# DSXiangLi/ChineseNER

Hardware: NVIDIA H100
Metric: sentences/sec bert_bilstm_crf MSRA L=128 (higher is better)
Workload: dtype bf16

## Files before the change

### chinesener_b200/_lib.py

```python
import ctypes
import os

import torch

_HERE = os.path.dirname(os.path.abspath(__file__))
LIB_PATH = os.path.join(_HERE, "libner_b200.so")

_c = ctypes
_vp, _i = _c.c_void_p, _c.c_int

SIGNATURES = {
    "ner_strerror": (_c.c_char_p, [_i]),
    "ner_abi_version": (_i, []),
    "ner_build_info": (_c.c_char_p, []),
    "ner_crf_viterbi": (_i, [_vp, _vp, _vp, _vp, _vp, _i, _i, _i, _vp]),
    "ner_crf_viterbi_plan": (_i, [_i, _i, _i, _i, _i]),
    "ner_crf_loglik_fwd": (_i, [_vp, _vp, _vp, _vp, _vp, _vp, _vp, _i, _i, _i, _i, _vp]),
    "ner_crf_loglik_bwd": (_i, [_vp, _vp, _vp, _vp, _vp, _vp, _vp, _c.c_float, _vp, _vp, _i, _i, _i, _vp]),
    "ner_crf_partial_loglik_fwd": (_i, [_vp, _vp, _vp, _vp, _vp, _vp, _vp, _i, _i, _i, _i, _vp]),
    "ner_crf_partial_loglik_bwd": (_i, [_vp, _vp, _vp, _vp, _vp, _vp, _vp, _c.c_float, _vp, _vp, _i, _i, _i, _vp]),
    "ner_crf_distill_fwd": (_i, [_vp, _vp, _vp, _vp, _vp, _c.c_float, _vp, _vp, _i, _i, _i, _i, _vp]),
    "ner_crf_distill_bwd": (_i, [_vp, _vp, _vp, _vp, _vp, _c.c_float, _vp, _vp, _vp, _c.c_float, _vp, _vp, _vp, _i, _i,
                                 _i, _i, _vp]),
    "ner_crf_viterbi_nbest_workspace_bytes": (_c.c_size_t, [_i, _i, _i, _i]),
    "ner_crf_viterbi_nbest": (_i, [_vp, _vp, _vp, _i, _vp, _vp, _vp, _vp, _c.c_size_t, _i, _i, _i, _vp]),
    "ner_gemm_bf16": (_i, [_vp, _vp, _vp, _vp, _vp, _i, _i, _i, _i, _i, _vp]),
    "ner_pack_weight_bf16": (_i, [_vp, _vp, _i, _i, _vp]),
    "ner_cast_bf16": (_i, [_vp, _vp, _c.c_size_t, _vp]),
    "ner_dense_small_n": (_i, [_vp, _i, _vp, _vp, _vp, _i, _i, _i, _vp, _vp]),
    "ner_seq_pack_plan": (_i, [_vp, _vp, _vp, _i, _i, _vp]),
    "ner_bert_embed_ln": (_i, [_vp] * 9 + [_i] * 6 + [_c.c_float, _vp, _i, _vp]),
    "ner_layernorm": (_i, [_vp, _i] + [_vp] * 5 + [_i, _i, _c.c_float, _vp]),
    "ner_layernorm_dropout": (_i, [_vp, _i] + [_vp] * 5 + [_i, _i, _c.c_float, _c.c_float, _c.c_uint64, _vp]),
    "ner_bert_attention": (_i, [_vp, _vp, _vp, _i, _i, _i, _i, _c.c_float, _c.c_float, _vp, _i, _c.c_float, _c.c_uint64, _vp]),
    "ner_bilstm_recurrence": (_i, [_vp] * 5 + [_i, _i, _i, _i, _c.c_float, _vp, _vp, _vp, _vp, _c.c_float, _c.c_uint64, _vp]),
    "ner_bilstm_recurrence_bwd": (_i, [_vp] * 7 + [_i, _i, _i, _i, _c.c_float, _c.c_uint64, _vp]),
    "ner_bigru_recurrence": (_i, [_vp] * 5 + [_i, _i, _i, _i, _i] + [_vp] * 4 + [_c.c_float, _c.c_uint64, _vp]),
    "ner_bigru_recurrence_bwd": (_i, [_vp] * 7 + [_i, _i, _i, _i, _c.c_float, _c.c_uint64, _vp]),
    "ner_transpose_cast_bf16": (_i, [_vp, _vp, _i, _i, _i, _i, _vp]),
    "ner_colsum_add": (_i, [_vp, _vp, _i, _i, _i, _c.c_float, _vp]),
    "ner_dense_small_n_bwd": (_i, [_vp] * 6 + [_i, _i, _i, _vp]),
    "ner_dropout": (_i, [_vp, _vp, _c.c_size_t, _c.c_float, _c.c_uint64, _vp]),
    "ner_relu_bwd_f32": (_i, [_vp, _vp, _vp, _c.c_size_t, _vp]),
    "ner_relu_f32": (_i, [_vp, _vp, _c.c_size_t, _vp]),
    "ner_reduce_max_time": (_i, [_vp, _vp, _i, _i, _i, _vp]),
    "ner_reduce_max_time_bwd": (_i, [_vp, _vp, _vp, _vp, _i, _i, _i, _c.c_float, _vp]),
    "ner_softmax_xent": (_i, [_vp, _vp, _vp, _vp, _i, _i, _c.c_float, _vp]),
    "ner_attention_f32_bwd": (_i, [_vp, _i, _vp, _i, _vp, _i, _vp, _vp, _vp, _vp, _c.c_float, _vp, _i, _vp, _i, _vp, _i, _vp, _i,
                                   _vp, _vp, _i, _i, _i, _i, _vp]),
    "ner_dropout_bf16": (_i, [_vp, _vp, _c.c_size_t, _c.c_float, _c.c_uint64, _vp]),
    "ner_sumsq_add": (_i, [_vp, _c.c_size_t, _vp, _vp, _vp]),
    "ner_sumsq_scratch_floats": (_c.c_size_t, []),
    "ner_token_xent": (_i, [_vp] * 6 + [_c.c_float, _vp, _i, _i, _i, _vp]),
    "ner_token_xent_scratch_floats": (_c.c_size_t, []),
    "ner_token_dice": (_i, [_vp] * 6 + [_c.c_float] * 3 + [_vp, _i, _i, _i, _vp]),
    "ner_mrc_pairs": (_i, [_vp] * 6 + [_i] * 6 + [_vp] * 7),
    "ner_mrc_merge": (_i, [_vp] * 3 + [_i] * 6 + [_vp, _vp]),
    "ner_mrc_span_targets": (_i, [_vp, _vp, _i, _i, _vp, _vp, _vp, _vp]),
    "ner_mrc_span_match_fwd_workspace_bytes": (_c.c_size_t, [_i, _i]),
    "ner_mrc_span_match_fwd": (_i, [_vp, _i] + [_vp] * 5 + [_i] * 3 + [_c.c_float, _c.c_uint64] + [_vp] * 3
                               + [_c.c_size_t, _vp]),
    "ner_mrc_span_match_bwd_workspace_bytes": (_c.c_size_t, [_i, _i]),
    "ner_mrc_span_match_bwd": (_i, [_vp, _i] + [_vp] * 5 + [_i] * 3 + [_c.c_float, _c.c_float, _c.c_uint64] + [_vp] * 5
                               + [_c.c_size_t, _vp]),
    "ner_mrc_span_decode_workspace_bytes": (_c.c_size_t, [_i, _i]),
    "ner_mrc_span_decode": (_i, [_vp] * 3 + [_i] + [_vp] * 5 + [_i] * 8 + [_vp] * 5 + [_c.c_size_t, _vp]),
    "ner_gp_targets": (_i, [_vp] * 3 + [_i] * 3 + [_vp, _vp]),
    "ner_gp_rope": (_i, [_vp, _i, _vp] + [_i] * 3 + [_vp] * 3),
    "ner_gp_rope_bwd": (_i, [_vp, _vp] + [_i] * 3 + [_vp, _i, _vp]),
    "ner_gp_loss_workspace_bytes": (_c.c_size_t, [_i] * 3),
    "ner_gp_loss_fwd": (_i, [_vp] * 5 + [_i] * 3 + [_vp] * 3 + [_c.c_size_t, _vp]),
    "ner_gp_loss_bwd": (_i, [_vp] * 5 + [_i] * 3 + [_c.c_float, _vp, _vp]),
    "ner_gp_decode_workspace_bytes": (_c.c_size_t, [_i] * 3),
    "ner_gp_decode": (_i, [_vp] * 5 + [_i] * 7 + [_vp] * 5 + [_c.c_size_t, _vp]),
    "ner_window_plan": (_i, [_vp] * 3 + [_i] * 5 + [_vp] * 6),
    "ner_layernorm_bwd": (_i, [_vp, _i] + [_vp] * 7 + [_i, _i, _c.c_float, _vp]),
    "ner_layernorm_dropout_bwd": (_i, [_vp, _i] + [_vp] * 7 + [_i, _i, _c.c_float, _c.c_float, _c.c_uint64, _vp]),
    "ner_layernorm_dropout_bwd_bias": (_i, [_vp, _i] + [_vp] * 8 + [_i, _i, _c.c_float, _c.c_float, _c.c_uint64, _vp]),
    "ner_transpose_bf16": (_i, [_vp, _vp, _i, _i, _i, _vp]),
    "ner_colsum_bf16_add": (_i, [_vp, _vp, _i, _i, _vp]),
    "ner_gelu_bf16": (_i, [_vp, _vp, _c.c_size_t, _i, _vp]),
    "ner_gelu_f32": (_i, [_vp, _vp, _c.c_size_t, _i, _vp]),
    "ner_gelu_bwd_bf16": (_i, [_vp, _vp, _vp, _c.c_size_t, _i, _vp]),
    "ner_gelu_bwd_bias_bf16": (_i, [_vp, _vp, _vp, _vp, _i, _i, _i, _vp]),
    "ner_bert_embed_bwd": (_i, [_vp] * 6 + [_i] * 5 + [_vp]),
    "ner_bert_attention_bwd": (_i, [_vp] * 5 + [_i] * 4 + [_c.c_float, _c.c_float, _c.c_float, _c.c_uint64, _vp]),
    "ner_bert_attention_bwd_packed": (_i, [_vp] * 5 + [_i] * 4 + [_c.c_float, _c.c_float, _c.c_uint64, _vp]),
    "ner_gather_rows": (_i, [_vp, _vp, _vp, _i, _i, _vp]),
    "ner_scatter_rows": (_i, [_vp, _vp, _vp, _i, _i, _vp]),
    "ner_adam_step": (_i, [_vp] * 4 + [_c.c_size_t] + [_c.c_float] * 5 + [_i, _c.c_float, _vp, _c.c_float, _vp]),
    "ner_softlexicon_pool_fwd": (_i, [_vp] * 4 + [_i] * 6 + [_vp]),
    "ner_embedding_lookup": (_i, [_vp, _vp, _vp, _i, _i, _i, _i, _vp]),
    "ner_cast_pad_bf16": (_i, [_vp, _vp, _i, _i, _i, _i, _vp]),
    "ner_split_bf16": (_i, [_vp, _vp, _vp, _i, _i, _i, _i, _vp]),
    "ner_attention_f32": (_i, [_vp, _i, _vp, _i, _vp, _i, _vp, _vp, _vp, _vp, _c.c_float, _vp, _vp, _vp, _i, _i, _i, _i, _vp]),
    "ner_softlexicon_pool_bwd": (_i, [_vp] * 4 + [_i] * 5 + [_vp]),
    "ner_multihot_embed_fwd": (_i, [_vp] * 3 + [_i] * 4 + [_vp]),
    "ner_small_table_grad_scratch_floats": (_c.c_size_t, [_i, _i]),
    "ner_small_table_grad": (_i, [_vp] * 4 + [_i] * 4 + [_vp, _vp]),
    "ner_gemm_e4m3": (_i, [_vp] * 7 + [_i] * 4 + [_vp]),
    "ner_quantize_weight_e4m3": (_i, [_vp, _vp, _vp, _i, _i, _vp]),
    "ner_bert_embed_ln_e4m3": (_i, [_vp] * 11 + [_i] * 6 + [_c.c_float, _vp, _i, _vp]),
    "ner_layernorm_e4m3": (_i, [_vp, _i] + [_vp] * 7 + [_i, _i, _c.c_float, _vp]),
}



class BertConfig(_c.Structure):
    _fields_ = [("hidden_size", _i), ("num_heads", _i), ("intermediate_size", _i), ("num_layers", _i),
                ("vocab_size", _i), ("type_vocab_size", _i), ("max_position", _i), ("ln_eps", _c.c_float),
                ("gelu_erf", _i), ("gemm_tile", _i)]


class BertLayerWeights(_c.Structure):
    _fields_ = [(n, _vp) for n in ("wqkv", "bqkv", "wo", "bo", "ln1_gamma", "ln1_beta", "wi", "bi", "wd", "bd",
                                   "ln2_gamma", "ln2_beta")]


class BertLayerWeightsFp8(_c.Structure):
    _fields_ = [(n, _vp) for n in ("wqkv", "sqkv", "bqkv", "wo", "bo", "ln1_gamma", "ln1_beta", "wi", "si", "bi", "wd", "sd",
                                   "bd", "ln2_gamma", "ln2_beta")]


class BertLayerGrads(_c.Structure):
    _fields_ = [(n, _vp) for n in ("wqkv_kn", "wo_kn", "wi_kn", "wd_kn", "d_wq", "d_wk", "d_wv", "d_bq", "d_bk", "d_bv",
                                   "d_wo", "d_bo", "d_ln1_gamma", "d_ln1_beta", "d_wi", "d_bi", "d_wd", "d_bd",
                                   "d_ln2_gamma", "d_ln2_beta")]


SIGNATURES["ner_bert_train_saved_bytes"] = (_c.c_size_t, [_c.POINTER(BertConfig), _i])
SIGNATURES["ner_bert_train_scratch_bytes"] = (_c.c_size_t, [_c.POINTER(BertConfig), _i])
SIGNATURES["ner_bert_encoder_train_fwd"] = (_i, [_c.POINTER(BertConfig)] + [_vp] * 5 + [_c.POINTER(BertLayerWeights)] + [_vp] * 3
                                            + [_i, _i, _c.c_float, _c.c_float, _c.c_uint64, _vp, _vp, _vp, _c.c_size_t, _vp])
SIGNATURES["ner_bert_encoder_train_bwd"] = (_i, [_c.POINTER(BertConfig), _vp, _c.POINTER(BertLayerWeights), _c.POINTER(BertLayerGrads)]
                                            + [_vp] * 5 + [_vp] * 3 + [_i, _i, _c.c_float, _c.c_float, _c.c_uint64, _vp, _vp,
                                                                       _c.c_size_t, _vp, _c.c_size_t, _vp])
SIGNATURES["ner_bert_train_packed_saved_bytes"] = (_c.c_size_t, [_c.POINTER(BertConfig), _i])
SIGNATURES["ner_bert_train_packed_scratch_bytes"] = (_c.c_size_t, [_c.POINTER(BertConfig), _i, _i])
SIGNATURES["ner_bert_encoder_train_fwd_packed"] = (_i, [_c.POINTER(BertConfig)] + [_vp] * 5 + [_c.POINTER(BertLayerWeights)] + [_vp] * 2
                                                   + [_i, _i, _vp, _vp, _i, _c.c_float, _c.c_float, _c.c_uint64, _vp, _vp, _vp,
                                                      _c.c_size_t, _vp])
SIGNATURES["ner_bert_encoder_train_bwd_packed"] = (_i, [_c.POINTER(BertConfig), _vp, _c.POINTER(BertLayerWeights),
                                                        _c.POINTER(BertLayerGrads)] + [_vp] * 5 + [_vp] * 2
                                                   + [_i, _i, _vp, _vp, _i, _c.c_float, _c.c_float, _c.c_uint64, _vp, _vp,
                                                      _c.c_size_t, _vp, _c.c_size_t, _vp])
SIGNATURES["ner_bert_bilstm_crf_predict_workspace_bytes"] = (_c.c_size_t, [_c.POINTER(BertConfig), _i, _i, _i, _i, _i])
SIGNATURES["ner_bert_bilstm_crf_predict"] = (_i, [_c.POINTER(BertConfig)] + [_vp] * 5 + [_c.POINTER(BertLayerWeights)] + [_vp] * 4
                                             + [_i, _i] + [_vp] * 3 + [_i] + [_vp] * 4 + [_i, _i, _i, _vp, _vp, _c.c_size_t, _vp])
SIGNATURES["ner_bert_embed_sum"] = (_i, [_vp] * 6 + [_i] * 6 + [_vp])
SIGNATURES["ner_axpy_f32"] = (_i, [_vp, _vp, _c.c_size_t, _c.c_float, _vp])
SIGNATURES["ner_bert_encoder_workspace_bytes"] = (_c.c_size_t, [_c.POINTER(BertConfig), _i])
SIGNATURES["ner_bert_encoder_fwd"] = (_i, [_c.POINTER(BertConfig)] + [_vp] * 5 + [_c.POINTER(BertLayerWeights)] + [_vp] * 3
                                      + [_i, _i, _vp, _vp, _i, _vp, _vp, _vp, _c.c_size_t, _vp])
SIGNATURES["ner_bert_encoder_fp8_workspace_bytes"] = (_c.c_size_t, [_c.POINTER(BertConfig), _i])
SIGNATURES["ner_bert_encoder_fwd_fp8"] = (_i, [_c.POINTER(BertConfig)] + [_vp] * 5 + [_c.POINTER(BertLayerWeightsFp8)] + [_vp] * 3
                                          + [_i, _i, _vp, _vp, _i, _vp, _vp, _vp, _c.c_size_t, _vp])

class PackEntry(_c.Structure):
    _fields_ = [("src", _vp), ("K", _i), ("N", _i), ("dst_nk_bf16", _vp), ("ld_nk", _i), ("dst_kn_bf16", _vp), ("ld_kn", _i)]


SIGNATURES["ner_pack_weights_group_bf16"] = (_i, [_vp, _vp, _i, _i, _vp])


class WgradProblem(_c.Structure):
    _fields_ = [("x_bf16", _vp), ("ld_x", _i), ("dy_bf16", _vp), ("ld_dy", _i), ("dy_col0", _i), ("dw", _vp), ("k_in", _i),
                ("n_out", _i)]


SIGNATURES["ner_wgrad_group_bf16"] = (_i, [_c.POINTER(WgradProblem), _i, _i, _vp])
SIGNATURES["ner_bert_train_bwd_set_layer_events"] = (_i, [_vp, _i])
SIGNATURES["ner_extract_spans"] = (_i, [_vp, _vp, _vp, _vp, _i, _i, _i, _i, _vp])
SIGNATURES["ner_lexicon_create"] = (_vp, [_vp, _vp, _vp, _i])
SIGNATURES["ner_lexicon_destroy"] = (None, [_vp])
SIGNATURES["ner_lexicon_num_nodes"] = (_c.c_int64, [_vp])
SIGNATURES["ner_lexicon_build"] = (_i, [_vp, _vp, _vp, _i, _vp, _vp, _i, _i, _vp, _vp, _i])
SIGNATURES["ner_lexicon_build_lattice"] = (_i, [_vp, _vp, _vp, _i, _i, _i, _vp, _vp, _vp, _i])
SIGNATURES["ner_lattice_recurrence"] = (_i, [_vp] * 9 + [_i] * 4 + [_vp] * 8)
SIGNATURES["ner_lattice_recurrence_bwd"] = (_i, [_vp] * 16 + [_i] * 4 + [_vp])

VIT_PLANS = ("small", "tma", "parked", "onchip_128", "onchip_32", "small_any_b", "none")

_lib = None


class NerB200Error(RuntimeError):
    pass


def lib():
    global _lib
    if _lib is None:
        if not os.path.exists(LIB_PATH):
            raise NerB200Error(
                f"{LIB_PATH} not found: build it with `python -m chinesener_b200.build` "
                "(there is no CPU fallback for the sm_90a kernels)")
        h = ctypes.CDLL(LIB_PATH)
        for name, (res, args) in SIGNATURES.items():
            fn = getattr(h, name)
            fn.restype = res
            fn.argtypes = args
        _lib = h
    return _lib


LAUNCHES = 0
_HOOK = None


def check(status):
    global LAUNCHES
    LAUNCHES += 1
    if status != 0:
        raise NerB200Error(lib().ner_strerror(status).decode())


def ptr(t):
    return 0 if t is None else t.data_ptr()


_raw_stream = getattr(torch._C, "_cuda_getCurrentRawStream", None)


def stream():
    if _raw_stream is not None:
        return _raw_stream(torch.cuda.current_device())
    return torch.cuda.current_stream().cuda_stream


def require_cuda(*tensors):
    for t in tensors:
        if t is not None and not t.is_cuda:
            raise NerB200Error("ner_b200 kernels take CUDA tensors (got a CPU tensor); there is no CPU path")
        if t is not None and not t.is_contiguous():
            raise NerB200Error("ner_b200 kernels take contiguous row-major tensors")
```

### chinesener_b200/csrc/bert_ops.cu

```cuda
#include "common.cuh"

namespace {

using namespace nerdev;

constexpr int LN_MAXV = 8;

template <bool Q = false>
__device__ __forceinline__ void ln_row(float4 (&v)[LN_MAXV], int nv4, int H, int lane, float eps,
                                       const float* __restrict__ gamma, const float* __restrict__ beta,
                                       float* __restrict__ out_f32, __nv_bfloat16* __restrict__ out_bf16,
                                       uint8_t* __restrict__ out_q = nullptr, float* __restrict__ out_s = nullptr) {
  float s = 0.f;
#pragma unroll
  for (int k = 0; k < LN_MAXV; ++k)
    if (k < nv4 && (lane + 32 * k) * 4 < H) s += v[k].x + v[k].y + v[k].z + v[k].w;
  s = warp_sum(s);
  const float mean = s / (float)H;
  float q = 0.f;
#pragma unroll
  for (int k = 0; k < LN_MAXV; ++k)
    if (k < nv4 && (lane + 32 * k) * 4 < H) {
      const float a = v[k].x - mean, b = v[k].y - mean, c = v[k].z - mean, d = v[k].w - mean;
      q += a * a + b * b + c * c + d * d;
    }
  q = warp_sum(q);
  const float rstd = rsqrtf(q / (float)H + eps);
#pragma unroll
  for (int k = 0; k < LN_MAXV; ++k) {
    const int e = (lane + 32 * k) * 4;
    if (k < nv4 && e < H) {
      const float4 g = __ldg(reinterpret_cast<const float4*>(gamma + e));
      const float4 b = __ldg(reinterpret_cast<const float4*>(beta + e));
      float4 o;
      o.x = (v[k].x - mean) * rstd * g.x + b.x;
      o.y = (v[k].y - mean) * rstd * g.y + b.y;
      o.z = (v[k].z - mean) * rstd * g.z + b.z;
      o.w = (v[k].w - mean) * rstd * g.w + b.w;
      if (out_f32 != nullptr) *reinterpret_cast<float4*>(out_f32 + e) = o;
      if (out_bf16 != nullptr) {
        __nv_bfloat162 lo = __floats2bfloat162_rn(o.x, o.y), hi = __floats2bfloat162_rn(o.z, o.w);
        uint2 pk;
        pk.x = *reinterpret_cast<uint32_t*>(&lo);
        pk.y = *reinterpret_cast<uint32_t*>(&hi);
        *reinterpret_cast<uint2*>(out_bf16 + e) = pk;
      }
      if constexpr (Q) {
        const float s = e4m3_scale(warp_max(fmaxf(fmaxf(fabsf(o.x), fabsf(o.y)), fmaxf(fabsf(o.z), fabsf(o.w)))));
        const uint32_t lo = cvt_e4m3x2(__fdiv_rn(o.x, s), __fdiv_rn(o.y, s)), hi = cvt_e4m3x2(__fdiv_rn(o.z, s), __fdiv_rn(o.w, s));
        *reinterpret_cast<uint32_t*>(out_q + e) = lo | (hi << 16);
        if (lane == 0) out_s[k] = s;
      }
    }
  }
}

template <bool Q>
__global__ void __launch_bounds__(256)
bert_embed_ln_kernel(const float* __restrict__ word_emb, const float* __restrict__ type_emb,
                     const float* __restrict__ pos_emb, const float* __restrict__ gamma,
                     const float* __restrict__ beta, const int32_t* __restrict__ ids,
                     const int32_t* __restrict__ seg, float* __restrict__ out_f32,
                     __nv_bfloat16* __restrict__ out_bf16, int n_tok, int L, int H, int V, int n_type, float eps,
                     const int32_t* __restrict__ tok_src, uint8_t* __restrict__ out_q, float* __restrict__ out_s) {
  const int lane = threadIdx.x & 31;
  const int nv4 = (H / 4 + 31) / 32;
  for (int tok = blockIdx.x * (blockDim.x >> 5) + (threadIdx.x >> 5); tok < n_tok; tok += gridDim.x * (blockDim.x >> 5)) {
    const int src = tok_src ? tok_src[tok] : tok;
    int id = ids[src];
    id = min(max(id, 0), V - 1);
    int sg = (seg != nullptr) ? seg[src] : 0;
    sg = min(max(sg, 0), n_type - 1);
    const int pos = src % L;
    const float* w = word_emb + (size_t)id * H;
    const float* ty = type_emb + (size_t)sg * H;
    const float* po = pos_emb + (size_t)pos * H;
    float4 v[LN_MAXV];
#pragma unroll
    for (int k = 0; k < LN_MAXV; ++k) {
      const int e = (lane + 32 * k) * 4;
      if (k < nv4 && e < H) {
        const float4 a = __ldg(reinterpret_cast<const float4*>(w + e));
        const float4 b = __ldg(reinterpret_cast<const float4*>(ty + e));
        const float4 c = __ldg(reinterpret_cast<const float4*>(po + e));
        v[k] = make_float4(a.x + b.x + c.x, a.y + b.y + c.y, a.z + b.z + c.z, a.w + b.w + c.w);
      }
    }
    ln_row<Q>(v, nv4, H, lane, eps, gamma, beta, out_f32 ? out_f32 + (size_t)tok * H : nullptr,
              out_bf16 ? out_bf16 + (size_t)tok * H : nullptr, Q ? out_q + (size_t)tok * H : nullptr,
              Q ? out_s + (size_t)tok * (H / 128) : nullptr);
  }
}

__global__ void __launch_bounds__(256)
bert_embed_sum_kernel(const float* __restrict__ word_emb, const float* __restrict__ type_emb,
                      const float* __restrict__ pos_emb, const int32_t* __restrict__ ids, const int32_t* __restrict__ seg,
                      float* __restrict__ out, int n_tok, int L, int H, int V, int n_type) {
  const int lane = threadIdx.x & 31;
  for (int tok = blockIdx.x * (blockDim.x >> 5) + (threadIdx.x >> 5); tok < n_tok; tok += gridDim.x * (blockDim.x >> 5)) {
    const int id = min(max(ids[tok], 0), V - 1);
    const int sg = min(max(seg != nullptr ? seg[tok] : 0, 0), n_type - 1);
    const float* w = word_emb + (size_t)id * H;
    const float* ty = type_emb + (size_t)sg * H;
    const float* po = pos_emb + (size_t)(tok % L) * H;
    for (int e = lane * 4; e < H; e += 128) {
      const float4 a = __ldg(reinterpret_cast<const float4*>(w + e));
      const float4 b = __ldg(reinterpret_cast<const float4*>(ty + e));
      const float4 c = __ldg(reinterpret_cast<const float4*>(po + e));
      *reinterpret_cast<float4*>(out + (size_t)tok * H + e) = make_float4(a.x + b.x + c.x, a.y + b.y + c.y, a.z + b.z + c.z, a.w + b.w + c.w);
    }
  }
}

template <bool YBF16, bool DROP, bool Q>
__global__ void __launch_bounds__(256)
layernorm_kernel(const void* __restrict__ yv, const float* __restrict__ residual, const float* __restrict__ gamma,
                 const float* __restrict__ beta, float* __restrict__ out_f32, __nv_bfloat16* __restrict__ out_bf16,
                 int M, int H, float eps, float keep, uint32_t seed_lo, uint32_t seed_hi, uint8_t* __restrict__ out_q,
                 float* __restrict__ out_s) {
  pdl_launch_dependents();
  pdl_wait();
  const int lane = threadIdx.x & 31;
  const int nv4 = (H / 4 + 31) / 32;
  const uint32_t thr = keep_threshold(keep);
  const float inv_keep = 1.f / keep;
  for (int row = blockIdx.x * (blockDim.x >> 5) + (threadIdx.x >> 5); row < M; row += gridDim.x * (blockDim.x >> 5)) {
    const float* r = residual ? residual + (size_t)row * H : nullptr;
    float4 v[LN_MAXV];
#pragma unroll
    for (int k = 0; k < LN_MAXV; ++k) {
      const int e = (lane + 32 * k) * 4;
      if (k < nv4 && e < H) {
        if constexpr (YBF16) {
          const uint2 pk = *reinterpret_cast<const uint2*>(static_cast<const __nv_bfloat16*>(yv) + (size_t)row * H + e);
          const __nv_bfloat162 lo = *reinterpret_cast<const __nv_bfloat162*>(&pk.x);
          const __nv_bfloat162 hi = *reinterpret_cast<const __nv_bfloat162*>(&pk.y);
          v[k] = make_float4(__low2float(lo), __high2float(lo), __low2float(hi), __high2float(hi));
        } else {
          v[k] = *reinterpret_cast<const float4*>(static_cast<const float*>(yv) + (size_t)row * H + e);
        }
        if constexpr (DROP) {
          const size_t i = (size_t)row * H + e;
          const uint32_t hi = seed_hi ^ (uint32_t)(i >> 32), lo = (uint32_t)i;
          v[k].x = hash3(seed_lo, hi, lo) < thr ? v[k].x * inv_keep : 0.f;
          v[k].y = hash3(seed_lo, hi, lo + 1) < thr ? v[k].y * inv_keep : 0.f;
          v[k].z = hash3(seed_lo, hi, lo + 2) < thr ? v[k].z * inv_keep : 0.f;
          v[k].w = hash3(seed_lo, hi, lo + 3) < thr ? v[k].w * inv_keep : 0.f;
        }
        if (r != nullptr) {
          const float4 b = *reinterpret_cast<const float4*>(r + e);
          v[k].x += b.x;
          v[k].y += b.y;
          v[k].z += b.z;
          v[k].w += b.w;
        }
      }
    }
    ln_row<Q>(v, nv4, H, lane, eps, gamma, beta, out_f32 ? out_f32 + (size_t)row * H : nullptr,
              out_bf16 ? out_bf16 + (size_t)row * H : nullptr, Q ? out_q + (size_t)row * H : nullptr,
              Q ? out_s + (size_t)row * (H / 128) : nullptr);
  }
}

__global__ void __launch_bounds__(256)
pack_weight_kernel(const float* __restrict__ src, __nv_bfloat16* __restrict__ dst, int K, int N) {
  __shared__ float tile[32][33];
  const int k0 = blockIdx.y * 32, n0 = blockIdx.x * 32;
  const int tx = threadIdx.x & 31, ty = threadIdx.x >> 5;
  for (int i = ty; i < 32; i += 8) {
    const int k = k0 + i, n = n0 + tx;
    tile[i][tx] = (k < K && n < N) ? src[(size_t)k * N + n] : 0.f;
  }
  __syncthreads();
  for (int i = ty; i < 32; i += 8) {
    const int n = n0 + i, k = k0 + tx;
    if (n < N && k < K) dst[(size_t)n * K + k] = __float2bfloat16_rn(tile[tx][i]);
  }
}

__global__ void __launch_bounds__(256)
pack_group_kernel(const ner_pack_entry* __restrict__ entries, const int32_t* __restrict__ tile_start, int count) {
  __shared__ __nv_bfloat16 tile[64][66];
  int e = 0;
  {
    int lo = 0, hi = count;
    while (hi - lo > 1) {
      const int mid = (lo + hi) >> 1;
      if (tile_start[mid] <= (int)blockIdx.x) lo = mid; else hi = mid;
    }
    e = lo;
  }
  const ner_pack_entry en = entries[e];
  const int t = blockIdx.x - tile_start[e], tn = (en.N + 63) / 64;
  const int k0 = (t / tn) * 64, n0 = (t % tn) * 64;
  const int c4 = (threadIdx.x & 15) * 4, r = threadIdx.x >> 4;
  __nv_bfloat16* kn = static_cast<__nv_bfloat16*>(en.dst_kn_bf16);
  __nv_bfloat16* nk = static_cast<__nv_bfloat16*>(en.dst_nk_bf16);
#pragma unroll
  for (int i = 0; i < 4; ++i) {
    const int k = k0 + r + 16 * i, n = n0 + c4;
    float4 v = make_float4(0.f, 0.f, 0.f, 0.f);
    if (k < en.K) {
      if (n + 3 < en.N && (en.N & 3) == 0) v = *reinterpret_cast<const float4*>(en.src + (size_t)k * en.N + n);
      else {
        if (n < en.N) v.x = en.src[(size_t)k * en.N + n];
        if (n + 1 < en.N) v.y = en.src[(size_t)k * en.N + n + 1];
        if (n + 2 < en.N) v.z = en.src[(size_t)k * en.N + n + 2];
        if (n + 3 < en.N) v.w = en.src[(size_t)k * en.N + n + 3];
      }
    }
    const __nv_bfloat16 b0 = __float2bfloat16_rn(v.x), b1 = __float2bfloat16_rn(v.y), b2 = __float2bfloat16_rn(v.z),
                        b3 = __float2bfloat16_rn(v.w);
    tile[r + 16 * i][c4] = b0; tile[r + 16 * i][c4 + 1] = b1; tile[r + 16 * i][c4 + 2] = b2; tile[r + 16 * i][c4 + 3] = b3;
    if (kn != nullptr && k < en.K) {
      __nv_bfloat16* d = kn + (size_t)k * en.ld_kn + n;
      if (n + 3 < en.N && (en.ld_kn & 3) == 0 && (reinterpret_cast<uintptr_t>(kn) & 7) == 0) {
        __nv_bfloat162 lo = __halves2bfloat162(b0, b1), hi = __halves2bfloat162(b2, b3);
        *reinterpret_cast<uint2*>(d) = make_uint2(*reinterpret_cast<uint32_t*>(&lo), *reinterpret_cast<uint32_t*>(&hi));
      } else {
        if (n < en.N) d[0] = b0;
        if (n + 1 < en.N) d[1] = b1;
        if (n + 2 < en.N) d[2] = b2;
        if (n + 3 < en.N) d[3] = b3;
      }
    }
  }
  __syncthreads();
  if (nk != nullptr) {
#pragma unroll
    for (int i = 0; i < 4; ++i) {
      const int n = n0 + r + 16 * i, k = k0 + c4;
      if (n < en.N) {
        __nv_bfloat16* d = nk + (size_t)n * en.ld_nk + k;
        const __nv_bfloat16 b0 = tile[c4][r + 16 * i], b1 = tile[c4 + 1][r + 16 * i], b2 = tile[c4 + 2][r + 16 * i],
                            b3 = tile[c4 + 3][r + 16 * i];
        if (k + 3 < en.K && (en.ld_nk & 3) == 0 && (reinterpret_cast<uintptr_t>(nk) & 7) == 0) {
          __nv_bfloat162 lo = __halves2bfloat162(b0, b1), hi = __halves2bfloat162(b2, b3);
          *reinterpret_cast<uint2*>(d) = make_uint2(*reinterpret_cast<uint32_t*>(&lo), *reinterpret_cast<uint32_t*>(&hi));
        } else {
          if (k < en.K) d[0] = b0;
          if (k + 1 < en.K) d[1] = b1;
          if (k + 2 < en.K) d[2] = b2;
          if (k + 3 < en.K) d[3] = b3;
        }
      }
    }
  }
}

__global__ void __launch_bounds__(256)
quantize_weight_e4m3_kernel(const float* __restrict__ src, uint8_t* __restrict__ dst, float* __restrict__ scale, int K, int N) {
  __shared__ float tile[32][33];
  __shared__ float red[8][32];
  const int n0 = blockIdx.x * 32, tx = threadIdx.x & 31, ty = threadIdx.x >> 5, n = n0 + tx;
  float m = 0.f;
  if (n < N)
    for (int k = ty; k < K; k += 8) m = fmaxf(m, fabsf(src[(size_t)k * N + n]));
  red[ty][tx] = m;
  __syncthreads();
  if (ty == 0) {
    for (int i = 1; i < 8; ++i) m = fmaxf(m, red[i][tx]);
    const float s = e4m3_scale(m);
    red[0][tx] = s;
    if (n < N) scale[n] = s;
  }
  __syncthreads();
  for (int k0 = 0; k0 < K; k0 += 32) {
    for (int i = ty; i < 32; i += 8) {
      const int k = k0 + i;
      tile[i][tx] = (k < K && n < N) ? src[(size_t)k * N + n] : 0.f;
    }
    __syncthreads();
    for (int i = ty; i < 32; i += 8) {
      const int nn = n0 + i, k = k0 + tx;
      if (nn < N && k < K) dst[(size_t)nn * K + k] = (uint8_t)(cvt_e4m3x2(__fdiv_rn(tile[tx][i], red[0][i]), 0.f) & 0xffu);
    }
    __syncthreads();
  }
}

__global__ void __launch_bounds__(256)
cast_bf16_kernel(const float* __restrict__ src, __nv_bfloat16* __restrict__ dst, size_t n) {
  const size_t stride = (size_t)gridDim.x * blockDim.x;
  for (size_t i = (size_t)blockIdx.x * blockDim.x + threadIdx.x; i < n; i += stride) dst[i] = __float2bfloat16_rn(src[i]);
}

template <typename XT, int NMAX>
__global__ void __launch_bounds__(256)
dense_small_n_kernel(const XT* __restrict__ x, const float* __restrict__ W, const float* __restrict__ bias,
                     float* __restrict__ out, int M, int F, int N, const int32_t* __restrict__ row_map) {
  extern __shared__ float s_w[];
  for (int e = threadIdx.x; e < F * N; e += blockDim.x) s_w[e] = W[e];
  __syncthreads();
  const int lane = threadIdx.x & 31;
  for (int row = blockIdx.x * (blockDim.x >> 5) + (threadIdx.x >> 5); row < M; row += gridDim.x * (blockDim.x >> 5)) {
    float acc[NMAX];
#pragma unroll
    for (int n = 0; n < NMAX; ++n) acc[n] = 0.f;
    const XT* xr = x + (size_t)row * F;
    for (int f = lane; f < F; f += 32) {
      float xv;
      if constexpr (sizeof(XT) == 2) xv = __bfloat162float(xr[f]);
      else xv = xr[f];
      const float* wr = s_w + f * N;
#pragma unroll
      for (int n = 0; n < NMAX; ++n)
        if (n < N) acc[n] = fmaf(xv, wr[n], acc[n]);
    }
#pragma unroll
    for (int n = 0; n < NMAX; ++n) acc[n] = warp_sum(acc[n]);
    if (lane < N) {
      float v = 0.f;
#pragma unroll
      for (int n = 0; n < NMAX; ++n)
        if (n == lane) v = acc[n];
      const size_t orow = row_map ? (size_t)row_map[row] : (size_t)row;
      out[orow * N + lane] = v + (bias ? bias[lane] : 0.f);
    }
  }
}


__global__ void __launch_bounds__(256)
embedding_lookup_kernel(const float* __restrict__ table, const int32_t* __restrict__ ids, float* __restrict__ out,
                        int n_tok, int E, int V, int ld_out) {
  const int lane = threadIdx.x & 31;
  const int wpb = blockDim.x >> 5;
  for (int tok = blockIdx.x * wpb + (threadIdx.x >> 5); tok < n_tok; tok += gridDim.x * wpb) {
    const int id = min(max(ids[tok], 0), V - 1);
    const float* row = table + (size_t)id * E;
    float* o = out + (size_t)tok * ld_out;
    for (int e = lane; e < E; e += 32) o[e] = __ldg(row + e);
  }
}

__global__ void __launch_bounds__(256)
cast_pad_bf16_kernel(const float* __restrict__ src, __nv_bfloat16* __restrict__ dst, int M, int D, int Dp, int ld_src) {
  const size_t total = (size_t)M * Dp;
  const size_t stride = (size_t)gridDim.x * blockDim.x;
  for (size_t i = (size_t)blockIdx.x * blockDim.x + threadIdx.x; i < total; i += stride) {
    const size_t r = i / Dp;
    const int c = (int)(i - r * Dp);
    dst[i] = __float2bfloat16_rn(c < D ? src[r * ld_src + c] : 0.f);
  }
}

__global__ void __launch_bounds__(1024)
seq_pack_plan_kernel(const int32_t* __restrict__ mask, int32_t* __restrict__ cu, int32_t* __restrict__ tok_src, int B, int L) {
  extern __shared__ int s_plan[];
  const int warp = threadIdx.x >> 5, lane = threadIdx.x & 31, nw = blockDim.x >> 5;
  for (int b = warp; b < B; b += nw) {
    int c = 0;
    for (int t = lane; t < L; t += 32) c += (mask[(size_t)b * L + t] != 0);
#pragma unroll
    for (int o = 16; o > 0; o >>= 1) c += __shfl_xor_sync(0xffffffffu, c, o);
    if (lane == 0) s_plan[b + 1] = c;
  }
  __syncthreads();
  if (threadIdx.x == 0) {
    s_plan[0] = 0;
    for (int b = 0; b < B; ++b) s_plan[b + 1] += s_plan[b];
  }
  __syncthreads();
  for (int b = threadIdx.x; b <= B; b += blockDim.x) cu[b] = s_plan[b];
  for (int b = warp; b < B; b += nw) {
    const int o = s_plan[b], n = s_plan[b + 1] - o;
    for (int t = lane; t < n; t += 32) tok_src[o + t] = b * L + t;
  }
}

__global__ void __launch_bounds__(256)
split_bf16_kernel(const float* __restrict__ src, __nv_bfloat16* __restrict__ hi, __nv_bfloat16* __restrict__ lo, int M,
                  int D, int Dp, int ld_src) {
  const size_t total = (size_t)M * Dp;
  const size_t stride = (size_t)gridDim.x * blockDim.x;
  for (size_t i = (size_t)blockIdx.x * blockDim.x + threadIdx.x; i < total; i += stride) {
    const size_t r = i / Dp;
    const int c = (int)(i - r * Dp);
    const float x = c < D ? src[r * ld_src + c] : 0.f;
    const __nv_bfloat16 h = __float2bfloat16_rn(x);
    hi[i] = h;
    lo[i] = __float2bfloat16_rn(x - __bfloat162float(h));
  }
}

int grid_for_rows(int rows, int rows_per_block) {
  long g = ((long)rows + rows_per_block - 1) / rows_per_block;
  if (g > (long)ner_num_sms() * 16) g = (long)ner_num_sms() * 16;
  if (g < 1) g = 1;
  return (int)g;
}

}

extern "C" int ner_bert_embed_ln(const float* word_emb, const float* type_emb, const float* pos_emb,
                                 const float* gamma, const float* beta, const int32_t* ids, const int32_t* seg,
                                 float* out_f32, void* out_bf16, int B, int L, int H, int vocab, int n_type,
                                 int max_pos, float eps, const int32_t* tok_src, int n_packed, ner_stream_t stream) {
  if (B < 0 || L < 1 || H < 4 || vocab < 1 || n_type < 1) return NER_ERR_INVALID_ARG;
  if (B == 0) return NER_OK;
  if (!word_emb || !type_emb || !pos_emb || !gamma || !beta || !ids || (!out_f32 && !out_bf16)) return NER_ERR_INVALID_ARG;
  if (H % 4 != 0 || H > 128 * LN_MAXV || L > max_pos) return NER_ERR_UNSUPPORTED;
  const int n_tok = tok_src ? n_packed : B * L;
  if (n_tok < 0 || n_tok > B * L) return NER_ERR_INVALID_ARG;
  if (n_tok == 0) return NER_OK;
  bert_embed_ln_kernel<false><<<grid_for_rows(n_tok, 8), 256, 0, static_cast<cudaStream_t>(stream)>>>(
      word_emb, type_emb, pos_emb, gamma, beta, ids, seg, out_f32, static_cast<__nv_bfloat16*>(out_bf16), n_tok, L, H,
      vocab, n_type, eps, tok_src, nullptr, nullptr);
  return ner_launch_status();
}

extern "C" int ner_bert_embed_sum(const float* word_emb, const float* type_emb, const float* pos_emb, const int32_t* ids,
                                  const int32_t* seg, float* out, int B, int L, int H, int vocab, int n_type, int max_pos,
                                  ner_stream_t stream) {
  if (B < 0 || L < 1 || H < 4 || H % 4 != 0) return NER_ERR_INVALID_ARG;
  if (B == 0) return NER_OK;
  if (!word_emb || !type_emb || !pos_emb || !ids || !out || L > max_pos) return NER_ERR_INVALID_ARG;
  bert_embed_sum_kernel<<<grid_for_rows(B * L, 8), 256, 0, static_cast<cudaStream_t>(stream)>>>(word_emb, type_emb, pos_emb, ids,
                                                                                             seg, out, B * L, L, H, vocab, n_type);
  return ner_launch_status();
}

extern "C" int ner_layernorm_dropout(const void* y, int y_is_bf16, const float* residual, const float* gamma,
                                     const float* beta, float* out_f32, void* out_bf16, int M, int H, float eps,
                                     float keep_prob, uint64_t seed, ner_stream_t stream) {
  if (M < 0 || H < 4) return NER_ERR_INVALID_ARG;
  if (M == 0) return NER_OK;
  if (!y || !gamma || !beta || (!out_f32 && !out_bf16)) return NER_ERR_INVALID_ARG;
  if (!(keep_prob > 0.f) || keep_prob > 1.f) return NER_ERR_INVALID_ARG;
  if (H % 4 != 0 || H > 128 * LN_MAXV) return NER_ERR_UNSUPPORTED;
  const bool drop = keep_prob < 1.f;
  auto kern = y_is_bf16 ? (drop ? layernorm_kernel<true, true, false> : layernorm_kernel<true, false, false>)
                        : (drop ? layernorm_kernel<false, true, false> : layernorm_kernel<false, false, false>);
  cudaError_t e = ner_launch_pdl(kern, dim3(grid_for_rows(M, 8)), dim3(256), 0, static_cast<cudaStream_t>(stream), y, residual,
                                 gamma, beta, out_f32, static_cast<__nv_bfloat16*>(out_bf16), M, H, eps, keep_prob,
                                 (uint32_t)seed, (uint32_t)(seed >> 32), (uint8_t*)nullptr, (float*)nullptr);
  if (e != cudaSuccess) return NER_ERR_CUDA_BASE - (int)e;
  return ner_launch_status();
}

extern "C" int ner_layernorm(const void* y, int y_is_bf16, const float* residual, const float* gamma,
                             const float* beta, float* out_f32, void* out_bf16, int M, int H, float eps,
                             ner_stream_t stream) {
  return ner_layernorm_dropout(y, y_is_bf16, residual, gamma, beta, out_f32, out_bf16, M, H, eps, 1.0f, 0, stream);
}

extern "C" int ner_pack_weight_bf16(const float* w_kn, void* wt_nk_bf16, int K, int N, ner_stream_t stream) {
  if (K < 1 || N < 1 || !w_kn || !wt_nk_bf16) return NER_ERR_INVALID_ARG;
  dim3 grid((N + 31) / 32, (K + 31) / 32);
  pack_weight_kernel<<<grid, 256, 0, static_cast<cudaStream_t>(stream)>>>(w_kn, static_cast<__nv_bfloat16*>(wt_nk_bf16), K, N);
  return ner_launch_status();
}

extern "C" int ner_pack_weights_group_bf16(const ner_pack_entry* entries_device, const int32_t* tile_start_device, int count,
                                           int total_tiles, ner_stream_t stream) {
  if (count < 0 || total_tiles < 0) return NER_ERR_INVALID_ARG;
  if (count == 0 || total_tiles == 0) return NER_OK;
  if (!entries_device || !tile_start_device) return NER_ERR_INVALID_ARG;
  pack_group_kernel<<<total_tiles, 256, 0, static_cast<cudaStream_t>(stream)>>>(entries_device, tile_start_device, count);
  return ner_launch_status();
}

extern "C" int ner_cast_bf16(const float* src, void* dst_bf16, size_t n, ner_stream_t stream) {
  if (!src || !dst_bf16) return n == 0 ? NER_OK : NER_ERR_INVALID_ARG;
  if (n == 0) return NER_OK;
  size_t g = (n + 255) / 256;
  if (g > ner_num_sms() * 32) g = ner_num_sms() * 32;
  cast_bf16_kernel<<<(int)g, 256, 0, static_cast<cudaStream_t>(stream)>>>(src, static_cast<__nv_bfloat16*>(dst_bf16), n);
  return ner_launch_status();
}

extern "C" int ner_dense_small_n(const void* x, int x_is_bf16, const float* W, const float* bias, float* out, int M,
                                 int F, int N, const int32_t* row_map, ner_stream_t stream) {
  if (M < 0 || F < 1 || N < 1) return NER_ERR_INVALID_ARG;
  if (M == 0) return NER_OK;
  if (!x || !W || !out) return NER_ERR_INVALID_ARG;
  if (N > 32 || (size_t)F * N * 4 > 200 * 1024) return NER_ERR_UNSUPPORTED;
  const size_t smem = (size_t)F * N * 4;
  cudaStream_t st = static_cast<cudaStream_t>(stream);
  const int grid = grid_for_rows(M, 8 * 4);
  cudaError_t e;
#define LAUNCH(XT, NM)                                                                                   \
  {                                                                                                      \
    auto kern = dense_small_n_kernel<XT, NM>;                                                            \
    e = cudaFuncSetAttribute(kern, cudaFuncAttributeMaxDynamicSharedMemorySize, (int)smem);              \
    if (e != cudaSuccess) return NER_ERR_CUDA_BASE - (int)e;                                             \
    kern<<<grid, 256, smem, st>>>(static_cast<const XT*>(x), W, bias, out, M, F, N, row_map);                     \
  }
  if (x_is_bf16) {
    if (N <= 16) LAUNCH(__nv_bfloat16, 16) else LAUNCH(__nv_bfloat16, 32)
  } else {
    if (N <= 16) LAUNCH(float, 16) else LAUNCH(float, 32)
  }
#undef LAUNCH
  return ner_launch_status();
}

extern "C" int ner_embedding_lookup(const float* table, const int32_t* ids, float* out, int n_tok, int E, int V,
                                    int ld_out, ner_stream_t stream) {
  if (n_tok < 0 || E < 1 || V < 1 || ld_out < E) return NER_ERR_INVALID_ARG;
  if (n_tok == 0) return NER_OK;
  if (!table || !ids || !out) return NER_ERR_INVALID_ARG;
  embedding_lookup_kernel<<<grid_for_rows(n_tok, 8), 256, 0, static_cast<cudaStream_t>(stream)>>>(table, ids, out, n_tok,
                                                                                               E, V, ld_out);
  return ner_launch_status();
}

extern "C" int ner_cast_pad_bf16(const float* src, void* dst_bf16, int M, int D, int Dp, int ld_src,
                                 ner_stream_t stream) {
  if (M < 0 || D < 1 || Dp < D || ld_src < D) return NER_ERR_INVALID_ARG;
  if (M == 0) return NER_OK;
  if (!src || !dst_bf16) return NER_ERR_INVALID_ARG;
  size_t g = ((size_t)M * Dp + 255) / 256;
  if (g > ner_num_sms() * 32) g = ner_num_sms() * 32;
  cast_pad_bf16_kernel<<<(int)g, 256, 0, static_cast<cudaStream_t>(stream)>>>(src, static_cast<__nv_bfloat16*>(dst_bf16), M,
                                                                              D, Dp, ld_src);
  return ner_launch_status();
}

extern "C" int ner_seq_pack_plan(const int32_t* mask, int32_t* cu_seqlens, int32_t* tok_src, int B, int L,
                                 ner_stream_t stream) {
  if (B < 0 || L < 1) return NER_ERR_INVALID_ARG;
  if (B == 0) return NER_OK;
  if (!mask || !cu_seqlens || !tok_src) return NER_ERR_INVALID_ARG;
  if ((size_t)(B + 1) * 4 > 200 * 1024) return NER_ERR_UNSUPPORTED;
  const size_t smem = (size_t)(B + 1) * 4;
  if (smem > 48 * 1024) {
    cudaError_t e = cudaFuncSetAttribute(seq_pack_plan_kernel, cudaFuncAttributeMaxDynamicSharedMemorySize, (int)smem);
    if (e != cudaSuccess) return NER_ERR_CUDA_BASE - (int)e;
  }
  seq_pack_plan_kernel<<<1, 1024, smem, static_cast<cudaStream_t>(stream)>>>(mask, cu_seqlens, tok_src, B, L);
  return ner_launch_status();
}

extern "C" int ner_split_bf16(const float* src, void* hi_bf16, void* lo_bf16, int M, int D, int Dp, int ld_src,
                              ner_stream_t stream) {
  if (M < 0 || D < 1 || Dp < D || ld_src < D) return NER_ERR_INVALID_ARG;
  if (M == 0) return NER_OK;
  if (!src || !hi_bf16 || !lo_bf16) return NER_ERR_INVALID_ARG;
  size_t g = ((size_t)M * Dp + 255) / 256;
  if (g > ner_num_sms() * 32) g = ner_num_sms() * 32;
  split_bf16_kernel<<<(int)g, 256, 0, static_cast<cudaStream_t>(stream)>>>(
      src, static_cast<__nv_bfloat16*>(hi_bf16), static_cast<__nv_bfloat16*>(lo_bf16), M, D, Dp, ld_src);
  return ner_launch_status();
}

extern "C" int ner_bert_embed_ln_e4m3(const float* word_emb, const float* type_emb, const float* pos_emb, const float* gamma,
                                      const float* beta, const int32_t* ids, const int32_t* seg, float* out_f32, void* out_bf16,
                                      void* out_e4m3, float* out_scale, int B, int L, int H, int vocab, int n_type, int max_pos,
                                      float eps, const int32_t* tok_src, int n_packed, ner_stream_t stream) {
  if (B < 0 || L < 1 || H < 4 || vocab < 1 || n_type < 1) return NER_ERR_INVALID_ARG;
  if (B == 0) return NER_OK;
  if (!word_emb || !type_emb || !pos_emb || !gamma || !beta || !ids || !out_e4m3 || !out_scale) return NER_ERR_INVALID_ARG;
  if (H % 128 != 0 || H > 128 * LN_MAXV || L > max_pos) return NER_ERR_UNSUPPORTED;
  const int n_tok = tok_src ? n_packed : B * L;
  if (n_tok < 0 || n_tok > B * L) return NER_ERR_INVALID_ARG;
  if (n_tok == 0) return NER_OK;
  bert_embed_ln_kernel<true><<<grid_for_rows(n_tok, 8), 256, 0, static_cast<cudaStream_t>(stream)>>>(
      word_emb, type_emb, pos_emb, gamma, beta, ids, seg, out_f32, static_cast<__nv_bfloat16*>(out_bf16), n_tok, L, H,
      vocab, n_type, eps, tok_src, static_cast<uint8_t*>(out_e4m3), out_scale);
  return ner_launch_status();
}

extern "C" int ner_layernorm_e4m3(const void* y, int y_is_bf16, const float* residual, const float* gamma, const float* beta,
                                  float* out_f32, void* out_bf16, void* out_e4m3, float* out_scale, int M, int H, float eps,
                                  ner_stream_t stream) {
  if (M < 0 || H < 4) return NER_ERR_INVALID_ARG;
  if (M == 0) return NER_OK;
  if (!y || !gamma || !beta || !out_e4m3 || !out_scale) return NER_ERR_INVALID_ARG;
  if (H % 128 != 0 || H > 128 * LN_MAXV) return NER_ERR_UNSUPPORTED;
  auto kern = y_is_bf16 ? layernorm_kernel<true, false, true> : layernorm_kernel<false, false, true>;
  cudaError_t e = ner_launch_pdl(kern, dim3(grid_for_rows(M, 8)), dim3(256), 0, static_cast<cudaStream_t>(stream), y, residual,
                                 gamma, beta, out_f32, static_cast<__nv_bfloat16*>(out_bf16), M, H, eps, 1.0f, 0u, 0u,
                                 static_cast<uint8_t*>(out_e4m3), out_scale);
  if (e != cudaSuccess) return NER_ERR_CUDA_BASE - (int)e;
  return ner_launch_status();
}

extern "C" int ner_quantize_weight_e4m3(const float* w_kn, void* wt_nk_e4m3, float* w_scale, int K, int N, ner_stream_t stream) {
  if (K < 1 || N < 1 || !w_kn || !wt_nk_e4m3 || !w_scale) return NER_ERR_INVALID_ARG;
  quantize_weight_e4m3_kernel<<<(N + 31) / 32, 256, 0, static_cast<cudaStream_t>(stream)>>>(
      w_kn, static_cast<uint8_t*>(wt_nk_e4m3), w_scale, K, N);
  return ner_launch_status();
}
```

### chinesener_b200/csrc/bilstm.cu

```cuda
#include <cooperative_groups.h>

#include "common.cuh"
#include "rnn_cluster.cuh"

namespace cg = cooperative_groups;

namespace {

template <int R, int ACT, int H4REG>
__global__ void __launch_bounds__(H4REG > 0 ? 256 : 512, 1) bilstm_rec_kernel(const float* __restrict__ xproj, const float* __restrict__ wh_fw,
                                  const float* __restrict__ wh_bw, const int32_t* __restrict__ seq_len,
                                  float* __restrict__ out, int B, int L, int H, int C, float forget_bias,
                                  const int32_t* __restrict__ cu_seqlens, float* __restrict__ gates_out,
                                  float* __restrict__ cstate_out, float* __restrict__ hstate_out, float keep_prob,
                                  uint32_t seed_lo, uint32_t seed_hi) {
  cg::cluster_group cluster = cg::this_cluster();
  const int HU = H / C;
  const int NC = 4 * HU;
  const int H4 = H / 4;
  const rnn::RowGroup grp = rnn::row_group(C, B, R);
  const int rank = grp.rank, dir = grp.dir, b0 = grp.b0;
  const int tid = threadIdx.x;

  extern __shared__ __align__(16) float smem[];
  constexpr bool WREG = H4REG > 0;
  float4* Ws4 = reinterpret_cast<float4*>(smem);
  float* hbuf = smem + (WREG ? 0 : (size_t)H * NC);
  int* s_len = reinterpret_cast<int*>(hbuf + 2 * R * H);
  uint64_t* hbar = reinterpret_cast<uint64_t*>(s_len + 8);

  const float* wh = dir == 0 ? wh_fw : wh_bw;
  float4 wreg[WREG ? H4REG : 1];
  if constexpr (WREG) {
    if (tid < NC) {
      const int g0 = tid & 3, u0 = tid >> 2;
      const size_t gc = (size_t)g0 * H + rank * HU + u0;
#pragma unroll
      for (int k4 = 0; k4 < H4REG; ++k4) {
        wreg[k4].x = wh[(size_t)(4 * k4 + 0) * 4 * H + gc];
        wreg[k4].y = wh[(size_t)(4 * k4 + 1) * 4 * H + gc];
        wreg[k4].z = wh[(size_t)(4 * k4 + 2) * 4 * H + gc];
        wreg[k4].w = wh[(size_t)(4 * k4 + 3) * 4 * H + gc];
      }
    }
  } else {
    for (int idx = tid; idx < H4 * NC; idx += blockDim.x) {
      const int k4 = idx / NC, col = idx - k4 * NC;
      const int g = col & 3, u = col >> 2;
      const size_t gc = (size_t)g * H + rank * HU + u;
      float4 w;
      w.x = wh[(size_t)(4 * k4 + 0) * 4 * H + gc];
      w.y = wh[(size_t)(4 * k4 + 1) * 4 * H + gc];
      w.z = wh[(size_t)(4 * k4 + 2) * 4 * H + gc];
      w.w = wh[(size_t)(4 * k4 + 3) * 4 * H + gc];
      Ws4[idx] = w;
    }
  }
  for (int idx = tid; idx < 2 * R * H; idx += blockDim.x) hbuf[idx] = 0.f;
  if (tid == 0) {
    rnn::mbar_init_(&hbar[0], 1);
    rnn::mbar_init_(&hbar[1], 1);
    asm volatile("fence.mbarrier_init.release.cluster;" ::: "memory");
  }
  const int maxlen = rnn::load_lengths<R>(s_len, seq_len, b0, B, L);
  cluster.sync();

  const bool col_ok = tid < NC;
  const int g = tid & 3, u = tid >> 2;
  const int ug = rank * HU + u;
  const size_t xcol = (size_t)dir * 4 * H + (size_t)g * H + ug;
  constexpr int RC = (R + 3) / 4;
  float c_state[RC];
#pragma unroll
  for (int rr = 0; rr < RC; ++rr) c_state[rr] = 0.f;

  size_t xrow0[R];
#pragma unroll
  for (int r = 0; r < R; ++r)
    xrow0[r] = (b0 + r < B) ? (cu_seqlens ? (size_t)cu_seqlens[b0 + r] : (size_t)(b0 + r) * L) : 0;
  float xp[R];
#pragma unroll
  for (int r = 0; r < R; ++r) {
    xp[r] = 0.f;
    const int len = s_len[r];
    if (col_ok && 0 < len) {
      const int pos = dir == 0 ? 0 : len - 1;
      xp[r] = xproj[(xrow0[r] + pos) * 8 * H + xcol];
    }
  }
  const uint32_t thr = nerdev::keep_threshold(keep_prob);
  const float inv_keep = 1.f / keep_prob;

  const uint32_t h_bytes = (uint32_t)(R * H * 4);
  for (int s = 0; s < maxlen; ++s) {
    const float* hcur = hbuf + (s & 1) * R * H;
    float* hnxt = hbuf + ((s + 1) & 1) * R * H;
    if (C > 1) {
      if (tid == 0) rnn::mbar_arrive_expect_tx_(&hbar[(s + 1) & 1], h_bytes);
      if (s > 0) rnn::mbar_wait_(&hbar[s & 1], (uint32_t)((s - 1) >> 1) & 1u);
    }
    nerdev::f32x2 pa[R], pb[R];
#pragma unroll
    for (int r = 0; r < R; ++r) {
      pa[r] = nerdev::pk2(xp[r], 0.f);
      pb[r] = nerdev::pk2(0.f, 0.f);
    }
    if (col_ok) {
#pragma unroll
      for (int r = 0; r < R; ++r) {
        const int len = s_len[r];
        xp[r] = 0.f;
        if (s + 1 < len) {
          const int pos = dir == 0 ? s + 1 : len - 2 - s;
          xp[r] = xproj[(xrow0[r] + pos) * 8 * H + xcol];
        }
      }
      const float4* hc4 = reinterpret_cast<const float4*>(hcur);
      if constexpr (WREG) {
#pragma unroll
        for (int k4 = 0; k4 < H4REG; ++k4) rnn::fma2_rows<R>(pa, pb, wreg[k4], hc4, H4, k4);
      } else {
#pragma unroll 4
        for (int k4 = 0; k4 < H4; ++k4) rnn::fma2_rows<R>(pa, pb, Ws4[k4 * NC + tid], hc4, H4, k4);
      }
    }
    float zi[RC], zj[RC], zf[RC], zo[RC];
#pragma unroll
    for (int rr = 0; rr < RC; ++rr) zi[rr] = zj[rr] = zf[rr] = zo[rr] = 0.f;
    const int qb = (tid & 31) & ~3;
#pragma unroll
    for (int r = 0; r < R; ++r) {
      const float z = rnn::sum_chains(pa[r], pb[r]);
      const float a0 = __shfl_sync(0xffffffffu, z, qb + 0);
      const float a1 = __shfl_sync(0xffffffffu, z, qb + 1);
      const float a2 = __shfl_sync(0xffffffffu, z, qb + 2);
      const float a3 = __shfl_sync(0xffffffffu, z, qb + 3);
      if (g == (r & 3)) {
        zi[r >> 2] = a0;
        zj[r >> 2] = a1;
        zf[r >> 2] = a2;
        zo[r >> 2] = a3;
      }
    }
#pragma unroll
    for (int rr = 0; rr < RC; ++rr) {
      const int r = g + 4 * rr;
      const bool cell_ok = col_ok && r < R;
      float i_s = 0.f, j_a = 0.f, f_s = 0.f, o_s = 0.f, h_out = 0.f, h_state = 0.f;
      const int len = cell_ok ? s_len[r] : 0;
      const int b = b0 + r;
      const bool live = cell_ok && s < len;
      const int pos = dir == 0 ? s : len - 1 - s;
      if (live) {
        i_s = rnn::sigmoid_fast(zi[rr]);
        j_a = rnn::act_fast<ACT>(zj[rr]);
        f_s = rnn::sigmoid_fast(zf[rr] + forget_bias);
        o_s = rnn::sigmoid_fast(zo[rr]);
        c_state[rr] = f_s * c_state[rr] + i_s * j_a;
        h_out = h_state = o_s * rnn::act_fast<ACT>(c_state[rr]);
        if (keep_prob < 1.f)
          rnn::dropout_out_state(h_out, h_state, seed_lo, seed_hi, thr, inv_keep, b, L, pos, H, dir, ug);
      }
      if (cell_ok) {
        if (C > 1) {
          const uint32_t la = nerdev::smem_u32(hnxt + r * H + ug), lb = nerdev::smem_u32(&hbar[(s + 1) & 1]);
          rnn::publish_all(la, lb, h_state, C);
        } else {
          hnxt[r * H + ug] = h_state;
        }
      }
      if (live) {
        out[((size_t)b * L + pos) * 2 * H + (size_t)dir * H + ug] = h_out;
        if (hstate_out != nullptr) hstate_out[((size_t)b * L + pos) * 2 * H + (size_t)dir * H + ug] = h_state;
        if (gates_out != nullptr) {
          const size_t gi = ((size_t)b * L + pos) * 8 * H + (size_t)dir * 4 * H;
          gates_out[gi + 0 * H + ug] = i_s;
          gates_out[gi + 1 * H + ug] = j_a;
          gates_out[gi + 2 * H + ug] = f_s;
          gates_out[gi + 3 * H + ug] = o_s;
          cstate_out[((size_t)b * L + pos) * 2 * H + (size_t)dir * H + ug] = c_state[rr];
        }
      } else if (cell_ok && b < B) {
        out[((size_t)b * L + s) * 2 * H + (size_t)dir * H + ug] = 0.f;
      }
    }
    if (C == 1) __syncthreads();
  }
  if (C > 1) cluster.sync();
  rnn::zero_past_maxlen(out, R, b0, B, L, H, dir, rank, HU, maxlen);
}

int pick_cluster(int H) {
  for (int C = 1; C <= 8; C *= 2) {
    if (H % C != 0) continue;
    const size_t bytes = (size_t)H * 4 * (H / C) * 4;
    if (bytes <= 190 * 1024 && 4 * (H / C) <= 512) return C;
  }
  return 0;
}

template <int R, int ACT, int H4REG>
int launch_rec(const float* xproj, const float* wh_fw, const float* wh_bw, const int32_t* seq_len, float* out, int B,
               int L, int H, int C, float forget_bias, const int32_t* cu_seqlens, float* gates_out, float* cstate_out,
               float* hstate_out, float keep_prob, uint64_t seed, cudaStream_t st) {
  const int HU = H / C, NC = 4 * HU;
  const size_t smem = ((H4REG > 0 ? 0 : (size_t)H * NC) + 2 * R * H + 32) * 4;
  return rnn::launch_cluster(bilstm_rec_kernel<R, ACT, H4REG>, B, R, C, (NC + 31) / 32 * 32, smem, st, xproj, wh_fw, wh_bw,
                             seq_len, out, B, L, H, C, forget_bias, cu_seqlens, gates_out, cstate_out, hstate_out,
                             keep_prob, (uint32_t)seed, (uint32_t)(seed >> 32));
}

}

extern "C" int ner_bilstm_recurrence(const float* xproj, const float* wh_fw, const float* wh_bw,
                                     const int32_t* seq_len, float* out, int B, int L, int H, int activation,
                                     float forget_bias, const int32_t* cu_seqlens, float* gates_out,
                                     float* cstate_out, float* hstate_out, float keep_prob, uint64_t seed,
                                     ner_stream_t stream) {
  if (B < 0 || L < 1 || H < 1) return NER_ERR_INVALID_ARG;
  if (B == 0) return NER_OK;
  if (!xproj || !wh_fw || !wh_bw || !seq_len || !out) return NER_ERR_INVALID_ARG;
  if ((gates_out == nullptr) != (cstate_out == nullptr)) return NER_ERR_INVALID_ARG;
  if (!(keep_prob > 0.f) || keep_prob > 1.f) return NER_ERR_INVALID_ARG;
  if (activation != 0 && activation != 1) return NER_ERR_INVALID_ARG;
  if (H % 4 != 0) return NER_ERR_UNSUPPORTED;
  const int C = pick_cluster(H);
  if (C == 0) return NER_ERR_UNSUPPORTED;
  cudaStream_t st = static_cast<cudaStream_t>(stream);
  int R = rnn::rows_per_cluster(B, C);
  if (H == 128 && (long)2 * ((B + 3) / 4) * C > ner_num_sms()) R = 8;
#define GO(RR, HR)                                                                                          \
  return activation == 1 ? launch_rec<RR, 1, HR>(xproj, wh_fw, wh_bw, seq_len, out, B, L, H, C, forget_bias, cu_seqlens, gates_out, cstate_out, hstate_out, keep_prob, seed, st) \
                         : launch_rec<RR, 0, HR>(xproj, wh_fw, wh_bw, seq_len, out, B, L, H, C, forget_bias, cu_seqlens, gates_out, cstate_out, hstate_out, keep_prob, seed, st)
  if (H == 128 && 4 * (H / C) <= 256) {
    if (R == 8) GO(8, 32);
    if (R == 2) GO(2, 32);
    GO(1, 32);
  }
  if (R >= 4) GO(4, 0);
  if (R == 2) GO(2, 0);
  GO(1, 0);
#undef GO
}
```

### chinesener_b200/csrc/predict_step.cu

```cuda
#include "common.cuh"

namespace {
inline size_t al256(size_t x) { return (x + 255) & ~(size_t)255; }
}

extern "C" size_t ner_bert_bilstm_crf_predict_workspace_bytes(const ner_bert_config* cfg, int B, int L, int rows,
                                                              int lstm_hidden, int num_tags) {
  if (!cfg || B < 0 || L < 1 || rows < 0) return 0;
  const size_t H = (size_t)cfg->hidden_size, R = (size_t)rows, Hl = (size_t)lstm_hidden;
  return al256((size_t)(B + 1) * 4)
         + al256((size_t)B * L * 4)
         + al256(R * H * 4) + al256(R * H * 2)
         + al256(R * 8 * Hl * 4)
         + al256((size_t)B * L * 2 * Hl * 4)
         + al256((size_t)B * L * num_tags * 4)
         + ner_bert_encoder_workspace_bytes(cfg, rows);
}

extern "C" int ner_bert_bilstm_crf_predict(const ner_bert_config* cfg, const float* word_emb, const float* type_emb,
                                           const float* pos_emb, const float* emb_ln_gamma, const float* emb_ln_beta,
                                           const ner_bert_layer_weights* layers, const void* lstm_wx_bf16,
                                           const float* lstm_bias, const float* lstm_wh_fw, const float* lstm_wh_bw,
                                           int lstm_hidden, int lstm_activation, const float* logits_w,
                                           const float* logits_b, const float* trans, int num_tags, const int32_t* ids,
                                           const int32_t* mask, const int32_t* seg, const int32_t* seq_len, int B, int L,
                                           int n_packed, int32_t* pred_ids, void* workspace, size_t workspace_bytes,
                                           ner_stream_t stream) {
  if (!cfg || !layers || !lstm_wx_bf16 || !lstm_bias || !lstm_wh_fw || !lstm_wh_bw || !logits_w || !logits_b || !trans ||
      !ids || !mask || !seq_len || !pred_ids || !workspace)
    return NER_ERR_INVALID_ARG;
  if (B < 0 || L < 1 || n_packed < 0 || n_packed > B * L) return NER_ERR_INVALID_ARG;
  if (B == 0) return NER_OK;
  const int H = cfg->hidden_size, Hl = lstm_hidden, K = num_tags;
  if (H % 8 != 0) return NER_ERR_UNSUPPORTED;
  if (workspace_bytes < ner_bert_bilstm_crf_predict_workspace_bytes(cfg, B, L, n_packed, Hl, K)) return NER_ERR_WORKSPACE;
  cudaStream_t st = static_cast<cudaStream_t>(stream);
  uint8_t* p = static_cast<uint8_t*>(workspace);
  int32_t* cu = reinterpret_cast<int32_t*>(p);       p += al256((size_t)(B + 1) * 4);
  int32_t* tok_src = reinterpret_cast<int32_t*>(p);  p += al256((size_t)B * L * 4);
  float* x32 = reinterpret_cast<float*>(p);          p += al256((size_t)n_packed * H * 4);
  void* x16 = p;                                     p += al256((size_t)n_packed * H * 2);
  float* xproj = reinterpret_cast<float*>(p);        p += al256((size_t)n_packed * 8 * Hl * 4);
  float* lstm_out = reinterpret_cast<float*>(p);     p += al256((size_t)B * L * 2 * Hl * 4);
  float* logits = reinterpret_cast<float*>(p);       p += al256((size_t)B * L * K * 4);
  void* enc_ws = p;
  const size_t enc_bytes = ner_bert_encoder_workspace_bytes(cfg, n_packed);

  int rc = ner_seq_pack_plan(mask, cu, tok_src, B, L, stream);
  if (rc != NER_OK) return rc;
  if (n_packed == 0) {
    if (cudaMemsetAsync(pred_ids, 0, (size_t)B * L * 4, st) != cudaSuccess) return NER_ERR_CUDA_BASE - (int)cudaGetLastError();
    return NER_OK;
  }
  rc = ner_bert_encoder_fwd(cfg, word_emb, type_emb, pos_emb, emb_ln_gamma, emb_ln_beta, layers, ids, mask, seg, B, L, cu,
                            tok_src, n_packed, x32, x16, enc_ws, enc_bytes, stream);
  if (rc != NER_OK) return rc;
  rc = ner_gemm_bf16(x16, lstm_wx_bf16, lstm_bias, nullptr, xproj, n_packed, 8 * Hl, H, NER_EPI_F32, cfg->gemm_tile, stream);
  if (rc != NER_OK) return rc;
  rc = ner_bilstm_recurrence(xproj, lstm_wh_fw, lstm_wh_bw, seq_len, lstm_out, B, L, Hl, lstm_activation, 1.0f, cu, nullptr,
                             nullptr, nullptr, 1.0f, 0, stream);
  if (rc != NER_OK) return rc;
  rc = ner_dense_small_n(lstm_out, 0, logits_w, logits_b, logits, B * L, 2 * Hl, K, nullptr, stream);
  if (rc != NER_OK) return rc;
  return ner_crf_viterbi(logits, seq_len, trans, pred_ids, nullptr, B, L, K, stream);
}
```

### chinesener_b200/csrc/rnn_cluster.cuh

```cuda
#pragma once
#include <cooperative_groups.h>
#include <stddef.h>
#include <stdint.h>

#include "common.cuh"

namespace rnn {


__device__ __forceinline__ uint32_t mapa_u32(uint32_t local_smem_addr, uint32_t rank) {
  uint32_t r;
  asm volatile("mapa.shared::cluster.u32 %0, %1, %2;" : "=r"(r) : "r"(local_smem_addr), "r"(rank));
  return r;
}
__device__ __forceinline__ void st_async_f32(uint32_t remote_addr, float v, uint32_t remote_bar) {
  asm volatile("st.async.weak.shared::cluster.mbarrier::complete_tx::bytes.b32 [%0], %1, [%2];" ::"r"(remote_addr),
               "r"(__float_as_uint(v)), "r"(remote_bar)
               : "memory");
}
__device__ __forceinline__ void mbar_init_(uint64_t* bar, uint32_t count) {
  asm volatile("mbarrier.init.shared::cta.b64 [%0], %1;" ::"r"(nerdev::smem_u32(bar)), "r"(count) : "memory");
}
__device__ __forceinline__ void mbar_arrive_expect_tx_(uint64_t* bar, uint32_t tx_bytes) {
  asm volatile("mbarrier.arrive.expect_tx.shared::cta.b64 _, [%0], %1;" ::"r"(nerdev::smem_u32(bar)), "r"(tx_bytes) : "memory");
}
__device__ __forceinline__ void mbar_wait_(uint64_t* bar, uint32_t parity) {
  uint32_t ok = 0;
  while (!ok) {
    asm volatile(
        "{\n\t.reg .pred p;\n\t"
        "mbarrier.try_wait.parity.shared::cta.b64 p, [%1], %2;\n\t"
        "selp.u32 %0, 1, 0, p;\n\t}"
        : "=r"(ok)
        : "r"(nerdev::smem_u32(bar)), "r"(parity)
        : "memory");
  }
}
__device__ __forceinline__ void publish_all(uint32_t la, uint32_t lb, float v, int C) {
  for (int dst = 0; dst < C; ++dst) st_async_f32(mapa_u32(la, (uint32_t)dst), v, mapa_u32(lb, (uint32_t)dst));
}


struct RowGroup {
  int rank;
  int dir;
  int b0;
};
__device__ __forceinline__ RowGroup row_group(int C, int B, int R) {
  const int ngroups = (B + R - 1) / R;
  const int cid = blockIdx.x / C;
  return RowGroup{(int)cooperative_groups::this_cluster().block_rank(), cid / ngroups, (cid % ngroups) * R};
}

template <int R>
__device__ __forceinline__ int load_lengths(int* s_len, const int32_t* __restrict__ seq_len, int b0, int B, int L) {
  const int tid = threadIdx.x;
  if (tid < R) s_len[tid] = (b0 + tid < B) ? min(max(seq_len[b0 + tid], 0), L) : 0;
  __syncthreads();
  int maxlen = 0;
#pragma unroll
  for (int r = 0; r < R; ++r) maxlen = max(maxlen, s_len[r]);
  return maxlen;
}


__device__ __forceinline__ float sigmoid_fast(float x) { return __fdividef(1.f, 1.f + __expf(-x)); }

template <int ACT>
__device__ __forceinline__ float act_fast(float x) {
  if (ACT == 1) return fmaxf(x, 0.f);
  return 1.f - __fdividef(2.f, 1.f + __expf(2.f * x));
}

template <int ACT>
__device__ __forceinline__ float act_grad_from_output(float a) {
  if (ACT == 1) return a > 0.f ? 1.f : 0.f;
  return 1.f - a * a;
}

__device__ __forceinline__ void dropout_out_state(float& out, float& state, uint32_t seed_lo, uint32_t seed_hi,
                                                  uint32_t thr, float inv_keep, int b, int L, int pos, int H, int dir,
                                                  int u) {
  const uint32_t e = (uint32_t)(((size_t)b * L + pos) * 2 * H + (size_t)dir * H + u);
  out = nerdev::hash3(seed_lo, seed_hi, e) < thr ? out * inv_keep : 0.f;
  state = nerdev::hash3(seed_lo ^ 0x5bd1e995u, seed_hi, e) < thr ? state * inv_keep : 0.f;
}

template <int R>
__device__ __forceinline__ void fma2_rows(nerdev::f32x2 (&a)[R], nerdev::f32x2 (&b)[R], float4 w, const float4* v4,
                                          int ld, int k4) {
#pragma unroll
  for (int r = 0; r < R; ++r) {
    const float4 v = v4[r * ld + k4];
    a[r] = nerdev::fma2(nerdev::pk2(w.x, w.y), nerdev::pk2(v.x, v.y), a[r]);
    b[r] = nerdev::fma2(nerdev::pk2(w.z, w.w), nerdev::pk2(v.z, v.w), b[r]);
  }
}
__device__ __forceinline__ float sum_chains(nerdev::f32x2 a, nerdev::f32x2 b) {
  float z0, z1, z2, z3;
  nerdev::upk2(a, z0, z1);
  nerdev::upk2(b, z2, z3);
  return (z0 + z1) + (z2 + z3);
}


__device__ __forceinline__ void zero_past_maxlen(float* out, int R, int b0, int B, int L, int H, int dir, int rank,
                                                 int HU, int maxlen) {
  for (int idx = threadIdx.x; idx < R * HU; idx += blockDim.x) {
    const int r = idx / HU, uu = idx - r * HU;
    const int b = b0 + r;
    if (b < B)
      for (int s = maxlen; s < L; ++s) out[((size_t)b * L + s) * 2 * H + (size_t)dir * H + rank * HU + uu] = 0.f;
  }
}

template <int G>
__device__ __forceinline__ void zero_unvisited(float* d_xproj, const int* s_len, int R, int b0, int B, int L, int H,
                                               int dir, int rank, int HU) {
  for (int idx = threadIdx.x; idx < R * G * HU; idx += blockDim.x) {
    const int r = idx / (G * HU), c = idx - r * G * HU;
    const int g = c / HU, u = c - g * HU;
    const int b = b0 + r;
    if (b < B)
      for (int t = s_len[r]; t < L; ++t)
        d_xproj[((size_t)b * L + t) * 2 * G * H + (size_t)dir * G * H + g * H + rank * HU + u] = 0.f;
  }
}


template <typename K, typename... Args>
int launch_cluster(K kern, int B, int R, int C, int threads, size_t smem, cudaStream_t st, Args... args) {
  cudaError_t e = cudaFuncSetAttribute(kern, cudaFuncAttributeMaxDynamicSharedMemorySize, (int)smem);
  if (e != cudaSuccess) return NER_ERR_CUDA_BASE - (int)e;
  cudaLaunchConfig_t cfg{};
  cfg.gridDim = dim3((unsigned)(2 * ((B + R - 1) / R) * C));
  cfg.blockDim = dim3((unsigned)threads);
  cfg.dynamicSmemBytes = smem;
  cfg.stream = st;
  cudaLaunchAttribute attr[1];
  attr[0].id = cudaLaunchAttributeClusterDimension;
  attr[0].val.clusterDim.x = (unsigned)C;
  attr[0].val.clusterDim.y = 1;
  attr[0].val.clusterDim.z = 1;
  cfg.attrs = attr;
  cfg.numAttrs = 1;
  e = cudaLaunchKernelEx(&cfg, kern, args...);
  if (e != cudaSuccess) return NER_ERR_CUDA_BASE - (int)e;
  return ner_launch_status();
}

static inline int rows_per_cluster(int B, int C) {
  int R = 1;
  if ((long)2 * B * C > ner_num_sms()) R = 2;
  if ((long)2 * ((B + 1) / 2) * C > 2 * ner_num_sms()) R = 4;
  return R;
}

static inline size_t gru_smem_bytes(int H, int C, int R) {
  const int NT = 4 * (H / C), H4 = H / 4;
  return (size_t)((H4 + 1) / 2 + (H4 + 3) / 4) * NT * 16 + (size_t)6 * R * H * 4 + 64;
}

static inline int gru_pick_cluster(int H) {
  for (int C = 1; C <= 8; C *= 2) {
    if (H % C != 0) continue;
    if (4 * (H / C) <= 512 && gru_smem_bytes(H, C, 4) <= 200 * 1024) return C;
  }
  return 0;
}

}
```

### chinesener_b200/ops.py

```python
import torch

from . import _lib
from ._lib import NerB200Error, check, lib, ptr, require_cuda, stream

EPI_F32, EPI_BF16, EPI_GELU_TANH_BF16, EPI_GELU_ERF_BF16, EPI_RELU_BF16, EPI_RES_F32, EPI_RES_RELU_F32 = range(7)
EPI_DIAG_DISCARD = 99
EPI_GELU_TANH_E4M3, EPI_GELU_ERF_E4M3 = 7, 8
E4M3 = torch.float8_e4m3fn
TILE_2CTA_128, TILE_2CTA_256 = 1128, 1256
TILE_SK_128, TILE_SK_256 = 2128, 2256
TILE_AUTO_THROUGHPUT = 3000
DEFAULT_TILE = 0


def _i32(t):
    return t if t.dtype == torch.int32 else t.to(torch.int32)


def crf_viterbi(logits, seq_len, trans, return_score=False):
    require_cuda(logits, seq_len, trans)
    assert logits.dtype == torch.float32 and trans.dtype == torch.float32
    B, L, K = logits.shape
    assert trans.shape == (K, K)
    seq_len = _i32(seq_len)
    tags = torch.empty((B, L), dtype=torch.int32, device=logits.device)
    score = torch.empty((B,), dtype=torch.float32, device=logits.device) if return_score else None
    check(lib().ner_crf_viterbi(ptr(logits), ptr(seq_len), ptr(trans), ptr(tags), ptr(score), B, L, K, stream()))
    return (tags, score) if return_score else tags


NBEST_MAX = 16


def crf_viterbi_nbest(logits, seq_len, trans, n):
    require_cuda(logits, seq_len, trans)
    assert logits.dtype == torch.float32 and trans.dtype == torch.float32
    B, L, K = logits.shape
    assert trans.shape == (K, K)
    n = int(n)
    seq_len = _i32(seq_len)
    dev = logits.device
    tags = torch.empty((B, n, L), dtype=torch.int32, device=dev)
    scores = torch.empty((B, n), dtype=torch.float32, device=dev)
    counts = torch.zeros((B,), dtype=torch.int32, device=dev)
    nbytes = int(lib().ner_crf_viterbi_nbest_workspace_bytes(B, L, K, n))
    ws = torch.empty((max(nbytes, 16),), dtype=torch.uint8, device=dev)
    check(lib().ner_crf_viterbi_nbest(ptr(logits), ptr(seq_len), ptr(trans), n, ptr(tags), ptr(scores), ptr(counts),
                                      ptr(ws), nbytes, B, L, K, stream()))
    return tags, scores, counts


def crf_loglik_fwd(logits, tags, seq_len, trans, want_alpha=False, exact=False):
    require_cuda(logits, tags, seq_len, trans)
    assert logits.dtype == torch.float32 and trans.dtype == torch.float32
    B, L, K = logits.shape
    tags, seq_len = _i32(tags), _i32(seq_len)
    ll = torch.empty((B,), dtype=torch.float32, device=logits.device)
    logz = torch.empty((B,), dtype=torch.float32, device=logits.device)
    alpha = torch.empty((B, L, K), dtype=torch.float32, device=logits.device) if want_alpha else None
    check(lib().ner_crf_loglik_fwd(ptr(logits), ptr(tags), ptr(seq_len), ptr(trans), ptr(ll), ptr(logz), ptr(alpha),
                                   B, L, K, 1 if exact else 0, stream()))
    return ll, logz, alpha


def gemm_bf16(a, wt, bias=None, residual=None, epilogue=EPI_BF16, tile_n=None, out=None):
    if tile_n is None:
        tile_n = DEFAULT_TILE
    require_cuda(a, wt, bias, residual, out)
    assert a.dtype == torch.bfloat16 and wt.dtype == torch.bfloat16
    M, K = a.shape
    N, K2 = wt.shape
    assert K == K2
    odt = torch.float32 if epilogue in (EPI_F32, EPI_RES_F32, EPI_RES_RELU_F32) else torch.bfloat16
    if out is None:
        out = torch.empty((M, N), dtype=odt, device=a.device)
    assert out.dtype == odt and out.shape == (M, N)
    if bias is not None:
        assert bias.dtype == torch.float32 and bias.numel() == N
    if residual is not None:
        assert residual.dtype == torch.float32 and residual.shape == (M, N)
    hook = _lib._HOOK
    if hook is not None:
        with hook("gemm_bf16", 2.0 * M * N * K):
            check(lib().ner_gemm_bf16(ptr(a), ptr(wt), ptr(bias), ptr(residual), ptr(out), M, N, K, epilogue, tile_n, stream()))
    else:
        check(lib().ner_gemm_bf16(ptr(a), ptr(wt), ptr(bias), ptr(residual), ptr(out), M, N, K, epilogue, tile_n, stream()))
    return out


def pack_weight_bf16(w_kn):
    require_cuda(w_kn)
    assert w_kn.dtype == torch.float32 and w_kn.dim() == 2
    K, N = w_kn.shape
    out = torch.empty((N, K), dtype=torch.bfloat16, device=w_kn.device)
    check(lib().ner_pack_weight_bf16(ptr(w_kn), ptr(out), K, N, stream()))
    return out


def gemm_e4m3(a, a_scale, wt, w_scale, bias=None, epilogue=EPI_BF16, out=None, out_scale=None):
    require_cuda(a, a_scale, wt, w_scale, bias, out, out_scale)
    assert a.dtype == E4M3 and wt.dtype == E4M3 and a_scale.dtype == torch.float32 and w_scale.dtype == torch.float32
    M, K = a.shape
    N, K2 = wt.shape
    assert K == K2 and w_scale.numel() == N and a_scale.shape == (M, K // 128)
    if bias is not None:
        assert bias.dtype == torch.float32 and bias.numel() == N
    q_out = epilogue in (EPI_GELU_TANH_E4M3, EPI_GELU_ERF_E4M3)
    if out is None:
        out = torch.empty((M, N), dtype=E4M3 if q_out else torch.bfloat16, device=a.device)
    if q_out and out_scale is None:
        out_scale = torch.empty((M, N // 128), dtype=torch.float32, device=a.device)
    hook = _lib._HOOK
    args = (ptr(a), ptr(a_scale), ptr(wt), ptr(w_scale), ptr(bias), ptr(out), ptr(out_scale), M, N, K, epilogue, stream())
    if hook is not None:
        with hook("gemm_e4m3", 2.0 * M * N * K):
            check(lib().ner_gemm_e4m3(*args))
    else:
        check(lib().ner_gemm_e4m3(*args))
    return (out, out_scale) if q_out else out


def quantize_weight_e4m3(w_kn):
    require_cuda(w_kn)
    assert w_kn.dtype == torch.float32 and w_kn.dim() == 2
    K, N = w_kn.shape
    q = torch.empty((N, K), dtype=E4M3, device=w_kn.device)
    sc = torch.empty((N,), dtype=torch.float32, device=w_kn.device)
    check(lib().ner_quantize_weight_e4m3(ptr(w_kn), ptr(q), ptr(sc), K, N, stream()))
    return q, sc


def cast_bf16(x):
    require_cuda(x)
    assert x.dtype == torch.float32
    out = torch.empty(x.shape, dtype=torch.bfloat16, device=x.device)
    check(lib().ner_cast_bf16(ptr(x), ptr(out), x.numel(), stream()))
    return out


def dense_small_n(x, w, bias=None, row_map=None, out=None):
    require_cuda(x, w, bias, row_map, out)
    assert w.dtype == torch.float32 and x.dtype in (torch.float32, torch.bfloat16)
    M, F = x.shape
    F2, N = w.shape
    assert F == F2
    if out is None:
        assert row_map is None
        out = torch.empty((M, N), dtype=torch.float32, device=x.device)
    check(lib().ner_dense_small_n(ptr(x), 1 if x.dtype == torch.bfloat16 else 0, ptr(w), ptr(bias), ptr(out), M, F, N,
                                  ptr(row_map), stream()))
    return out


def seq_pack_plan(mask):
    require_cuda(mask)
    B, L = mask.shape
    mask = _i32(mask)
    cu = torch.empty((B + 1,), dtype=torch.int32, device=mask.device)
    tok_src = torch.empty((B * L,), dtype=torch.int32, device=mask.device)
    check(lib().ner_seq_pack_plan(ptr(mask), ptr(cu), ptr(tok_src), B, L, stream()))
    return cu, tok_src


def bert_embed_ln(word_emb, type_emb, pos_emb, gamma, beta, ids, seg, eps=1e-12, want_f32=True, want_bf16=True,
                  tok_src=None, n_packed=0):
    require_cuda(word_emb, type_emb, pos_emb, gamma, beta, ids, seg, tok_src)
    B, L = ids.shape
    V, H = word_emb.shape
    ids = _i32(ids)
    seg = None if seg is None else _i32(seg)
    rows = n_packed if tok_src is not None else B * L
    of = torch.empty((rows, H), dtype=torch.float32, device=ids.device) if want_f32 else None
    ob = torch.empty((rows, H), dtype=torch.bfloat16, device=ids.device) if want_bf16 else None
    check(lib().ner_bert_embed_ln(ptr(word_emb), ptr(type_emb), ptr(pos_emb), ptr(gamma), ptr(beta), ptr(ids), ptr(seg),
                                  ptr(of), ptr(ob), B, L, H, V, type_emb.shape[0], pos_emb.shape[0], eps, ptr(tok_src),
                                  n_packed, stream()))
    return of, ob


def layernorm(y, gamma, beta, residual=None, eps=1e-12, want_f32=True, want_bf16=True, keep_prob=1.0, seed=0):
    require_cuda(y, gamma, beta, residual)
    assert y.dtype in (torch.float32, torch.bfloat16)
    M, H = y.shape
    of = torch.empty((M, H), dtype=torch.float32, device=y.device) if want_f32 else None
    ob = torch.empty((M, H), dtype=torch.bfloat16, device=y.device) if want_bf16 else None
    check(lib().ner_layernorm_dropout(ptr(y), 1 if y.dtype == torch.bfloat16 else 0, ptr(residual), ptr(gamma), ptr(beta),
                                      ptr(of), ptr(ob), M, H, eps, float(keep_prob), int(seed) & 0xFFFFFFFFFFFFFFFF, stream()))
    return of, ob


def bert_embed_ln_e4m3(word_emb, type_emb, pos_emb, gamma, beta, ids, seg, eps=1e-12, tok_src=None, n_packed=0):
    require_cuda(word_emb, type_emb, pos_emb, gamma, beta, ids, seg, tok_src)
    B, L = ids.shape
    V, H = word_emb.shape
    ids = _i32(ids)
    seg = None if seg is None else _i32(seg)
    rows = n_packed if tok_src is not None else B * L
    of = torch.empty((rows, H), dtype=torch.float32, device=ids.device)
    oq = torch.empty((rows, H), dtype=E4M3, device=ids.device)
    osc = torch.empty((rows, H // 128), dtype=torch.float32, device=ids.device)
    check(lib().ner_bert_embed_ln_e4m3(ptr(word_emb), ptr(type_emb), ptr(pos_emb), ptr(gamma), ptr(beta), ptr(ids), ptr(seg),
                                       ptr(of), None, ptr(oq), ptr(osc), B, L, H, V, type_emb.shape[0], pos_emb.shape[0], eps,
                                       ptr(tok_src), n_packed, stream()))
    return of, oq, osc


def layernorm_e4m3(y, gamma, beta, residual=None, eps=1e-12):
    require_cuda(y, gamma, beta, residual)
    assert y.dtype in (torch.float32, torch.bfloat16)
    M, H = y.shape
    of = torch.empty((M, H), dtype=torch.float32, device=y.device)
    oq = torch.empty((M, H), dtype=E4M3, device=y.device)
    osc = torch.empty((M, H // 128), dtype=torch.float32, device=y.device)
    check(lib().ner_layernorm_e4m3(ptr(y), 1 if y.dtype == torch.bfloat16 else 0, ptr(residual), ptr(gamma), ptr(beta),
                                   ptr(of), None, ptr(oq), ptr(osc), M, H, eps, stream()))
    return of, oq, osc


def bert_attention(qkv, mask, B, L, num_heads, head_dim=64, scale=None, mask_add=-10000.0, cu_seqlens=None, keep_prob=1.0,
                   seed=0):
    require_cuda(qkv, mask, cu_seqlens)
    assert qkv.dtype == torch.bfloat16 and qkv.shape[1] == 3 * num_heads * head_dim
    assert cu_seqlens is not None or qkv.shape[0] == B * L
    mask = None if mask is None else _i32(mask)
    ctx = torch.empty((qkv.shape[0], num_heads * head_dim), dtype=torch.bfloat16, device=qkv.device)
    if scale is None:
        scale = 1.0 / (head_dim ** 0.5)
    check(lib().ner_bert_attention(ptr(qkv), ptr(mask), ptr(ctx), B, L, num_heads, head_dim, scale, mask_add,
                                   ptr(cu_seqlens), int(qkv.shape[0]), float(keep_prob), int(seed) & 0xFFFFFFFFFFFFFFFF, stream()))
    return ctx


def bilstm_recurrence(xproj, wh_fw, wh_bw, seq_len, B, L, H, activation="tanh", forget_bias=1.0, cu_seqlens=None,
                      save_for_backward=False, keep_prob=1.0, seed=0):
    require_cuda(xproj, wh_fw, wh_bw, seq_len, cu_seqlens)
    assert xproj.dtype == torch.float32 and xproj.shape[1] == 8 * H
    assert cu_seqlens is not None or xproj.shape[0] == B * L
    assert wh_fw.shape == (H, 4 * H) and wh_bw.shape == (H, 4 * H)
    act = {"tanh": 0, "relu": 1}[activation]
    out = torch.empty((B, L, 2 * H), dtype=torch.float32, device=xproj.device)
    gates = cst = hst = None
    if save_for_backward:
        assert cu_seqlens is None, "training runs on the padded layout"
        gates = torch.zeros((B * L, 8 * H), dtype=torch.float32, device=xproj.device)
        cst = torch.zeros((B, L, 2 * H), dtype=torch.float32, device=xproj.device)
        hst = torch.zeros((B, L, 2 * H), dtype=torch.float32, device=xproj.device)
    check(lib().ner_bilstm_recurrence(ptr(xproj), ptr(wh_fw), ptr(wh_bw), ptr(_i32(seq_len)), ptr(out), B, L, H, act,
                                      forget_bias, ptr(cu_seqlens), ptr(gates), ptr(cst), ptr(hst), float(keep_prob),
                                      int(seed) & 0xFFFFFFFFFFFFFFFF, stream()))
    return (out, gates, cst, hst) if save_for_backward else out


def bilstm_recurrence_bwd(d_out, gates, cstate, wh_fw, wh_bw, seq_len, B, L, H, activation="tanh", keep_prob=1.0, seed=0):
    require_cuda(d_out, gates, cstate, wh_fw, wh_bw, seq_len)
    assert d_out.shape == (B, L, 2 * H) and d_out.dtype == torch.float32
    act = {"tanh": 0, "relu": 1}[activation]
    d_xproj = torch.empty((B * L, 8 * H), dtype=torch.float32, device=d_out.device)
    check(lib().ner_bilstm_recurrence_bwd(ptr(d_out), ptr(gates), ptr(cstate), ptr(wh_fw), ptr(wh_bw), ptr(_i32(seq_len)),
                                          ptr(d_xproj), B, L, H, act, float(keep_prob), int(seed) & 0xFFFFFFFFFFFFFFFF,
                                          stream()))
    return d_xproj


def bigru_recurrence(xproj, wh_fw, wh_bw, seq_len, B, L, H, activation="tanh", cu_seqlens=None, save_for_backward=False,
                     keep_prob=1.0, seed=0):
    require_cuda(xproj, wh_fw, wh_bw, seq_len, cu_seqlens)
    assert xproj.dtype == torch.float32 and xproj.shape[1] >= 6 * H
    assert cu_seqlens is not None or xproj.shape[0] == B * L
    assert wh_fw.shape == (H, 3 * H) and wh_bw.shape == (H, 3 * H)
    act = {"tanh": 0, "relu": 1}[activation]
    out = torch.empty((B, L, 2 * H), dtype=torch.float32, device=xproj.device)
    gates = hst = rh = None
    if save_for_backward:
        assert cu_seqlens is None, "training runs on the padded layout"
        gates = torch.zeros((B * L, 6 * H), dtype=torch.float32, device=xproj.device)
        hst = torch.zeros((B, L, 2 * H), dtype=torch.float32, device=xproj.device)
        rh = torch.zeros((B, L, 2 * H), dtype=torch.float32, device=xproj.device)
    check(lib().ner_bigru_recurrence(ptr(xproj), ptr(wh_fw), ptr(wh_bw), ptr(_i32(seq_len)), ptr(out), B, L, H, xproj.shape[1],
                                     act, ptr(cu_seqlens), ptr(gates), ptr(hst), ptr(rh), float(keep_prob),
                                     int(seed) & 0xFFFFFFFFFFFFFFFF, stream()))
    return (out, gates, hst, rh) if save_for_backward else out


def bigru_recurrence_bwd(d_out, gates, hstate, wh_fw, wh_bw, seq_len, B, L, H, activation="tanh", keep_prob=1.0, seed=0):
    require_cuda(d_out, gates, hstate, wh_fw, wh_bw, seq_len)
    assert d_out.shape == (B, L, 2 * H) and d_out.dtype == torch.float32
    assert gates.shape == (B * L, 6 * H) and hstate.shape == (B, L, 2 * H)
    act = {"tanh": 0, "relu": 1}[activation]
    d_xproj = torch.empty((B * L, 6 * H), dtype=torch.float32, device=d_out.device)
    check(lib().ner_bigru_recurrence_bwd(ptr(d_out), ptr(gates), ptr(hstate), ptr(wh_fw), ptr(wh_bw), ptr(_i32(seq_len)),
                                         ptr(d_xproj), B, L, H, act, float(keep_prob), int(seed) & 0xFFFFFFFFFFFFFFFF,
                                         stream()))
    return d_xproj


def lattice_recurrence(xproj, wproj, lat_len, wrec_fw, wrec_bw, wac_fw, wac_bw, seq_len, B, L, H, Kw,
                       save_for_backward=False):
    require_cuda(xproj, wproj, lat_len, wrec_fw, wrec_bw, wac_fw, wac_bw, seq_len)
    assert xproj.dtype == torch.float32 and xproj.shape == (B * L, 8 * H)
    assert wproj.dtype == torch.float32 and wproj.shape == (B * L * Kw, 6 * H)
    assert lat_len.dtype == torch.int32 and lat_len.numel() == B * L * Kw
    assert wrec_fw.shape == (H, 6 * H) and wrec_bw.shape == (H, 6 * H) and wac_fw.shape == (H, H) and wac_bw.shape == (H, H)
    dev = xproj.device
    out = torch.empty((B, L, 2 * H), dtype=torch.float32, device=dev)
    sv = None
    if save_for_backward:
        sv = dict(gates=torch.zeros((B * L, 6 * H), dtype=torch.float32, device=dev),
                  cstate=torch.zeros((B, L, 2 * H), dtype=torch.float32, device=dev),
                  norm=torch.zeros((B, L, 2 * H), dtype=torch.float32, device=dev),
                  wgates=torch.zeros((B * L * Kw, 6 * H), dtype=torch.float32, device=dev),
                  cw=torch.zeros((B * L * Kw, 2 * H), dtype=torch.float32, device=dev),
                  aw=torch.zeros((B * L * Kw, 2 * H), dtype=torch.float32, device=dev),
                  hw=torch.zeros((B * L * Kw, 2 * H), dtype=torch.float32, device=dev))
    s = sv or {}
    check(lib().ner_lattice_recurrence(ptr(xproj), ptr(wproj), ptr(lat_len), ptr(wrec_fw), ptr(wrec_bw), ptr(wac_fw),
                                       ptr(wac_bw), ptr(_i32(seq_len)), ptr(out), B, L, H, Kw, ptr(s.get('gates')),
                                       ptr(s.get('cstate')), ptr(s.get('norm')), ptr(s.get('wgates')), ptr(s.get('cw')),
                                       ptr(s.get('aw')), ptr(s.get('hw')), stream()))
    return (out, sv) if save_for_backward else out


def lattice_recurrence_bwd(d_out, saved, lat_len, wrec_fw, wrec_bw, wac_fw, wac_bw, seq_len, B, L, H, Kw):
    require_cuda(d_out, lat_len, wrec_fw, wrec_bw, wac_fw, wac_bw, seq_len)
    assert d_out.shape == (B, L, 2 * H) and d_out.dtype == torch.float32
    dev = d_out.device
    d_xproj = torch.empty((B * L, 8 * H), dtype=torch.float32, device=dev)
    d_wproj = torch.zeros((B * L * Kw, 6 * H), dtype=torch.float32, device=dev)
    d_alpha = torch.zeros((B * L * Kw, 2 * H), dtype=torch.float32, device=dev)
    s = saved
    check(lib().ner_lattice_recurrence_bwd(ptr(d_out), ptr(s['gates']), ptr(s['cstate']), ptr(s['norm']), ptr(s['wgates']),
                                           ptr(s['cw']), ptr(s['aw']), ptr(lat_len), ptr(wrec_fw), ptr(wrec_bw),
                                           ptr(wac_fw), ptr(wac_bw), ptr(_i32(seq_len)), ptr(d_xproj), ptr(d_wproj),
                                           ptr(d_alpha), B, L, H, Kw, stream()))
    return d_xproj, d_wproj, d_alpha


def softlexicon_pool(table, ids, weights, G=4, S=10, out=None):
    require_cuda(table, ids, weights, out)
    assert table.dtype == torch.float32 and weights.dtype == torch.float32
    V, E = table.shape
    lead = ids.shape[:-1]
    assert ids.shape[-1] == G * S and weights.shape == ids.shape
    n_tok = ids.numel() // (G * S)
    if out is None:
        out = torch.empty((*lead, G * E), dtype=torch.float32, device=table.device)
    ld = out.shape[-1]
    check(lib().ner_softlexicon_pool_fwd(ptr(table), ptr(_i32(ids)), ptr(weights), ptr(out), n_tok, G, S, E, V, ld,
                                         stream()))
    return out


def embedding_lookup(table, ids, out=None, col_offset=0):
    require_cuda(table, ids, out)
    assert table.dtype == torch.float32
    V, E = table.shape
    n_tok = ids.numel()
    if out is None:
        out = torch.empty((*ids.shape, E), dtype=torch.float32, device=table.device)
    ld = out.shape[-1]
    assert col_offset + E <= ld
    check(lib().ner_embedding_lookup(ptr(table), ptr(_i32(ids)), out.data_ptr() + 4 * col_offset, n_tok, E, V, ld, stream()))
    return out


def cast_pad_bf16(x2d, Dp):
    require_cuda(x2d)
    assert x2d.dtype == torch.float32 and x2d.dim() == 2
    M, D = x2d.shape
    out = torch.empty((M, Dp), dtype=torch.bfloat16, device=x2d.device)
    check(lib().ner_cast_pad_bf16(ptr(x2d), ptr(out), M, D, Dp, D, stream()))
    return out


def softlexicon_pool_bwd(d_table, ids, weights, d_out, G=4, S=10):
    require_cuda(d_table, ids, weights, d_out)
    V, E = d_table.shape
    n_tok = ids.numel() // (G * S)
    check(lib().ner_softlexicon_pool_bwd(ptr(d_table), ptr(_i32(ids)), ptr(weights), ptr(d_out), n_tok, G, S, E, V,
                                         stream()))
    return d_table


def multihot_embed(table, weights, out=None, col_offset=0):
    require_cuda(table, weights, out)
    assert table.dtype == torch.float32 and weights.dtype == torch.float32
    V, E = table.shape
    assert weights.shape[-1] == V
    n_tok = weights.numel() // V
    if out is None:
        out = torch.empty((*weights.shape[:-1], E), dtype=torch.float32, device=table.device)
    ld = out.shape[-1]
    assert col_offset + E <= ld and out.numel() == n_tok * ld
    check(lib().ner_multihot_embed_fwd(ptr(table), ptr(weights), out.data_ptr() + 4 * col_offset, n_tok, V, E, ld, stream()))
    return out


_small_table_scratch = {}


def small_table_grad(d_table, d_out, ids=None, weights=None, col_offset=0):
    require_cuda(d_table, d_out, ids, weights)
    assert (ids is None) != (weights is None)
    assert d_table.dtype == torch.float32 and d_out.dtype == torch.float32
    V, E = d_table.shape
    n_tok = ids.numel() if ids is not None else weights.numel() // V
    ld = d_out.shape[-1]
    assert col_offset + E <= ld and d_out.numel() == n_tok * ld
    need = int(lib().ner_small_table_grad_scratch_floats(V, E))
    key = (d_table.device.index, stream())
    scratch = _small_table_scratch.get(key)
    if scratch is None or scratch.numel() < need:
        scratch = _small_table_scratch[key] = torch.empty(max(need, 1), dtype=torch.float32, device=d_table.device)
    check(lib().ner_small_table_grad(ptr(d_table), ptr(None if ids is None else _i32(ids)), ptr(weights),
                                     d_out.data_ptr() + 4 * col_offset, n_tok, V, E, ld, ptr(scratch), stream()))
    return d_table


def crf_loglik_bwd(logits, tags, seq_len, trans, alpha, logz, d_ll=None, scale=1.0):
    require_cuda(logits, tags, seq_len, trans, alpha, logz, d_ll)
    B, L, K = logits.shape
    assert all(t.dtype == torch.float32 for t in (logits, trans, alpha, logz) + ((d_ll,) if d_ll is not None else ()))
    assert trans.shape == (K, K) and alpha.shape == (B, L, K) and logz.shape == (B,)
    assert d_ll is None or d_ll.shape == (B,)
    d_logits = torch.empty_like(logits)
    d_trans = torch.zeros_like(trans)
    check(lib().ner_crf_loglik_bwd(ptr(logits), ptr(_i32(tags)), ptr(_i32(seq_len)), ptr(trans), ptr(alpha), ptr(logz),
                                   ptr(d_ll), scale, ptr(d_logits), ptr(d_trans), B, L, K, stream()))
    return d_logits, d_trans


def crf_partial_loglik_fwd(logits, label_mask, seq_len, trans, want_alpha=False, exact=False):
    require_cuda(logits, label_mask, seq_len, trans)
    assert logits.dtype == torch.float32 and trans.dtype == torch.float32
    B, L, K = logits.shape
    assert trans.shape == (K, K) and label_mask.shape == (B, L)
    label_mask, seq_len = _i32(label_mask), _i32(seq_len)
    ll = torch.empty((B,), dtype=torch.float32, device=logits.device)
    logz = torch.empty((B, 2), dtype=torch.float32, device=logits.device)
    alpha = torch.empty((2, B, L, K), dtype=torch.float32, device=logits.device) if want_alpha else None
    check(lib().ner_crf_partial_loglik_fwd(ptr(logits), ptr(label_mask), ptr(seq_len), ptr(trans), ptr(ll), ptr(logz),
                                           ptr(alpha), B, L, K, 1 if exact else 0, stream()))
    return ll, logz, alpha


def crf_partial_loglik_bwd(logits, label_mask, seq_len, trans, alpha, logz, d_ll=None, scale=1.0):
    require_cuda(logits, label_mask, seq_len, trans, alpha, logz, d_ll)
    B, L, K = logits.shape
    assert all(t.dtype == torch.float32 for t in (logits, trans, alpha, logz) + ((d_ll,) if d_ll is not None else ()))
    assert trans.shape == (K, K) and alpha.shape == (2, B, L, K) and logz.shape == (B, 2)
    assert label_mask.shape == (B, L) and (d_ll is None or d_ll.shape == (B,))
    d_logits = torch.empty_like(logits)
    d_trans = torch.zeros_like(trans)
    check(lib().ner_crf_partial_loglik_bwd(ptr(logits), ptr(_i32(label_mask)), ptr(_i32(seq_len)), ptr(trans),
                                           ptr(alpha), ptr(logz), ptr(d_ll), scale, ptr(d_logits), ptr(d_trans),
                                           B, L, K, stream()))
    return d_logits, d_trans


def crf_distill_fwd(t_logits, t_trans, s_logits, s_trans, seq_len, temperature=1.0, exact=False):
    require_cuda(t_logits, t_trans, s_logits, s_trans, seq_len)
    assert all(t.dtype == torch.float32 for t in (t_logits, t_trans, s_logits, s_trans))
    B, L, K = s_logits.shape
    assert t_logits.shape == (B, L, K) and t_trans.shape == (K, K) and s_trans.shape == (K, K)
    t_logits, s_logits = t_logits.contiguous(), s_logits.contiguous()
    logz = torch.empty((B, 2), dtype=torch.float32, device=s_logits.device)
    alpha = torch.empty((2, B, L, K), dtype=torch.float32, device=s_logits.device)
    check(lib().ner_crf_distill_fwd(ptr(t_logits), ptr(t_trans.contiguous()), ptr(s_logits), ptr(s_trans.contiguous()),
                                    ptr(_i32(seq_len)), 1.0 / float(temperature), ptr(logz), ptr(alpha), B, L, K,
                                    1 if exact else 0, stream()))
    return logz, alpha


def crf_distill_bwd(t_logits, t_trans, s_logits, s_trans, seq_len, alpha, logz, temperature=1.0, d_kl=None, scale=1.0,
                    exact=False):
    require_cuda(t_logits, t_trans, s_logits, s_trans, seq_len, alpha, logz, d_kl)
    B, L, K = s_logits.shape
    assert all(t.dtype == torch.float32 for t in (t_logits, t_trans, s_logits, s_trans, alpha, logz)
               + ((d_kl,) if d_kl is not None else ()))
    assert t_logits.shape == (B, L, K) and alpha.shape == (2, B, L, K) and logz.shape == (B, 2)
    assert d_kl is None or d_kl.shape == (B,)
    t_logits, s_logits = t_logits.contiguous(), s_logits.contiguous()
    kl = torch.empty((B,), dtype=torch.float32, device=s_logits.device)
    d_logits = torch.empty_like(s_logits)
    d_trans = torch.zeros_like(s_trans)
    check(lib().ner_crf_distill_bwd(ptr(t_logits), ptr(t_trans.contiguous()), ptr(s_logits), ptr(s_trans.contiguous()),
                                    ptr(_i32(seq_len)), 1.0 / float(temperature), ptr(alpha), ptr(logz),
                                    ptr(None if d_kl is None else d_kl.contiguous()), scale, ptr(kl), ptr(d_logits),
                                    ptr(d_trans), B, L, K, 1 if exact else 0, stream()))
    return kl, d_logits, d_trans


def split_bf16(x2d, Dp=None):
    require_cuda(x2d)
    assert x2d.dtype == torch.float32 and x2d.dim() == 2 and x2d.stride(1) == 1
    M, D = x2d.shape
    Dp = Dp or (D + 7) // 8 * 8
    hi = torch.empty((M, Dp), dtype=torch.bfloat16, device=x2d.device)
    lo = torch.empty((M, Dp), dtype=torch.bfloat16, device=x2d.device)
    check(lib().ner_split_bf16(ptr(x2d), ptr(hi), ptr(lo), M, D, Dp, x2d.stride(0), stream()))
    return hi, lo


def gemm_split_f32(a_hi, a_lo, w_hi, w_lo, bias=None, residual=None, relu=False, out=None):
    M, N = a_hi.shape[0], w_hi.shape[0]
    if out is None:
        out = torch.empty((M, N), dtype=torch.float32, device=a_hi.device)
    gemm_bf16(a_hi, w_hi, bias, residual=residual, epilogue=EPI_RES_F32 if residual is not None else EPI_F32, out=out)
    gemm_bf16(a_hi, w_lo, None, residual=out, epilogue=EPI_RES_F32, out=out)
    gemm_bf16(a_lo, w_hi, None, residual=out, epilogue=EPI_RES_RELU_F32 if relu else EPI_RES_F32, out=out)
    return out


def attention_f32(q, k, v, seq_len, B, L, num_heads, head_dim, scale=1.0, bias_u=None, bias_v=None, rel_table=None,
                  want_f32=True, want_split=False):
    require_cuda(seq_len, bias_u, bias_v, rel_table)
    for t in (q, k, v):
        assert t.is_cuda and t.dtype == torch.float32 and t.dim() == 2 and t.stride(1) == 1 and t.shape[0] == B * L
    HD = num_heads * head_dim
    of = torch.empty((B * L, HD), dtype=torch.float32, device=q.device) if want_f32 else None
    hi = torch.empty((B * L, HD), dtype=torch.bfloat16, device=q.device) if want_split else None
    lo = torch.empty((B * L, HD), dtype=torch.bfloat16, device=q.device) if want_split else None
    check(lib().ner_attention_f32(q.data_ptr(), q.stride(0), k.data_ptr(), k.stride(0), v.data_ptr(), v.stride(0),
                                  ptr(bias_u), ptr(bias_v), ptr(rel_table), ptr(_i32(seq_len)), scale, ptr(of), ptr(hi), ptr(lo),
                                  B, L, num_heads, head_dim, stream()))
    return of, hi, lo


def attention_f32_bwd(q, k, v, seq_len, B, L, num_heads, head_dim, d_out, scale=1.0, bias_u=None, bias_v=None, rel_table=None):
    require_cuda(seq_len, bias_u, bias_v, rel_table, d_out)
    for t in (q, k, v, d_out):
        assert t.is_cuda and t.dtype == torch.float32 and t.dim() == 2 and t.stride(1) == 1 and t.shape[0] == B * L
    HD = num_heads * head_dim
    dq = torch.empty((B * L, HD), dtype=torch.float32, device=q.device)
    dk = torch.zeros((B * L, HD), dtype=torch.float32, device=q.device)
    dv = torch.zeros((B * L, HD), dtype=torch.float32, device=q.device)
    du = torch.zeros((num_heads, head_dim), dtype=torch.float32, device=q.device) if bias_u is not None else None
    dvb = torch.zeros((num_heads, head_dim), dtype=torch.float32, device=q.device) if bias_v is not None else None
    check(lib().ner_attention_f32_bwd(q.data_ptr(), q.stride(0), k.data_ptr(), k.stride(0), v.data_ptr(), v.stride(0),
                                      ptr(bias_u), ptr(bias_v), ptr(rel_table), ptr(_i32(seq_len)), scale, d_out.data_ptr(),
                                      d_out.stride(0), ptr(dq), HD, ptr(dk), HD, ptr(dv), HD, ptr(du), ptr(dvb), B, L, num_heads,
                                      head_dim, stream()))
    return dq, dk, dv, du, dvb


def relu(x, inplace=False):
    require_cuda(x)
    assert x.dtype == torch.float32 and x.is_contiguous()
    y = x if inplace else torch.empty_like(x)
    check(lib().ner_relu_f32(ptr(x), ptr(y), x.numel(), stream()))
    return y


def relu_bwd(act, dact):
    require_cuda(act, dact)
    assert act.dtype == torch.float32 and dact.dtype == torch.float32 and act.numel() == dact.numel()
    out = torch.empty_like(dact)
    check(lib().ner_relu_bwd_f32(ptr(act), ptr(dact), ptr(out), act.numel(), stream()))
    return out


def reduce_max_time(x):
    require_cuda(x)
    assert x.dtype == torch.float32 and x.dim() == 3
    B, L, C = x.shape
    y = torch.empty((B, C), dtype=torch.float32, device=x.device)
    check(lib().ner_reduce_max_time(ptr(x), ptr(y), B, L, C, stream()))
    return y


def reduce_max_time_bwd(x, y, dy, dx, scale=1.0):
    require_cuda(x, y, dy, dx)
    B, L, C = x.shape
    assert dy.dtype == torch.float32 and tuple(dy.shape) == (B, C) and dx.shape == x.shape
    check(lib().ner_reduce_max_time_bwd(ptr(x), ptr(y), ptr(dy), ptr(dx), B, L, C, float(scale), stream()))
    return dx


def softmax_xent(logits, labels, scale=1.0, want_grad=False):
    require_cuda(logits, labels)
    assert logits.dtype == torch.float32 and labels.dtype == torch.int32 and logits.dim() == 2
    B, N = logits.shape
    loss = torch.empty((B,), dtype=torch.float32, device=logits.device)
    dz = torch.empty_like(logits) if want_grad else None
    check(lib().ner_softmax_xent(ptr(logits), ptr(labels), ptr(loss), ptr(dz), B, N, float(scale), stream()))
    return (loss, dz) if want_grad else loss


_token_xent_scratch = {}


def _token_head_scratch(dev):
    key = (dev.index, stream())
    scratch = _token_xent_scratch.get(key)
    if scratch is None:
        scratch = _token_xent_scratch[key] = torch.empty(int(lib().ner_token_xent_scratch_floats()), dtype=torch.float32,
                                                         device=dev)
    return scratch


def token_xent(logits, labels=None, seq_len=None, want_pred=True, want_loss=True, want_grad=False, d_loss=1.0):
    require_cuda(logits, labels, seq_len)
    assert logits.dtype == torch.float32 and logits.dim() == 3
    B, L, K = logits.shape
    dev = logits.device
    if labels is None:
        want_loss = want_grad = False
    else:
        labels, seq_len = _i32(labels), _i32(seq_len)
        assert tuple(labels.shape) == (B, L) and tuple(seq_len.shape) == (B,)
    pred = torch.empty((B, L), dtype=torch.int32, device=dev) if want_pred else None
    loss = torch.empty((), dtype=torch.float32, device=dev) if want_loss else None
    dz = torch.empty_like(logits) if want_grad else None
    scratch = _token_head_scratch(dev) if labels is not None else None
    check(lib().ner_token_xent(ptr(logits), ptr(labels), ptr(seq_len), ptr(pred), ptr(loss), ptr(dz), float(d_loss),
                               ptr(scratch), B, L, K, stream()))
    if B == 0 and loss is not None:
        loss.zero_()
    if B == 0 and dz is not None:
        dz.zero_()
    return pred, loss, dz


def token_dice(logits, labels, seq_len, alpha=1.0, gamma=1.0, want_pred=True, want_loss=True, want_grad=False, d_loss=1.0):
    require_cuda(logits, labels, seq_len)
    assert logits.dtype == torch.float32 and logits.dim() == 3
    B, L, K = logits.shape
    dev = logits.device
    labels, seq_len = _i32(labels), _i32(seq_len)
    assert tuple(labels.shape) == (B, L) and tuple(seq_len.shape) == (B,)
    pred = torch.empty((B, L), dtype=torch.int32, device=dev) if want_pred else None
    loss = torch.empty((), dtype=torch.float32, device=dev) if want_loss else None
    dz = torch.empty_like(logits) if want_grad else None
    check(lib().ner_token_dice(ptr(logits), ptr(labels), ptr(seq_len), ptr(pred), ptr(loss), ptr(dz), float(d_loss),
                               float(alpha), float(gamma), ptr(_token_head_scratch(dev)), B, L, K, stream()))
    if B == 0 and loss is not None:
        loss.zero_()
    if B == 0 and dz is not None:
        dz.zero_()
    return pred, loss, dz


def mrc_pairs(token_ids, seq_len, query_ids, query_len, type_tag, L2, sep_id, label_ids=None):
    require_cuda(token_ids, seq_len, query_ids, query_len, type_tag, label_ids)
    B, L = token_ids.shape
    T, Qmax = query_ids.shape
    token_ids, seq_len = _i32(token_ids), _i32(seq_len)
    label_ids = None if label_ids is None else _i32(label_ids)
    assert query_len.dtype == torch.int32 and type_tag.dtype == torch.int32 and tuple(type_tag.shape) == (T, 2)
    dev = token_ids.device
    pair = lambda *shape: torch.empty(shape, dtype=torch.int32, device=dev)
    out = dict(ids=pair(B * T, L2), segment_ids=pair(B * T, L2), mask=pair(B * T, L2), seq_len=pair(B * T),
               align=pair(B * T * L), labels=None if label_ids is None else pair(B * T, L))
    check(lib().ner_mrc_pairs(ptr(token_ids), ptr(seq_len), ptr(label_ids), ptr(query_ids) if Qmax else None, ptr(query_len),
                              ptr(type_tag), B, L, T, Qmax, L2, int(sep_id), ptr(out['ids']), ptr(out['segment_ids']),
                              ptr(out['mask']), ptr(out['seq_len']), ptr(out['labels']), ptr(out['align']), stream()))
    return out


def mrc_merge(logits, seq_len, type_tag, o_id, cls_id, sep_id):
    require_cuda(logits, seq_len, type_tag)
    assert logits.dtype == torch.float32 and logits.dim() == 3 and logits.shape[2] == 3
    T = type_tag.shape[0]
    BT, L, _ = logits.shape
    assert BT % T == 0 and type_tag.dtype == torch.int32
    seq_len = _i32(seq_len)
    B = BT // T
    assert tuple(seq_len.shape) == (B,)
    pred = torch.empty((B, L), dtype=torch.int32, device=logits.device)
    check(lib().ner_mrc_merge(ptr(logits), ptr(seq_len), ptr(type_tag), B, L, T, int(o_id), int(cls_id), int(sep_id), ptr(pred),
                              stream()))
    return pred


_span_workspace = {}


def _span_scratch(kind, nbytes, dev):
    key = (kind, dev.index, stream())
    buf = _span_workspace.get(key)
    if buf is None or buf.numel() < nbytes:
        buf = _span_workspace[key] = torch.empty(max(int(nbytes), 16), dtype=torch.uint8, device=dev)
    return buf


def _span_uv(uv):
    if not uv.is_cuda:
        raise NerB200Error("ner_b200 kernels take CUDA tensors (got a CPU tensor); there is no CPU path")
    assert uv.dtype == torch.float32 and uv.dim() == 2 and uv.stride(1) == 1
    return uv.stride(0)


def mrc_span_targets(pair_labels, pair_seq_len):
    require_cuda(pair_labels, pair_seq_len)
    P, L = pair_labels.shape
    pair_labels, pair_seq_len = _i32(pair_labels), _i32(pair_seq_len)
    out = [torch.empty((P, L), dtype=torch.int32, device=pair_labels.device) for _ in range(3)]
    check(lib().ner_mrc_span_targets(ptr(pair_labels), ptr(pair_seq_len), P, L, *(ptr(t) for t in out), stream()))
    return tuple(out)


def mrc_span_match_fwd(uv, b1, w2, b2, pair_seq_len, L, span_end=None, keep_prob=1.0, seed=0):
    require_cuda(b1, w2, b2, pair_seq_len, span_end)
    ld = _span_uv(uv)
    I = b1.numel()
    P = pair_seq_len.numel()
    dev = uv.device
    z = torch.empty((P, L, L), dtype=torch.float32, device=dev)
    loss = torch.empty((), dtype=torch.float32, device=dev) if span_end is not None else None
    ws, nbytes = None, 0
    if loss is not None:
        nbytes = int(lib().ner_mrc_span_match_fwd_workspace_bytes(P, L))
        ws = _span_scratch('fwd', nbytes, dev)
    check(lib().ner_mrc_span_match_fwd(ptr(uv), ld, ptr(b1), ptr(w2), ptr(b2), ptr(_i32(pair_seq_len)),
                                       ptr(None if span_end is None else _i32(span_end)), P, L, I, float(keep_prob),
                                       int(seed) & 0xFFFFFFFFFFFFFFFF, ptr(z), ptr(loss), ptr(ws), nbytes, stream()))
    if P == 0 and loss is not None:
        loss.zero_()
    return z, loss


def mrc_span_match_bwd(uv, z, b1, w2, pair_seq_len, span_end, d_loss=1.0, keep_prob=1.0, seed=0):
    require_cuda(z, b1, w2, pair_seq_len, span_end)
    ld = _span_uv(uv)
    I = b1.numel()
    P, L, _ = z.shape
    dev = uv.device
    d_uv = torch.empty((P * L, 2 * I), dtype=torch.float32, device=dev)
    d_b1 = torch.empty((I,), dtype=torch.float32, device=dev)
    d_w2 = torch.empty((I,), dtype=torch.float32, device=dev)
    d_b2 = torch.empty((1,), dtype=torch.float32, device=dev)
    nbytes = int(lib().ner_mrc_span_match_bwd_workspace_bytes(P, I))
    ws = _span_scratch('bwd', nbytes, dev)
    check(lib().ner_mrc_span_match_bwd(ptr(uv), ld, ptr(z), ptr(b1), ptr(w2), ptr(_i32(pair_seq_len)), ptr(_i32(span_end)), P, L,
                                       I, float(d_loss), float(keep_prob), int(seed) & 0xFFFFFFFFFFFFFFFF, ptr(d_uv), ptr(d_b1),
                                       ptr(d_w2), ptr(d_b2), ptr(ws), nbytes, stream()))
    if P == 0:
        for t in (d_uv, d_b1, d_w2, d_b2):
            t.zero_()
    return d_uv, d_b1, d_w2, d_b2


def mrc_span_decode(start_logits, end_logits, uv, b1, w2, b2, seq_len, type_tag, o_id, cls_id, sep_id, cap=None):
    require_cuda(start_logits, end_logits, b1, w2, b2, seq_len, type_tag)
    assert start_logits.dtype == torch.float32 and end_logits.dtype == torch.float32
    ld = _span_uv(uv)
    T = type_tag.shape[0]
    P, L, _ = start_logits.shape
    B = P // T
    I = b1.numel()
    cap = L if cap is None else int(cap)
    dev = start_logits.device
    pred = torch.empty((B, L), dtype=torch.int32, device=dev)
    spans = torch.empty((B, cap), dtype=torch.int32, device=dev)
    probs = torch.empty((B, cap), dtype=torch.float32, device=dev)
    counts = torch.empty((B,), dtype=torch.int32, device=dev)
    nbytes = int(lib().ner_mrc_span_decode_workspace_bytes(P, L))
    ws = _span_scratch('decode', nbytes, dev)
    check(lib().ner_mrc_span_decode(ptr(start_logits.contiguous()), ptr(end_logits.contiguous()), ptr(uv), ld, ptr(b1), ptr(w2),
                                    ptr(b2), ptr(_i32(seq_len)), ptr(type_tag), B, T, L, I, int(o_id), int(cls_id), int(sep_id),
                                    cap, ptr(pred), ptr(spans), ptr(probs), ptr(counts), ptr(ws), nbytes, stream()))
    if B == 0:
        counts.zero_()
    pred.spans, pred.span_probs, pred.span_counts = spans, probs, counts
    return pred


GP_HEAD = 64


def _gp_rows(rot, B, L, cu_seqlens):
    require_cuda(rot, cu_seqlens)
    assert rot.dtype == torch.bfloat16 and rot.dim() == 4 and rot.shape[2] == 2 and rot.shape[3] == GP_HEAD
    assert cu_seqlens is not None or rot.shape[0] == B * L
    return rot.shape[1]


def gp_targets(label_ids, seq_len, type_tag):
    require_cuda(label_ids, seq_len, type_tag)
    B, L = label_ids.shape
    T = type_tag.shape[0]
    assert type_tag.dtype == torch.int32 and tuple(type_tag.shape) == (T, 2)
    out = torch.empty((B, T, L), dtype=torch.int32, device=label_ids.device)
    check(lib().ner_gp_targets(ptr(_i32(label_ids)), ptr(_i32(seq_len)), ptr(type_tag), B, T, L, ptr(out), stream()))
    return out


def gp_rope(proj, B, L, T, cu_seqlens=None, split=False):
    _require_rows(proj)
    require_cuda(cu_seqlens)
    rows = proj.shape[0]
    hi = torch.empty((rows, T, 2, GP_HEAD), dtype=torch.bfloat16, device=proj.device)
    lo = torch.empty_like(hi) if split else None
    check(lib().ner_gp_rope(ptr(proj), proj.stride(0), ptr(cu_seqlens), B, T, L, ptr(hi), ptr(lo), stream()))
    return hi, lo


def gp_rope_bwd(d_rot, B, L, cu_seqlens=None):
    require_cuda(d_rot, cu_seqlens)
    rows, T = d_rot.shape[:2]
    d_proj = torch.empty((rows, T * 2 * GP_HEAD), dtype=torch.float32, device=d_rot.device)
    check(lib().ner_gp_rope_bwd(ptr(d_rot), ptr(cu_seqlens), B, T, L, ptr(d_proj), d_proj.stride(0), stream()))
    return d_proj


def gp_loss_fwd(hi, lo, seq_len, span_end, L, cu_seqlens=None):
    require_cuda(lo, seq_len, span_end)
    B = seq_len.shape[0]
    T = _gp_rows(hi, B, L, cu_seqlens)
    assert tuple(span_end.shape) == (B, T, L) and span_end.dtype == torch.int32
    dev = hi.device
    loss = torch.zeros((), dtype=torch.float32, device=dev)
    lse = torch.zeros((B, T, 2), dtype=torch.float32, device=dev)
    nbytes = int(lib().ner_gp_loss_workspace_bytes(B, T, L))
    ws = _span_scratch('gp_loss', nbytes, dev)
    check(lib().ner_gp_loss_fwd(ptr(hi), ptr(lo), ptr(_i32(seq_len)), ptr(cu_seqlens), ptr(span_end), B, T, L, ptr(loss),
                                ptr(lse), ptr(ws), nbytes, stream()))
    return loss, lse


def gp_loss_bwd(rot, seq_len, span_end, lse, L, d_loss=1.0, cu_seqlens=None):
    require_cuda(seq_len, span_end, lse)
    B = seq_len.shape[0]
    T = _gp_rows(rot, B, L, cu_seqlens)
    d_rot = torch.zeros(rot.shape, dtype=torch.float32, device=rot.device)
    check(lib().ner_gp_loss_bwd(ptr(rot), ptr(_i32(seq_len)), ptr(cu_seqlens), ptr(span_end), ptr(lse), B, T, L,
                                float(d_loss), ptr(d_rot), stream()))
    return d_rot


def gp_decode(hi, lo, seq_len, type_tag, o_id, cls_id, sep_id, L, cu_seqlens=None, cap=None, want_scores=False):
    require_cuda(lo, seq_len, type_tag)
    B = seq_len.shape[0]
    T = _gp_rows(hi, B, L, cu_seqlens)
    assert tuple(type_tag.shape) == (T, 2) and type_tag.dtype == torch.int32
    cap = L if cap is None else int(cap)
    dev = hi.device
    pred = torch.empty((B, L), dtype=torch.int32, device=dev)
    spans = torch.empty((B, cap), dtype=torch.int32, device=dev)
    probs = torch.empty((B, cap), dtype=torch.float32, device=dev)
    counts = torch.zeros((B,), dtype=torch.int32, device=dev)
    nbytes = int(lib().ner_gp_decode_workspace_bytes(B, T, L))
    ws = _span_scratch('gp_decode', nbytes, dev)
    check(lib().ner_gp_decode(ptr(hi), ptr(lo), ptr(_i32(seq_len)), ptr(cu_seqlens), ptr(type_tag), B, T, L, int(o_id),
                              int(cls_id), int(sep_id), cap, ptr(pred), ptr(spans), ptr(probs), ptr(counts), ptr(ws), nbytes,
                              stream()))
    pred.spans, pred.span_probs, pred.span_counts = spans, probs, counts
    if want_scores:
        return pred, ws[:nbytes].view(torch.float32).view(B, T, L, L)
    return pred


def window_plan(token_ids, segment_ids, seq_len, W, S, NW, n_doc, packed=False, padded=False):
    require_cuda(token_ids, segment_ids, seq_len)
    B, L = token_ids.shape
    token_ids, seq_len = _i32(token_ids), _i32(seq_len)
    segment_ids = None if segment_ids is None else _i32(segment_ids)
    dev = token_ids.device
    i32 = lambda *shape: torch.empty(shape, dtype=torch.int32, device=dev)
    out = dict(ids=i32(NW, W), segment_ids=i32(NW, W), mask=i32(NW, W), doc_src_packed=i32(n_doc) if packed else None,
               doc_src_padded=i32(n_doc) if padded else None)
    check(lib().ner_window_plan(ptr(token_ids), ptr(segment_ids), ptr(seq_len), B, L, int(W), int(S), int(NW), ptr(out['ids']),
                                ptr(out['segment_ids']), ptr(out['mask']), ptr(out['doc_src_packed']),
                                ptr(out['doc_src_padded']), stream()))
    return out


def _require_rows(x2d):
    if not x2d.is_cuda:
        raise _lib.NerB200Error("ner_b200 kernels take CUDA tensors (got a CPU tensor); there is no CPU path")
    assert x2d.dtype == torch.float32 and x2d.dim() == 2 and x2d.stride(1) == 1


def transpose_cast_bf16(x2d, Mp=None):
    _require_rows(x2d)
    M, N = x2d.shape
    Mp = Mp or (M + 7) // 8 * 8
    out = torch.empty((N, Mp), dtype=torch.bfloat16, device=x2d.device)
    check(lib().ner_transpose_cast_bf16(ptr(x2d), ptr(out), M, N, Mp, x2d.stride(0), stream()))
    return out


def wgrad_gemm(x2d, dy2d, out=None):
    M = x2d.shape[0]
    Mp = (M + 7) // 8 * 8
    xt = transpose_cast_bf16(x2d, Mp)
    dyt = transpose_cast_bf16(dy2d, Mp)
    N = dyt.shape[0]
    if N % 32 != 0:
        Np = (N + 31) // 32 * 32
        dyt = torch.nn.functional.pad(dyt, (0, 0, 0, Np - N))
    res = gemm_bf16(xt, dyt.contiguous(), None, epilogue=EPI_F32)
    res = res[:, :N] if res.shape[1] != N else res
    if out is not None:
        out.add_(res)
        return out
    return res.contiguous()


def colsum_add(x2d, out, scale=1.0):
    _require_rows(x2d)
    require_cuda(out)
    M, N = x2d.shape
    check(lib().ner_colsum_add(ptr(x2d), ptr(out), M, N, x2d.stride(0), scale, stream()))
    return out


def dense_small_n_bwd(x2d, w, dy, dW, db=None, want_dx=True):
    require_cuda(x2d, w, dy, dW, db)
    assert x2d.dtype == torch.float32
    M, F = x2d.shape
    N = w.shape[1]
    dx = torch.empty((M, F), dtype=torch.float32, device=x2d.device) if want_dx else None
    check(lib().ner_dense_small_n_bwd(ptr(x2d), ptr(w), ptr(dy), ptr(dW), ptr(db), ptr(dx), M, F, N, stream()))
    return dx


def dropout(x, keep_prob, seed, inplace=False):
    require_cuda(x)
    assert x.dtype in (torch.float32, torch.bfloat16) and x.is_contiguous()
    y = x if inplace else torch.empty_like(x)
    fn = lib().ner_dropout if x.dtype == torch.float32 else lib().ner_dropout_bf16
    check(fn(ptr(x), ptr(y), x.numel(), float(keep_prob), int(seed) & 0xFFFFFFFFFFFFFFFF, stream()))
    return y


_sumsq_scratch = {}


def sumsq_add(g, out):
    require_cuda(g, out)
    key = (g.device.index, stream())
    scratch = _sumsq_scratch.get(key)
    if scratch is None:
        scratch = _sumsq_scratch[key] = torch.empty(int(lib().ner_sumsq_scratch_floats()), dtype=torch.float32, device=g.device)
    check(lib().ner_sumsq_add(ptr(g), g.numel(), ptr(out), ptr(scratch), stream()))
    return out


def adam_step(p, g, m, v, lr, beta1=0.9, beta2=0.999, eps=1e-8, weight_decay=0.0, mode=1, clip=0.0, gnorm_sq=None,
              grad_scale=1.0):
    require_cuda(p, g, m, v, gnorm_sq)
    n = p.numel()
    assert g.numel() == n and m.numel() == n and v.numel() == n
    check(lib().ner_adam_step(ptr(p), ptr(g), ptr(m), ptr(v), n, lr, beta1, beta2, eps, weight_decay, mode, clip,
                              ptr(gnorm_sq), grad_scale, stream()))


def layernorm_bwd(y, gamma, d_out, d_gamma, d_beta, residual=None, eps=1e-12, want_f32=True, want_bf16=True, keep_prob=1.0,
                  seed=0, d_bias=None):
    require_cuda(y, gamma, d_out, d_gamma, d_beta, residual, d_bias)
    M, H = y.shape
    dz32 = torch.empty((M, H), dtype=torch.float32, device=y.device) if want_f32 else None
    dz16 = torch.empty((M, H), dtype=torch.bfloat16, device=y.device) if want_bf16 else None
    check(lib().ner_layernorm_dropout_bwd_bias(ptr(y), 1 if y.dtype == torch.bfloat16 else 0, ptr(residual), ptr(gamma),
                                               ptr(d_out), ptr(dz32), ptr(dz16), ptr(d_gamma), ptr(d_beta), ptr(d_bias), M, H, eps,
                                               float(keep_prob), int(seed) & 0xFFFFFFFFFFFFFFFF, stream()))
    return dz32, dz16


def transpose_bf16(x, Mp=None):
    require_cuda(x)
    assert x.dtype == torch.bfloat16 and x.dim() == 2
    M, N = x.shape
    Mp = Mp or (M + 7) // 8 * 8
    out = torch.empty((N, Mp), dtype=torch.bfloat16, device=x.device)
    check(lib().ner_transpose_bf16(ptr(x), ptr(out), M, N, Mp, stream()))
    return out


def wgrad_gemm_bf16(x16, dy16, out_f32=None):
    M = x16.shape[0]
    Mp = (M + 7) // 8 * 8
    xt, dyt = transpose_bf16(x16, Mp), transpose_bf16(dy16, Mp)
    if out_f32 is None:
        return gemm_bf16(xt, dyt, None, epilogue=EPI_F32)
    return gemm_bf16(xt, dyt, None, residual=out_f32, epilogue=EPI_RES_F32, out=out_f32)


def colsum_bf16_add(x16, out):
    require_cuda(x16, out)
    M, N = x16.shape
    check(lib().ner_colsum_bf16_add(ptr(x16), ptr(out), M, N, stream()))
    return out


def gelu_bf16(pre, erf=False):
    require_cuda(pre)
    out = torch.empty_like(pre)
    check(lib().ner_gelu_bf16(ptr(pre), ptr(out), pre.numel(), 1 if erf else 0, stream()))
    return out


def gelu_f32(x, erf=False, inplace=False):
    require_cuda(x)
    assert x.dtype == torch.float32 and x.is_contiguous()
    y = x if inplace else torch.empty_like(x)
    check(lib().ner_gelu_f32(ptr(x), ptr(y), x.numel(), 1 if erf else 0, stream()))
    return y


def gelu_bwd_bias_bf16(pre, dact, d_bias, erf=False):
    require_cuda(pre, dact, d_bias)
    M, N = pre.shape
    out = torch.empty_like(pre)
    check(lib().ner_gelu_bwd_bias_bf16(ptr(pre), ptr(dact), ptr(out), ptr(d_bias), M, N, 1 if erf else 0, stream()))
    return out


def gelu_bwd_bf16(pre, dact, erf=False):
    require_cuda(pre, dact)
    out = torch.empty_like(pre)
    check(lib().ner_gelu_bwd_bf16(ptr(pre), ptr(dact), ptr(out), pre.numel(), 1 if erf else 0, stream()))
    return out


def bert_embed_bwd(dx, ids, seg, d_word, d_type, d_pos):
    require_cuda(dx, ids, seg, d_word, d_type, d_pos)
    B, L = ids.shape
    H = dx.shape[-1]
    check(lib().ner_bert_embed_bwd(ptr(dx), ptr(_i32(ids)), ptr(None if seg is None else _i32(seg)), ptr(d_word), ptr(d_type),
                                   ptr(d_pos), B, L, H, d_word.shape[0], d_type.shape[0], stream()))


def gather_rows(src2d, idx, n):
    require_cuda(src2d, idx)
    assert idx.dtype == torch.int32 and src2d.dim() == 2
    dst = torch.empty((n, src2d.shape[1]), dtype=src2d.dtype, device=src2d.device)
    check(lib().ner_gather_rows(ptr(src2d), ptr(idx), ptr(dst), n, src2d.shape[1] * src2d.element_size(), stream()))
    return dst


def scatter_rows(src2d, idx, rows):
    require_cuda(src2d, idx)
    assert idx.dtype == torch.int32 and src2d.dim() == 2
    dst = torch.zeros((rows, src2d.shape[1]), dtype=src2d.dtype, device=src2d.device)
    check(lib().ner_scatter_rows(ptr(src2d), ptr(idx), ptr(dst), src2d.shape[0], src2d.shape[1] * src2d.element_size(), stream()))
    return dst


def bert_attention_bwd(qkv, mask, ctx, dctx, B, L, num_heads, head_dim=64, scale=None, mask_add=-10000.0, keep_prob=1.0, seed=0,
                       cu_seqlens=None):
    require_cuda(qkv, mask, ctx, dctx, cu_seqlens)
    assert qkv.dtype == torch.bfloat16 and ctx.dtype == torch.bfloat16 and dctx.dtype == torch.bfloat16
    dqkv = torch.empty_like(qkv)
    if scale is None:
        scale = 1.0 / (head_dim ** 0.5)
    if cu_seqlens is not None:
        check(lib().ner_bert_attention_bwd_packed(ptr(qkv), ptr(cu_seqlens), ptr(ctx), ptr(dctx), ptr(dqkv), B, L, num_heads, head_dim,
                                                  scale, float(keep_prob), int(seed) & 0xFFFFFFFFFFFFFFFF, stream()))
        return dqkv
    check(lib().ner_bert_attention_bwd(ptr(qkv), ptr(_i32(mask)), ptr(ctx), ptr(dctx), ptr(dqkv), B, L, num_heads, head_dim,
                                       scale, mask_add, float(keep_prob), int(seed) & 0xFFFFFFFFFFFFFFFF, stream()))
    return dqkv


def tag_classes(idx2tag):
    K = max(idx2tag) + 1
    types, table = [], [0] * K
    for i, tag in idx2tag.items():
        head = tag.split('-')[0]
        kind = 1 if head == 'B' else 2 if head == 'I' else 0
        t = 0
        if kind and '-' in tag:
            name = tag.split('-')[1]
            if name not in types:
                types.append(name)
            t = types.index(name)
        table[i] = kind | (4 if tag[:1] in ('B', 'I') else 0) | (t << 3)
    assert len(types) <= 32
    return torch.tensor(table, dtype=torch.uint8), types


def extract_spans(pred_ids, tag_class, cap=None):
    require_cuda(pred_ids, tag_class)
    B, L = pred_ids.shape
    cap = cap or L
    spans = torch.empty((B, cap), dtype=torch.int32, device=pred_ids.device)
    counts = torch.empty((B,), dtype=torch.int32, device=pred_ids.device)
    check(lib().ner_extract_spans(ptr(_i32(pred_ids)), ptr(tag_class), ptr(spans), ptr(counts), B, L, tag_class.numel(), cap, stream()))
    return spans, counts


def wgrad_group(problems, rows):
    from ._lib import WgradProblem
    arr = (WgradProblem * len(problems))()
    for q, (x, dy, col0, dw) in zip(arr, problems):
        require_cuda(x, dy, dw)
        assert x.dtype == torch.bfloat16 and dy.dtype == torch.bfloat16 and dw.dtype == torch.float32
        q.x_bf16, q.ld_x, q.dy_bf16, q.ld_dy, q.dy_col0 = ptr(x), x.shape[1], ptr(dy), dy.shape[1], int(col0)
        q.dw, q.k_in, q.n_out = ptr(dw), dw.shape[0], dw.shape[1]
    check(lib().ner_wgrad_group_bf16(arr, len(problems), int(rows), stream()))


class PackGroup(object):

    def __init__(self, triples):
        import ctypes
        from ._lib import PackEntry
        arr = (PackEntry * len(triples))()
        starts = [0]
        self.keep = triples
        for q, (src, nk, kn) in zip(arr, triples):
            require_cuda(src)
            for t in (nk, kn):
                if t is not None and not (t.is_cuda and t.dtype == torch.bfloat16 and t.stride(1) == 1):
                    raise NerB200Error("PackGroup destinations must be CUDA bf16 matrices with contiguous rows")
            K, N = src.shape
            assert src.dtype == torch.float32 and src.is_contiguous()
            q.src, q.K, q.N = ptr(src), K, N
            q.dst_nk_bf16, q.ld_nk = (ptr(nk), nk.stride(0)) if nk is not None else (0, 0)
            q.dst_kn_bf16, q.ld_kn = (ptr(kn), kn.stride(0)) if kn is not None else (0, 0)
            starts.append(starts[-1] + ((K + 63) // 64) * ((N + 63) // 64))
        dev = triples[0][0].device
        raw = bytes(memoryview(arr))
        self.table = torch.frombuffer(bytearray(raw), dtype=torch.uint8).to(dev)
        self.starts = torch.tensor(starts, dtype=torch.int32, device=dev)
        self.count, self.tiles = len(triples), starts[-1]
        self.signature = tuple(ptr(t[0]) for t in triples)

    def run(self):
        check(lib().ner_pack_weights_group_bf16(ptr(self.table), ptr(self.starts), self.count, self.tiles, stream()))
```

### include/ner_b200.h

```cpp
#ifndef NER_B200_H_
#define NER_B200_H_

#include <stddef.h>
#include <stdint.h>

#ifdef __cplusplus
extern "C" {
#endif

#define NER_OK 0
#define NER_ERR_INVALID_ARG (-1)
#define NER_ERR_UNSUPPORTED (-2)
#define NER_ERR_WORKSPACE (-3)
#define NER_ERR_NO_DRIVER (-4)
#define NER_ERR_CUDA_BASE (-1000)

typedef void* ner_stream_t;

const char* ner_strerror(int status);
int ner_abi_version(void);
const char* ner_build_info(void);


int ner_crf_viterbi(const float* logits, const int32_t* seq_len, const float* trans,
                    int32_t* tags_out, float* best_score, int B, int L, int K,
                    ner_stream_t stream);

enum {
  NER_VIT_SMALL = 0,
  NER_VIT_TMA = 1,
  NER_VIT_PARKED = 2,
  NER_VIT_ONCHIP_128 = 3,
  NER_VIT_ONCHIP_32 = 4,
  NER_VIT_SMALL_ANY_B = 5,
  NER_VIT_NONE = 6
};
int ner_crf_viterbi_plan(int B, int L, int K, int logits_aligned, int num_sms);

int ner_crf_loglik_fwd(const float* logits, const int32_t* tags, const int32_t* seq_len,
                       const float* trans, float* ll, float* logz_out, float* alpha_ws,
                       int B, int L, int K, int flags, ner_stream_t stream);

int ner_crf_loglik_bwd(const float* logits, const int32_t* tags, const int32_t* seq_len,
                       const float* trans, const float* alpha_ws, const float* logz,
                       const float* d_ll, float scale, float* d_logits, float* d_trans, int B,
                       int L, int K, ner_stream_t stream);

int ner_crf_partial_loglik_fwd(const float* logits, const int32_t* label_mask, const int32_t* seq_len,
                               const float* trans, float* ll, float* logz, float* alpha_ws, int B, int L, int K,
                               int flags, ner_stream_t stream);

int ner_crf_partial_loglik_bwd(const float* logits, const int32_t* label_mask, const int32_t* seq_len,
                               const float* trans, const float* alpha_ws, const float* logz, const float* d_ll,
                               float scale, float* d_logits, float* d_trans, int B, int L, int K, ner_stream_t stream);

int ner_crf_distill_fwd(const float* t_logits, const float* t_trans, const float* s_logits, const float* s_trans,
                        const int32_t* seq_len, float inv_temp, float* logz, float* alpha_ws, int B, int L, int K,
                        int flags, ner_stream_t stream);

int ner_crf_distill_bwd(const float* t_logits, const float* t_trans, const float* s_logits, const float* s_trans,
                        const int32_t* seq_len, float inv_temp, const float* alpha_ws, const float* logz,
                        const float* d_kl, float scale, float* kl, float* d_s_logits, float* d_s_trans, int B, int L,
                        int K, int flags, ner_stream_t stream);

size_t ner_crf_viterbi_nbest_workspace_bytes(int B, int L, int K, int N);
int ner_crf_viterbi_nbest(const float* logits, const int32_t* seq_len, const float* trans, int N, int32_t* tags_out,
                          float* scores_out, int32_t* count_out, void* workspace, size_t workspace_bytes, int B, int L,
                          int K, ner_stream_t stream);


#define NER_EPI_F32 0
#define NER_EPI_BF16 1
#define NER_EPI_GELU_TANH_BF16 2
#define NER_EPI_GELU_ERF_BF16 3
#define NER_EPI_RELU_BF16 4
#define NER_EPI_RES_F32 5
#define NER_EPI_RES_RELU_F32 6
#define NER_EPI_DIAG_DISCARD 99

#define NER_TILE_2CTA_128 1128
#define NER_TILE_2CTA_256 1256
#define NER_TILE_SK_128 2128
#define NER_TILE_SK_256 2256
#define NER_TILE_AUTO_THROUGHPUT 3000

int ner_gemm_bf16(const void* A, const void* Wt, const float* bias, const float* residual,
                  void* out, int M, int N, int K, int epilogue, int tile_n,
                  ner_stream_t stream);

#define NER_EPI_GELU_TANH_E4M3 7
#define NER_EPI_GELU_ERF_E4M3 8
int ner_gemm_e4m3(const void* A, const float* a_scale, const void* Wt, const float* w_scale, const float* bias,
                  void* out, float* out_scale, int M, int N, int K, int epilogue, ner_stream_t stream);

int ner_quantize_weight_e4m3(const float* w_kn, void* wt_nk_e4m3, float* w_scale, int K, int N, ner_stream_t stream);

int ner_pack_weight_bf16(const float* w_kn, void* wt_nk_bf16, int K, int N, ner_stream_t stream);
typedef struct {
  const float* src;
  int K;
  int N;
  void* dst_nk_bf16;
  int ld_nk;
  void* dst_kn_bf16;
  int ld_kn;
} ner_pack_entry;
int ner_pack_weights_group_bf16(const ner_pack_entry* entries_device, const int32_t* tile_start_device, int count,
                                int total_tiles, ner_stream_t stream);
int ner_cast_bf16(const float* src, void* dst_bf16, size_t n, ner_stream_t stream);

int ner_dense_small_n(const void* x, int x_is_bf16, const float* W, const float* bias, float* out,
                      int M, int F, int N, const int32_t* row_map, ner_stream_t stream);

int ner_embedding_lookup(const float* table, const int32_t* ids, float* out, int n_tok, int E,
                         int V, int ld_out, ner_stream_t stream);
int ner_cast_pad_bf16(const float* src, void* dst_bf16, int M, int D, int Dp, int ld_src,
                      ner_stream_t stream);

int ner_seq_pack_plan(const int32_t* mask, int32_t* cu_seqlens, int32_t* tok_src, int B, int L,
                      ner_stream_t stream);

int ner_split_bf16(const float* src, void* hi_bf16, void* lo_bf16, int M, int D, int Dp,
                   int ld_src, ner_stream_t stream);

int ner_attention_f32(const float* Q, int ldq, const float* K, int ldk, const float* V, int ldv,
                      const float* bias_u, const float* bias_v, const float* rel_table,
                      const int32_t* seq_len, float scale, float* out_f32, void* out_hi_bf16,
                      void* out_lo_bf16, int B, int L, int num_heads, int head_dim,
                      ner_stream_t stream);


int ner_bert_embed_ln(const float* word_emb, const float* type_emb, const float* pos_emb,
                      const float* gamma, const float* beta, const int32_t* ids,
                      const int32_t* seg, float* out_f32, void* out_bf16, int B, int L, int H,
                      int vocab, int n_type, int max_pos, float eps, const int32_t* tok_src,
                      int n_packed, ner_stream_t stream);

int ner_layernorm(const void* y, int y_is_bf16, const float* residual, const float* gamma,
                  const float* beta, float* out_f32, void* out_bf16, int M, int H, float eps,
                  ner_stream_t stream);

int ner_bert_embed_ln_e4m3(const float* word_emb, const float* type_emb, const float* pos_emb,
                           const float* gamma, const float* beta, const int32_t* ids,
                           const int32_t* seg, float* out_f32, void* out_bf16, void* out_e4m3, float* out_scale,
                           int B, int L, int H, int vocab, int n_type, int max_pos, float eps,
                           const int32_t* tok_src, int n_packed, ner_stream_t stream);
int ner_layernorm_e4m3(const void* y, int y_is_bf16, const float* residual, const float* gamma,
                       const float* beta, float* out_f32, void* out_bf16, void* out_e4m3, float* out_scale, int M,
                       int H, float eps, ner_stream_t stream);

int ner_layernorm_dropout(const void* y, int y_is_bf16, const float* residual, const float* gamma,
                          const float* beta, float* out_f32, void* out_bf16, int M, int H, float eps,
                          float keep_prob, uint64_t seed, ner_stream_t stream);

int ner_bert_attention(const void* qkv_bf16, const int32_t* mask, void* ctx_bf16, int B, int L,
                       int num_heads, int head_dim, float scale, float mask_add,
                       const int32_t* cu_seqlens, int n_rows, float keep_prob, uint64_t seed,
                       ner_stream_t stream);

int ner_attention_f32_bwd(const float* Q, int ldq, const float* K, int ldk, const float* V, int ldv,
                          const float* bias_u, const float* bias_v, const float* rel_table,
                          const int32_t* seq_len, float scale, const float* d_out, int ld_dout,
                          float* dQ, int ld_dq, float* dK, int ld_dk, float* dV, int ld_dv,
                          float* d_bias_u, float* d_bias_v, int B, int L, int num_heads, int head_dim,
                          ner_stream_t stream);

typedef struct {
  int hidden_size, num_heads, intermediate_size, num_layers;
  int vocab_size, type_vocab_size, max_position;
  float ln_eps;
  int gelu_erf;
  int gemm_tile;
} ner_bert_config;

typedef struct {
  const void* wqkv;  const float* bqkv;
  const void* wo;    const float* bo;
  const float* ln1_gamma; const float* ln1_beta;
  const void* wi;    const float* bi;
  const void* wd;    const float* bd;
  const float* ln2_gamma; const float* ln2_beta;
} ner_bert_layer_weights;

size_t ner_bert_encoder_workspace_bytes(const ner_bert_config* cfg, int rows);
int ner_bert_encoder_fwd(const ner_bert_config* cfg, const float* word_emb, const float* type_emb,
                         const float* pos_emb, const float* emb_ln_gamma, const float* emb_ln_beta,
                         const ner_bert_layer_weights* layers, const int32_t* ids,
                         const int32_t* mask, const int32_t* seg, int B, int L,
                         const int32_t* cu_seqlens, const int32_t* tok_src, int n_packed,
                         float* out_f32, void* out_bf16, void* workspace, size_t workspace_bytes,
                         ner_stream_t stream);

typedef struct {
  const void* wqkv;  const float* sqkv;  const float* bqkv;
  const void* wo;    const float* bo;
  const float* ln1_gamma; const float* ln1_beta;
  const void* wi;    const float* si;    const float* bi;
  const void* wd;    const float* sd;    const float* bd;
  const float* ln2_gamma; const float* ln2_beta;
} ner_bert_layer_weights_fp8;

size_t ner_bert_encoder_fp8_workspace_bytes(const ner_bert_config* cfg, int rows);
int ner_bert_encoder_fwd_fp8(const ner_bert_config* cfg, const float* word_emb, const float* type_emb,
                             const float* pos_emb, const float* emb_ln_gamma, const float* emb_ln_beta,
                             const ner_bert_layer_weights_fp8* layers, const int32_t* ids,
                             const int32_t* mask, const int32_t* seg, int B, int L,
                             const int32_t* cu_seqlens, const int32_t* tok_src, int n_packed,
                             float* out_f32, void* out_bf16, void* workspace, size_t workspace_bytes,
                             ner_stream_t stream);

typedef struct {
  const void* wqkv_kn; const void* wo_kn; const void* wi_kn; const void* wd_kn;
  float* d_wq; float* d_wk; float* d_wv; float* d_bq; float* d_bk; float* d_bv;
  float* d_wo; float* d_bo; float* d_ln1_gamma; float* d_ln1_beta;
  float* d_wi; float* d_bi; float* d_wd; float* d_bd; float* d_ln2_gamma; float* d_ln2_beta;
} ner_bert_layer_grads;

size_t ner_bert_train_saved_bytes(const ner_bert_config* cfg, int rows);
size_t ner_bert_train_scratch_bytes(const ner_bert_config* cfg, int rows);
int ner_bert_encoder_train_fwd(const ner_bert_config* cfg, const float* word_emb, const float* type_emb,
                               const float* pos_emb, const float* emb_ln_gamma, const float* emb_ln_beta,
                               const ner_bert_layer_weights* layers, const int32_t* ids,
                               const int32_t* mask, const int32_t* seg, int B, int L,
                               float hidden_keep, float attn_keep, uint64_t seed, float* out_f32,
                               void* out_bf16, void* saved, size_t saved_bytes, ner_stream_t stream);
int ner_bert_encoder_train_bwd(const ner_bert_config* cfg, const float* emb_ln_gamma,
                               const ner_bert_layer_weights* layers, const ner_bert_layer_grads* grads,
                               float* d_word_emb, float* d_type_emb, float* d_pos_emb,
                               float* d_emb_ln_gamma, float* d_emb_ln_beta, const int32_t* ids,
                               const int32_t* mask, const int32_t* seg, int B, int L,
                               float hidden_keep, float attn_keep, uint64_t seed, const float* d_out,
                               const void* saved, size_t saved_bytes, void* scratch,
                               size_t scratch_bytes, ner_stream_t stream);
size_t ner_bert_train_packed_saved_bytes(const ner_bert_config* cfg, int n_packed);
size_t ner_bert_train_packed_scratch_bytes(const ner_bert_config* cfg, int n_packed, int padded_rows);
int ner_bert_encoder_train_fwd_packed(const ner_bert_config* cfg, const float* word_emb, const float* type_emb,
                                      const float* pos_emb, const float* emb_ln_gamma, const float* emb_ln_beta,
                                      const ner_bert_layer_weights* layers, const int32_t* ids, const int32_t* seg,
                                      int B, int L, const int32_t* cu_seqlens, const int32_t* tok_src, int n_packed,
                                      float hidden_keep, float attn_keep, uint64_t seed, float* out_f32,
                                      void* out_bf16, void* saved, size_t saved_bytes, ner_stream_t stream);
int ner_bert_encoder_train_bwd_packed(const ner_bert_config* cfg, const float* emb_ln_gamma,
                                      const ner_bert_layer_weights* layers, const ner_bert_layer_grads* grads,
                                      float* d_word_emb, float* d_type_emb, float* d_pos_emb,
                                      float* d_emb_ln_gamma, float* d_emb_ln_beta, const int32_t* ids,
                                      const int32_t* seg, int B, int L, const int32_t* cu_seqlens,
                                      const int32_t* tok_src, int n_packed, float hidden_keep, float attn_keep,
                                      uint64_t seed, const float* d_out, const void* saved, size_t saved_bytes,
                                      void* scratch, size_t scratch_bytes, ner_stream_t stream);
int ner_gather_rows(const void* src, const int32_t* idx, void* dst, int n, int row_bytes, ner_stream_t stream);
int ner_scatter_rows(const void* src, const int32_t* idx, void* dst, int n, int row_bytes, ner_stream_t stream);
int ner_bert_embed_sum(const float* word_emb, const float* type_emb, const float* pos_emb,
                       const int32_t* ids, const int32_t* seg, float* out, int B, int L, int H,
                       int vocab, int n_type, int max_pos, ner_stream_t stream);

size_t ner_bert_bilstm_crf_predict_workspace_bytes(const ner_bert_config* cfg, int B, int L, int rows,
                                                   int lstm_hidden, int num_tags);
int ner_bert_bilstm_crf_predict(const ner_bert_config* cfg, const float* word_emb, const float* type_emb,
                                const float* pos_emb, const float* emb_ln_gamma, const float* emb_ln_beta,
                                const ner_bert_layer_weights* layers, const void* lstm_wx_bf16,
                                const float* lstm_bias, const float* lstm_wh_fw, const float* lstm_wh_bw,
                                int lstm_hidden, int lstm_activation, const float* logits_w,
                                const float* logits_b, const float* trans, int num_tags,
                                const int32_t* ids, const int32_t* mask, const int32_t* seg,
                                const int32_t* seq_len, int B, int L, int n_packed, int32_t* pred_ids,
                                void* workspace, size_t workspace_bytes, ner_stream_t stream);


int ner_bilstm_recurrence(const float* xproj, const float* wh_fw, const float* wh_bw,
                          const int32_t* seq_len, float* out, int B, int L, int H,
                          int activation, float forget_bias, const int32_t* cu_seqlens,
                          float* gates_out, float* cstate_out, float* hstate_out, float keep_prob,
                          uint64_t seed, ner_stream_t stream);

int ner_bilstm_recurrence_bwd(const float* d_out, const float* gates, const float* cstate,
                              const float* wh_fw, const float* wh_bw, const int32_t* seq_len,
                              float* d_xproj, int B, int L, int H, int activation, float keep_prob,
                              uint64_t seed, ner_stream_t stream);


int ner_bigru_recurrence(const float* xproj, const float* wh_fw, const float* wh_bw, const int32_t* seq_len,
                         float* out, int B, int L, int H, int ld_xproj, int activation,
                         const int32_t* cu_seqlens, float* gates_out, float* hstate_out, float* rh_out, float keep_prob, uint64_t seed,
                         ner_stream_t stream);

int ner_bigru_recurrence_bwd(const float* d_out, const float* gates, const float* hstate, const float* wh_fw,
                             const float* wh_bw, const int32_t* seq_len, float* d_xproj, int B, int L, int H,
                             int activation, float keep_prob, uint64_t seed, ner_stream_t stream);


int ner_softlexicon_pool_fwd(const float* table, const int32_t* ids, const float* weights,
                             float* out, int n_tok, int G, int S, int E, int V, int ld_out,
                             ner_stream_t stream);
int ner_softlexicon_pool_bwd(float* d_table, const int32_t* ids, const float* weights,
                             const float* d_out, int n_tok, int G, int S, int E, int V,
                             ner_stream_t stream);


int ner_multihot_embed_fwd(const float* table, const float* weights, float* out, int n_tok, int V, int E,
                           int ld_out, ner_stream_t stream);
size_t ner_small_table_grad_scratch_floats(int V, int E);
int ner_small_table_grad(float* d_table, const int32_t* ids, const float* weights, const float* d_out, int n_tok,
                         int V, int E, int ld_dout, float* scratch, ner_stream_t stream);


int ner_transpose_cast_bf16(const float* src, void* dst_bf16, int M, int N, int Mp, int ld_src,
                            ner_stream_t stream);
int ner_colsum_add(const float* x, float* out, int M, int N, int ld, float scale,
                   ner_stream_t stream);
int ner_dense_small_n_bwd(const float* x, const float* W, const float* dy, float* dW, float* db,
                          float* dx, int M, int F, int N, ner_stream_t stream);
int ner_dropout(const float* x, float* y, size_t n, float keep_prob, uint64_t seed,
                ner_stream_t stream);
int ner_dropout_bf16(const void* x_bf16, void* y_bf16, size_t n, float keep_prob, uint64_t seed,
                     ner_stream_t stream);
int ner_relu_f32(const float* x, float* y, size_t n, ner_stream_t stream);
int ner_relu_bwd_f32(const float* act, const float* dact, float* dpre, size_t n, ner_stream_t stream);
int ner_reduce_max_time(const float* x, float* y, int B, int L, int C, ner_stream_t stream);
int ner_reduce_max_time_bwd(const float* x, const float* y, const float* dy, float* dx, int B, int L, int C,
                            float scale, ner_stream_t stream);
int ner_softmax_xent(const float* logits, const int32_t* labels, float* loss, float* dlogits, int B, int N,
                     float scale, ner_stream_t stream);
size_t ner_token_xent_scratch_floats(void);
int ner_token_xent(const float* logits, const int32_t* labels, const int32_t* seq_len, int32_t* pred_ids, float* loss,
                   float* d_logits, float d_loss, float* scratch, int B, int L, int K, ner_stream_t stream);
int ner_token_dice(const float* logits, const int32_t* labels, const int32_t* seq_len, int32_t* pred_ids, float* loss,
                   float* d_logits, float d_loss, float alpha, float gamma, float* scratch, int B, int L, int K,
                   ner_stream_t stream);
int ner_mrc_pairs(const int32_t* token_ids, const int32_t* seq_len, const int32_t* label_ids, const int32_t* query_ids,
                  const int32_t* query_len, const int32_t* type_tag, int B, int L, int T, int Qmax, int L2, int sep_id,
                  int32_t* pair_ids, int32_t* pair_segment_ids, int32_t* pair_mask, int32_t* pair_seq_len,
                  int32_t* pair_labels, int32_t* align_rows, ner_stream_t stream);
int ner_mrc_merge(const float* logits, const int32_t* seq_len, const int32_t* type_tag, int B, int L, int T, int o_id,
                  int cls_id, int sep_id, int32_t* pred_ids, ner_stream_t stream);
int ner_mrc_span_targets(const int32_t* pair_labels, const int32_t* pair_seq_len, int P, int L, int32_t* start_y,
                         int32_t* end_y, int32_t* span_end, ner_stream_t stream);
size_t ner_mrc_span_match_fwd_workspace_bytes(int P, int L);
int ner_mrc_span_match_fwd(const float* uv, int ld_uv, const float* b1, const float* w2, const float* b2,
                           const int32_t* pair_seq_len, const int32_t* span_end, int P, int L, int I, float keep_prob,
                           uint64_t seed, float* z, float* loss, void* workspace, size_t workspace_bytes, ner_stream_t stream);
size_t ner_mrc_span_match_bwd_workspace_bytes(int P, int I);
int ner_mrc_span_match_bwd(const float* uv, int ld_uv, const float* z, const float* b1, const float* w2,
                           const int32_t* pair_seq_len, const int32_t* span_end, int P, int L, int I, float d_loss,
                           float keep_prob, uint64_t seed, float* d_uv, float* d_b1, float* d_w2, float* d_b2, void* workspace,
                           size_t workspace_bytes, ner_stream_t stream);
size_t ner_mrc_span_decode_workspace_bytes(int P, int L);
int ner_mrc_span_decode(const float* start_logits, const float* end_logits, const float* uv, int ld_uv, const float* b1,
                        const float* w2, const float* b2, const int32_t* seq_len, const int32_t* type_tag, int B, int T, int L,
                        int I, int o_id, int cls_id, int sep_id, int cap, int32_t* pred_ids, int32_t* spans,
                        float* span_probs, int32_t* span_counts, void* workspace, size_t workspace_bytes,
                        ner_stream_t stream);
int ner_gp_targets(const int32_t* label_ids, const int32_t* seq_len, const int32_t* type_tag, int B, int T, int L,
                   int32_t* span_end, ner_stream_t stream);
int ner_gp_rope(const float* proj, int ld_proj, const int32_t* cu_seqlens, int B, int T, int L, void* rot_hi, void* rot_lo,
                ner_stream_t stream);
int ner_gp_rope_bwd(const float* d_rot, const int32_t* cu_seqlens, int B, int T, int L, float* d_proj, int ld_dproj,
                    ner_stream_t stream);
size_t ner_gp_loss_workspace_bytes(int B, int T, int L);
int ner_gp_loss_fwd(const void* rot_hi, const void* rot_lo, const int32_t* seq_len, const int32_t* cu_seqlens,
                    const int32_t* span_end, int B, int T, int L, float* loss, float* lse, void* workspace,
                    size_t workspace_bytes, ner_stream_t stream);
int ner_gp_loss_bwd(const void* rot, const int32_t* seq_len, const int32_t* cu_seqlens, const int32_t* span_end,
                    const float* lse, int B, int T, int L, float d_loss, float* d_rot, ner_stream_t stream);
size_t ner_gp_decode_workspace_bytes(int B, int T, int L);
int ner_gp_decode(const void* rot_hi, const void* rot_lo, const int32_t* seq_len, const int32_t* cu_seqlens,
                  const int32_t* type_tag, int B, int T, int L, int o_id, int cls_id, int sep_id, int cap, int32_t* pred_ids,
                  int32_t* spans, float* span_probs, int32_t* span_counts, void* workspace, size_t workspace_bytes,
                  ner_stream_t stream);
int ner_window_plan(const int32_t* token_ids, const int32_t* segment_ids, const int32_t* seq_len, int B, int L, int W, int S,
                    int NW, int32_t* win_ids, int32_t* win_segment_ids, int32_t* win_mask, int32_t* doc_src_packed,
                    int32_t* doc_src_padded, ner_stream_t stream);
int ner_axpy_f32(float* dst, const float* src, size_t n, float a, ner_stream_t stream);
size_t ner_sumsq_scratch_floats(void);
int ner_sumsq_add(const float* g, size_t n, float* out, float* scratch, ner_stream_t stream);
int ner_adam_step(float* p, const float* g, float* m, float* v, size_t n, float lr, float beta1,
                  float beta2, float eps, float weight_decay, int mode, float clip,
                  const float* gnorm_sq, float grad_scale, ner_stream_t stream);


int ner_layernorm_bwd(const void* y, int y_is_bf16, const float* residual, const float* gamma,
                      const float* d_out, float* dz_f32, void* dz_bf16, float* d_gamma,
                      float* d_beta, int M, int H, float eps, ner_stream_t stream);
int ner_layernorm_dropout_bwd(const void* y, int y_is_bf16, const float* residual, const float* gamma,
                              const float* d_out, float* dz_f32, void* dz_bf16, float* d_gamma,
                              float* d_beta, int M, int H, float eps, float keep_prob, uint64_t seed,
                              ner_stream_t stream);
int ner_layernorm_dropout_bwd_bias(const void* y, int y_is_bf16, const float* residual, const float* gamma,
                                   const float* d_out, float* dz_f32, void* dz_bf16, float* d_gamma, float* d_beta,
                                   float* d_bias, int M, int H, float eps, float keep_prob, uint64_t seed,
                                   ner_stream_t stream);
int ner_transpose_bf16(const void* src_bf16, void* dst_bf16, int M, int N, int Mp,
                       ner_stream_t stream);
int ner_colsum_bf16_add(const void* x_bf16, float* out, int M, int N, ner_stream_t stream);
int ner_gelu_bf16(const void* pre_bf16, void* act_bf16, size_t n, int erf_variant, ner_stream_t stream);
int ner_gelu_f32(const float* x, float* y, size_t n, int erf_variant, ner_stream_t stream);
int ner_gelu_bwd_bf16(const void* pre_bf16, const void* dact_bf16, void* dpre_bf16, size_t n,
                      int erf_variant, ner_stream_t stream);
int ner_gelu_bwd_bias_bf16(const void* pre_bf16, const void* dact_bf16, void* dpre_bf16, float* d_bias, int M, int N,
                           int erf_variant, ner_stream_t stream);
int ner_bert_embed_bwd(const float* dx, const int32_t* ids, const int32_t* seg, float* d_word,
                       float* d_type, float* d_pos, int B, int L, int H, int vocab, int n_type,
                       ner_stream_t stream);
int ner_bert_attention_bwd(const void* qkv_bf16, const int32_t* mask, const void* ctx_bf16,
                           const void* dctx_bf16, void* dqkv_bf16, int B, int L, int num_heads,
                           int head_dim, float scale, float mask_add, float keep_prob, uint64_t seed,
                           ner_stream_t stream);
int ner_bert_attention_bwd_packed(const void* qkv_bf16, const int32_t* cu_seqlens, const void* ctx_bf16,
                                  const void* dctx_bf16, void* dqkv_bf16, int B, int L, int num_heads,
                                  int head_dim, float scale, float keep_prob, uint64_t seed,
                                  ner_stream_t stream);

typedef struct {
  const void* x_bf16;
  int ld_x;
  const void* dy_bf16;
  int ld_dy;
  int dy_col0;
  float* dw;
  int k_in;
  int n_out;
} ner_wgrad_problem;
int ner_wgrad_group_bf16(const ner_wgrad_problem* problems_host, int count, int rows, ner_stream_t stream);

int ner_bert_train_bwd_set_layer_events(void* const* events_host, int n_events);

int ner_extract_spans(const int32_t* pred_ids, const uint8_t* tag_class, int32_t* spans, int32_t* counts, int B, int L,
                      int K, int cap, ner_stream_t stream);

typedef struct ner_lexicon ner_lexicon;
ner_lexicon* ner_lexicon_create(const uint32_t* word_codepoints_host, const int64_t* word_offsets_host,
                                const double* freq_host, int n_words);
void ner_lexicon_destroy(ner_lexicon* lexicon);
int64_t ner_lexicon_num_nodes(const ner_lexicon* lexicon);
int ner_lexicon_build(const ner_lexicon* lexicon, const uint32_t* codepoints_host, const int64_t* sent_offsets_host,
                      int n_sent, const int32_t* tok_len_host, const int64_t* tok_offsets_host, int max_seq_len,
                      int bert_mode, int32_t* ids_out_host, float* weights_out_host, int n_threads);
int ner_lexicon_build_lattice(const ner_lexicon* lexicon, const uint32_t* codepoints_host, const int64_t* sent_offsets_host,
                              int n_sent, int max_seq_len, int Kw, int32_t* ids_out_host, int32_t* lens_out_host,
                              int64_t* dropped_out_host, int n_threads);

int ner_lattice_recurrence(const float* xproj, const float* wproj, const int32_t* lat_len, const float* wrec_fw,
                           const float* wrec_bw, const float* wac_fw, const float* wac_bw, const int32_t* seq_len,
                           float* out, int B, int L, int H, int Kw, float* gates, float* cstate, float* norm,
                           float* wgates, float* cw, float* aw, float* hw, ner_stream_t stream);
int ner_lattice_recurrence_bwd(const float* d_out, const float* gates, const float* cstate, const float* norm,
                               const float* wgates, const float* cw, const float* aw, const int32_t* lat_len,
                               const float* wrec_fw, const float* wrec_bw, const float* wac_fw, const float* wac_bw,
                               const int32_t* seq_len, float* d_xproj, float* d_wproj, float* d_alpha, int B, int L,
                               int H, int Kw, ner_stream_t stream);

#ifdef __cplusplus
}
#endif
#endif
```

Before: 49750.

## Sort BiLSTM rows by length and restructure register-weight recurrence dot products

Adds a small kernel that orders batch rows by descending sequence length so each LSTM cluster groups rows of similar length. This cuts the steps wasted waiting on the longest row in a group. Directions are interleaved per cluster, and the inference R=8 override is disabled when an ordering is used. The register-weight path now computes all four gates for a unit per thread on a padded shared-memory h layout, combining results with xor shuffles, which trades register pressure for fewer redundant loads.

```diff
diff --git a/chinesener_b200/_lib.py b/chinesener_b200/_lib.py
--- a/chinesener_b200/_lib.py
+++ b/chinesener_b200/_lib.py
@@ -29,11 +29,12 @@
     "ner_cast_bf16": (_i, [_vp, _vp, _c.c_size_t, _vp]),
     "ner_dense_small_n": (_i, [_vp, _i, _vp, _vp, _vp, _i, _i, _i, _vp, _vp]),
     "ner_seq_pack_plan": (_i, [_vp, _vp, _vp, _i, _i, _vp]),
+    "ner_seq_row_order": (_i, [_vp, _vp, _i, _i, _vp]),
     "ner_bert_embed_ln": (_i, [_vp] * 9 + [_i] * 6 + [_c.c_float, _vp, _i, _vp]),
     "ner_layernorm": (_i, [_vp, _i] + [_vp] * 5 + [_i, _i, _c.c_float, _vp]),
     "ner_layernorm_dropout": (_i, [_vp, _i] + [_vp] * 5 + [_i, _i, _c.c_float, _c.c_float, _c.c_uint64, _vp]),
     "ner_bert_attention": (_i, [_vp, _vp, _vp, _i, _i, _i, _i, _c.c_float, _c.c_float, _vp, _i, _c.c_float, _c.c_uint64, _vp]),
-    "ner_bilstm_recurrence": (_i, [_vp] * 5 + [_i, _i, _i, _i, _c.c_float, _vp, _vp, _vp, _vp, _c.c_float, _c.c_uint64, _vp]),
+    "ner_bilstm_recurrence": (_i, [_vp] * 5 + [_i, _i, _i, _i, _c.c_float, _vp, _vp, _vp, _vp, _vp, _c.c_float, _c.c_uint64, _vp]),
     "ner_bilstm_recurrence_bwd": (_i, [_vp] * 7 + [_i, _i, _i, _i, _c.c_float, _c.c_uint64, _vp]),
     "ner_bigru_recurrence": (_i, [_vp] * 5 + [_i, _i, _i, _i, _i] + [_vp] * 4 + [_c.c_float, _c.c_uint64, _vp]),
     "ner_bigru_recurrence_bwd": (_i, [_vp] * 7 + [_i, _i, _i, _i, _c.c_float, _c.c_uint64, _vp]),
diff --git a/chinesener_b200/csrc/bert_ops.cu b/chinesener_b200/csrc/bert_ops.cu
--- a/chinesener_b200/csrc/bert_ops.cu
+++ b/chinesener_b200/csrc/bert_ops.cu
@@ -369,6 +369,42 @@
   }
 }
 
+__global__ void __launch_bounds__(32) seq_row_order_kernel(const int32_t* __restrict__ seq_len, int32_t* __restrict__ order,
+                                                           int B, int L) {
+  extern __shared__ int s_next[];
+  const int lane = threadIdx.x;
+  for (int v = lane; v <= L; v += 32) s_next[v] = 0;
+  __syncwarp();
+  for (int b = lane; b < B; b += 32) atomicAdd(&s_next[min(max(seq_len[b], 0), L)], 1);
+  __syncwarp();
+  int base = 0;
+  for (int v0 = L; v0 >= 0; v0 -= 32) {
+    const int v = v0 - lane;
+    const int c = v >= 0 ? s_next[v] : 0;
+    int x = c;
+#pragma unroll
+    for (int o = 1; o < 32; o <<= 1) {
+      const int y = __shfl_up_sync(0xffffffffu, x, o);
+      if (lane >= o) x += y;
+    }
+    if (v >= 0) s_next[v] = base + x - c;
+    base += __shfl_sync(0xffffffffu, x, 31);
+  }
+  __syncwarp();
+  for (int b0 = 0; b0 < B; b0 += 32) {
+    const int b = b0 + lane;
+    const int v = b < B ? min(max(seq_len[b], 0), L) : -1;
+    const unsigned peers = __match_any_sync(0xffffffffu, v);
+    const int slot = b < B ? s_next[v] + __popc(peers & ((1u << lane) - 1u)) : 0;
+    __syncwarp();
+    if (b < B) {
+      order[slot] = b;
+      if ((peers >> lane) == 1u) s_next[v] += __popc(peers);
+    }
+    __syncwarp();
+  }
+}
+
 __global__ void __launch_bounds__(256)
 split_bf16_kernel(const float* __restrict__ src, __nv_bfloat16* __restrict__ hi, __nv_bfloat16* __restrict__ lo, int M,
                   int D, int Dp, int ld_src) {
@@ -533,6 +569,15 @@
   return ner_launch_status();
 }
 
+extern "C" int ner_seq_row_order(const int32_t* seq_len, int32_t* row_order, int B, int L, ner_stream_t stream) {
+  if (B < 0 || L < 1) return NER_ERR_INVALID_ARG;
+  if (B == 0) return NER_OK;
+  if (!seq_len || !row_order) return NER_ERR_INVALID_ARG;
+  if ((size_t)(L + 1) * 4 > 48 * 1024) return NER_ERR_UNSUPPORTED;
+  seq_row_order_kernel<<<1, 32, (size_t)(L + 1) * 4, static_cast<cudaStream_t>(stream)>>>(seq_len, row_order, B, L);
+  return ner_launch_status();
+}
+
 extern "C" int ner_split_bf16(const float* src, void* hi_bf16, void* lo_bf16, int M, int D, int Dp, int ld_src,
                               ner_stream_t stream) {
   if (M < 0 || D < 1 || Dp < D || ld_src < D) return NER_ERR_INVALID_ARG;
diff --git a/chinesener_b200/csrc/bilstm.cu b/chinesener_b200/csrc/bilstm.cu
--- a/chinesener_b200/csrc/bilstm.cu
+++ b/chinesener_b200/csrc/bilstm.cu
@@ -11,37 +11,37 @@
 __global__ void __launch_bounds__(H4REG > 0 ? 256 : 512, 1) bilstm_rec_kernel(const float* __restrict__ xproj, const float* __restrict__ wh_fw,
                                   const float* __restrict__ wh_bw, const int32_t* __restrict__ seq_len,
                                   float* __restrict__ out, int B, int L, int H, int C, float forget_bias,
-                                  const int32_t* __restrict__ cu_seqlens, float* __restrict__ gates_out,
+                                  const int32_t* __restrict__ cu_seqlens, const int32_t* __restrict__ row_order,
+                                  float* __restrict__ gates_out,
                                   float* __restrict__ cstate_out, float* __restrict__ hstate_out, float keep_prob,
                                   uint32_t seed_lo, uint32_t seed_hi) {
   cg::cluster_group cluster = cg::this_cluster();
   const int HU = H / C;
   const int NC = 4 * HU;
   const int H4 = H / 4;
-  const rnn::RowGroup grp = rnn::row_group(C, B, R);
+  const rnn::RowGroup grp = rnn::row_group(C, B, R, row_order != nullptr);
   const int rank = grp.rank, dir = grp.dir, b0 = grp.b0;
   const int tid = threadIdx.x;
 
   extern __shared__ __align__(16) float smem[];
   constexpr bool WREG = H4REG > 0;
+  constexpr int HS = H4REG + 4;
+  const int RS = WREG ? 4 * HS : H;
   float4* Ws4 = reinterpret_cast<float4*>(smem);
   float* hbuf = smem + (WREG ? 0 : (size_t)H * NC);
-  int* s_len = reinterpret_cast<int*>(hbuf + 2 * R * H);
-  uint64_t* hbar = reinterpret_cast<uint64_t*>(s_len + 8);
+  int* s_len = reinterpret_cast<int*>(hbuf + 2 * R * RS);
+  int* s_row = s_len + 8;
+  uint64_t* hbar = reinterpret_cast<uint64_t*>(s_len + 16);
 
   const float* wh = dir == 0 ? wh_fw : wh_bw;
-  float4 wreg[WREG ? H4REG : 1];
+  float wq[WREG ? 4 : 1][WREG ? H4REG : 1];
   if constexpr (WREG) {
     if (tid < NC) {
-      const int g0 = tid & 3, u0 = tid >> 2;
-      const size_t gc = (size_t)g0 * H + rank * HU + u0;
-#pragma unroll
-      for (int k4 = 0; k4 < H4REG; ++k4) {
-        wreg[k4].x = wh[(size_t)(4 * k4 + 0) * 4 * H + gc];
-        wreg[k4].y = wh[(size_t)(4 * k4 + 1) * 4 * H + gc];
-        wreg[k4].z = wh[(size_t)(4 * k4 + 2) * 4 * H + gc];
-        wreg[k4].w = wh[(size_t)(4 * k4 + 3) * 4 * H + gc];
-      }
+      const int q0 = tid & 3, u0 = tid >> 2;
+#pragma unroll
+      for (int c = 0; c < 4; ++c)
+#pragma unroll
+        for (int k4 = 0; k4 < H4REG; ++k4) wq[c][k4] = wh[(size_t)(4 * k4 + q0) * 4 * H + (size_t)c * H + rank * HU + u0];
     }
   } else {
     for (int idx = tid; idx < H4 * NC; idx += blockDim.x) {
@@ -56,13 +56,13 @@
       Ws4[idx] = w;
     }
   }
-  for (int idx = tid; idx < 2 * R * H; idx += blockDim.x) hbuf[idx] = 0.f;
+  for (int idx = tid; idx < 2 * R * RS; idx += blockDim.x) hbuf[idx] = 0.f;
   if (tid == 0) {
     rnn::mbar_init_(&hbar[0], 1);
     rnn::mbar_init_(&hbar[1], 1);
     asm volatile("fence.mbarrier_init.release.cluster;" ::: "memory");
   }
-  const int maxlen = rnn::load_lengths<R>(s_len, seq_len, b0, B, L);
+  const int maxlen = rnn::load_lengths<R>(s_len, seq_len, b0, B, L, s_row, row_order);
   cluster.sync();
 
   const bool col_ok = tid < NC;
@@ -77,7 +77,7 @@
   size_t xrow0[R];
 #pragma unroll
   for (int r = 0; r < R; ++r)
-    xrow0[r] = (b0 + r < B) ? (cu_seqlens ? (size_t)cu_seqlens[b0 + r] : (size_t)(b0 + r) * L) : 0;
+    xrow0[r] = (s_row[r] < B) ? (cu_seqlens ? (size_t)cu_seqlens[s_row[r]] : (size_t)s_row[r] * L) : 0;
   float xp[R];
 #pragma unroll
   for (int r = 0; r < R; ++r) {
@@ -93,44 +93,88 @@
 
   const uint32_t h_bytes = (uint32_t)(R * H * 4);
   for (int s = 0; s < maxlen; ++s) {
-    const float* hcur = hbuf + (s & 1) * R * H;
-    float* hnxt = hbuf + ((s + 1) & 1) * R * H;
+    const float* hcur = hbuf + (s & 1) * R * RS;
+    float* hnxt = hbuf + ((s + 1) & 1) * R * RS;
     if (C > 1) {
       if (tid == 0) rnn::mbar_arrive_expect_tx_(&hbar[(s + 1) & 1], h_bytes);
       if (s > 0) rnn::mbar_wait_(&hbar[s & 1], (uint32_t)((s - 1) >> 1) & 1u);
     }
-    nerdev::f32x2 pa[R], pb[R];
-#pragma unroll
-    for (int r = 0; r < R; ++r) {
-      pa[r] = nerdev::pk2(xp[r], 0.f);
-      pb[r] = nerdev::pk2(0.f, 0.f);
-    }
-    if (col_ok) {
+    const int qb = (tid & 31) & ~3;
+    float z_dot[R];
+    if constexpr (WREG) {
+      float acc[4][R];
+#pragma unroll
+      for (int r = 0; r < R; ++r)
+#pragma unroll
+        for (int c = 0; c < 4; ++c) {
+          const float x = __shfl_sync(0xffffffffu, xp[r], qb + c);
+          acc[c][r] = g == 0 ? x : 0.f;
+        }
+      if (col_ok) {
+#pragma unroll
+        for (int r = 0; r < R; ++r) {
+          const int len = s_len[r];
+          xp[r] = 0.f;
+          if (s + 1 < len) {
+            const int pos = dir == 0 ? s + 1 : len - 2 - s;
+            xp[r] = xproj[(xrow0[r] + pos) * 8 * H + xcol];
+          }
+        }
+        const float4* hq4 = reinterpret_cast<const float4*>(hcur + g * HS);
+#pragma unroll
+        for (int j = 0; j < H4REG / 4; ++j) {
+          float4 v[R];
+#pragma unroll
+          for (int r = 0; r < R; ++r) v[r] = hq4[r * (RS / 4) + j];
+#pragma unroll
+          for (int r = 0; r < R; ++r)
+#pragma unroll
+            for (int c = 0; c < 4; ++c) {
+              acc[c][r] = __fmaf_rn(wq[c][4 * j + 0], v[r].x, acc[c][r]);
+              acc[c][r] = __fmaf_rn(wq[c][4 * j + 1], v[r].y, acc[c][r]);
+              acc[c][r] = __fmaf_rn(wq[c][4 * j + 2], v[r].z, acc[c][r]);
+              acc[c][r] = __fmaf_rn(wq[c][4 * j + 3], v[r].w, acc[c][r]);
+            }
+        }
+      }
+      const bool odd = g & 1, high = g & 2;
 #pragma unroll
       for (int r = 0; r < R; ++r) {
-        const int len = s_len[r];
-        xp[r] = 0.f;
-        if (s + 1 < len) {
-          const int pos = dir == 0 ? s + 1 : len - 2 - s;
-          xp[r] = xproj[(xrow0[r] + pos) * 8 * H + xcol];
-        }
-      }
-      const float4* hc4 = reinterpret_cast<const float4*>(hcur);
-      if constexpr (WREG) {
-#pragma unroll
-        for (int k4 = 0; k4 < H4REG; ++k4) rnn::fma2_rows<R>(pa, pb, wreg[k4], hc4, H4, k4);
-      } else {
+        const float k0 = odd ? acc[1][r] : acc[0][r], k1 = odd ? acc[3][r] : acc[2][r];
+        const float t0 = k0 + __shfl_xor_sync(0xffffffffu, odd ? acc[0][r] : acc[1][r], 1);
+        const float t1 = k1 + __shfl_xor_sync(0xffffffffu, odd ? acc[2][r] : acc[3][r], 1);
+        z_dot[r] = (high ? t1 : t0) + __shfl_xor_sync(0xffffffffu, high ? t0 : t1, 2);
+      }
+    } else {
+      nerdev::f32x2 pa[R], pb[R];
+#pragma unroll
+      for (int r = 0; r < R; ++r) {
+        pa[r] = nerdev::pk2(xp[r], 0.f);
+        pb[r] = nerdev::pk2(0.f, 0.f);
+      }
+      if (col_ok) {
+#pragma unroll
+        for (int r = 0; r < R; ++r) {
+          const int len = s_len[r];
+          xp[r] = 0.f;
+          if (s + 1 < len) {
+            const int pos = dir == 0 ? s + 1 : len - 2 - s;
+            xp[r] = xproj[(xrow0[r] + pos) * 8 * H + xcol];
+          }
+        }
+        const float4* hc4 = reinterpret_cast<const float4*>(hcur);
 #pragma unroll 4
         for (int k4 = 0; k4 < H4; ++k4) rnn::fma2_rows<R>(pa, pb, Ws4[k4 * NC + tid], hc4, H4, k4);
       }
+#pragma unroll
+      for (int r = 0; r < R; ++r) z_dot[r] = rnn::sum_chains(pa[r], pb[r]);
     }
     float zi[RC], zj[RC], zf[RC], zo[RC];
 #pragma unroll
     for (int rr = 0; rr < RC; ++rr) zi[rr] = zj[rr] = zf[rr] = zo[rr] = 0.f;
-    const int qb = (tid & 31) & ~3;
 #pragma unroll
     for (int r = 0; r < R; ++r) {
-      const float z = rnn::sum_chains(pa[r], pb[r]);
+      const float z = z_dot[r];
       const float a0 = __shfl_sync(0xffffffffu, z, qb + 0);
       const float a1 = __shfl_sync(0xffffffffu, z, qb + 1);
       const float a2 = __shfl_sync(0xffffffffu, z, qb + 2);
@@ -148,7 +192,7 @@
       const bool cell_ok = col_ok && r < R;
       float i_s = 0.f, j_a = 0.f, f_s = 0.f, o_s = 0.f, h_out = 0.f, h_state = 0.f;
       const int len = cell_ok ? s_len[r] : 0;
-      const int b = b0 + r;
+      const int b = cell_ok ? s_row[r] : B;
       const bool live = cell_ok && s < len;
       const int pos = dir == 0 ? s : len - 1 - s;
       if (live) {
@@ -163,10 +207,11 @@
       }
       if (cell_ok) {
         if (C > 1) {
-          const uint32_t la = nerdev::smem_u32(hnxt + r * H + ug), lb = nerdev::smem_u32(&hbar[(s + 1) & 1]);
+          const int hidx = r * RS + (WREG ? (ug & 3) * HS + (ug >> 2) : ug);
+          const uint32_t la = nerdev::smem_u32(hnxt + hidx), lb = nerdev::smem_u32(&hbar[(s + 1) & 1]);
           rnn::publish_all(la, lb, h_state, C);
         } else {
-          hnxt[r * H + ug] = h_state;
+          hnxt[r * RS + (WREG ? (ug & 3) * HS + (ug >> 2) : ug)] = h_state;
         }
       }
       if (live) {
@@ -187,7 +232,7 @@
     if (C == 1) __syncthreads();
   }
   if (C > 1) cluster.sync();
-  rnn::zero_past_maxlen(out, R, b0, B, L, H, dir, rank, HU, maxlen);
+  rnn::zero_past_maxlen(out, R, b0, B, L, H, dir, rank, HU, maxlen, s_row);
 }
 
 int pick_cluster(int H) {
@@ -201,26 +246,47 @@
 
 template <int R, int ACT, int H4REG>
 int launch_rec(const float* xproj, const float* wh_fw, const float* wh_bw, const int32_t* seq_len, float* out, int B,
-               int L, int H, int C, float forget_bias, const int32_t* cu_seqlens, float* gates_out, float* cstate_out,
-               float* hstate_out, float keep_prob, uint64_t seed, cudaStream_t st) {
+               int L, int H, int C, float forget_bias, const int32_t* cu_seqlens, const int32_t* row_order, float* gates_out,
+               float* cstate_out, float* hstate_out, float keep_prob, uint64_t seed, cudaStream_t st) {
   const int HU = H / C, NC = 4 * HU;
-  const size_t smem = ((H4REG > 0 ? 0 : (size_t)H * NC) + 2 * R * H + 32) * 4;
+  const size_t RS = H4REG > 0 ? 4 * (H4REG + 4) : H;
+  const size_t smem = ((H4REG > 0 ? 0 : (size_t)H * NC) + 2 * R * RS + 32) * 4;
   return rnn::launch_cluster(bilstm_rec_kernel<R, ACT, H4REG>, B, R, C, (NC + 31) / 32 * 32, smem, st, xproj, wh_fw, wh_bw,
-                             seq_len, out, B, L, H, C, forget_bias, cu_seqlens, gates_out, cstate_out, hstate_out,
+                             seq_len, out, B, L, H, C, forget_bias, cu_seqlens, row_order, gates_out, cstate_out, hstate_out,
                              keep_prob, (uint32_t)seed, (uint32_t)(seed >> 32));
+}
+
+template <int ACT>
+int launch_forward(int R, const float* xproj, const float* wh_fw, const float* wh_bw, const int32_t* seq_len, float* out,
+                   int B, int L, int H, int C, float forget_bias, const int32_t* cu_seqlens, const int32_t* row_order,
+                   float* gates_out, float* cstate_out, float* hstate_out, float keep_prob, uint64_t seed, cudaStream_t st) {
+#define GO(RR, HR)                                                                                                      \
+  return launch_rec<RR, ACT, HR>(xproj, wh_fw, wh_bw, seq_len, out, B, L, H, C, forget_bias, cu_seqlens, row_order, \
+                                 gates_out, cstate_out, hstate_out, keep_prob, seed, st)
+  if (H == 128 && 4 * (H / C) <= 256) {
+    if (R == 8) GO(8, 32);
+    if (R == 4) GO(4, 32);
+    if (R == 2) GO(2, 32);
+    GO(1, 32);
+  }
+  if (R >= 4) GO(4, 0);
+  if (R == 2) GO(2, 0);
+  GO(1, 0);
+#undef GO
 }
 
 }
 
 extern "C" int ner_bilstm_recurrence(const float* xproj, const float* wh_fw, const float* wh_bw,
                                      const int32_t* seq_len, float* out, int B, int L, int H, int activation,
-                                     float forget_bias, const int32_t* cu_seqlens, float* gates_out,
-                                     float* cstate_out, float* hstate_out, float keep_prob, uint64_t seed,
+                                     float forget_bias, const int32_t* cu_seqlens, const int32_t* row_order,
+                                     float* gates_out, float* cstate_out, float* hstate_out, float keep_prob, uint64_t seed,
                                      ner_stream_t stream) {
   if (B < 0 || L < 1 || H < 1) return NER_ERR_INVALID_ARG;
   if (B == 0) return NER_OK;
   if (!xproj || !wh_fw || !wh_bw || !seq_len || !out) return NER_ERR_INVALID_ARG;
   if ((gates_out == nullptr) != (cstate_out == nullptr)) return NER_ERR_INVALID_ARG;
+  if (row_order != nullptr && gates_out != nullptr) return NER_ERR_INVALID_ARG;
   if (!(keep_prob > 0.f) || keep_prob > 1.f) return NER_ERR_INVALID_ARG;
   if (activation != 0 && activation != 1) return NER_ERR_INVALID_ARG;
   if (H % 4 != 0) return NER_ERR_UNSUPPORTED;
@@ -228,17 +294,9 @@
   if (C == 0) return NER_ERR_UNSUPPORTED;
   cudaStream_t st = static_cast<cudaStream_t>(stream);
   int R = rnn::rows_per_cluster(B, C);
-  if (H == 128 && (long)2 * ((B + 3) / 4) * C > ner_num_sms()) R = 8;
-#define GO(RR, HR)                                                                                          \
-  return activation == 1 ? launch_rec<RR, 1, HR>(xproj, wh_fw, wh_bw, seq_len, out, B, L, H, C, forget_bias, cu_seqlens, gates_out, cstate_out, hstate_out, keep_prob, seed, st) \
-                         : launch_rec<RR, 0, HR>(xproj, wh_fw, wh_bw, seq_len, out, B, L, H, C, forget_bias, cu_seqlens, gates_out, cstate_out, hstate_out, keep_prob, seed, st)
-  if (H == 128 && 4 * (H / C) <= 256) {
-    if (R == 8) GO(8, 32);
-    if (R == 2) GO(2, 32);
-    GO(1, 32);
-  }
-  if (R >= 4) GO(4, 0);
-  if (R == 2) GO(2, 0);
-  GO(1, 0);
-#undef GO
-}
+  if (row_order == nullptr && H == 128 && (long)2 * ((B + 3) / 4) * C > ner_num_sms()) R = 8;
+  return activation == 1 ? launch_forward<1>(R, xproj, wh_fw, wh_bw, seq_len, out, B, L, H, C, forget_bias, cu_seqlens,
+                                             row_order, gates_out, cstate_out, hstate_out, keep_prob, seed, st)
+                         : launch_forward<0>(R, xproj, wh_fw, wh_bw, seq_len, out, B, L, H, C, forget_bias, cu_seqlens,
+                                             row_order, gates_out, cstate_out, hstate_out, keep_prob, seed, st);
+}
diff --git a/chinesener_b200/csrc/predict_step.cu b/chinesener_b200/csrc/predict_step.cu
--- a/chinesener_b200/csrc/predict_step.cu
+++ b/chinesener_b200/csrc/predict_step.cu
@@ -9,6 +9,7 @@
   if (!cfg || B < 0 || L < 1 || rows < 0) return 0;
   const size_t H = (size_t)cfg->hidden_size, R = (size_t)rows, Hl = (size_t)lstm_hidden;
   return al256((size_t)(B + 1) * 4)
+         + al256((size_t)B * 4)
          + al256((size_t)B * L * 4)
          + al256(R * H * 4) + al256(R * H * 2)
          + al256(R * 8 * Hl * 4)
@@ -37,6 +38,7 @@
   cudaStream_t st = static_cast<cudaStream_t>(stream);
   uint8_t* p = static_cast<uint8_t*>(workspace);
   int32_t* cu = reinterpret_cast<int32_t*>(p);       p += al256((size_t)(B + 1) * 4);
+  int32_t* order = reinterpret_cast<int32_t*>(p);    p += al256((size_t)B * 4);
   int32_t* tok_src = reinterpret_cast<int32_t*>(p);  p += al256((size_t)B * L * 4);
   float* x32 = reinterpret_cast<float*>(p);          p += al256((size_t)n_packed * H * 4);
   void* x16 = p;                                     p += al256((size_t)n_packed * H * 2);
@@ -57,8 +59,10 @@
   if (rc != NER_OK) return rc;
   rc = ner_gemm_bf16(x16, lstm_wx_bf16, lstm_bias, nullptr, xproj, n_packed, 8 * Hl, H, NER_EPI_F32, cfg->gemm_tile, stream);
   if (rc != NER_OK) return rc;
-  rc = ner_bilstm_recurrence(xproj, lstm_wh_fw, lstm_wh_bw, seq_len, lstm_out, B, L, Hl, lstm_activation, 1.0f, cu, nullptr,
-                             nullptr, nullptr, 1.0f, 0, stream);
+  rc = ner_seq_row_order(seq_len, order, B, L, stream);
+  if (rc != NER_OK) return rc;
+  rc = ner_bilstm_recurrence(xproj, lstm_wh_fw, lstm_wh_bw, seq_len, lstm_out, B, L, Hl, lstm_activation, 1.0f, cu, order,
+                             nullptr, nullptr, nullptr, 1.0f, 0, stream);
   if (rc != NER_OK) return rc;
   rc = ner_dense_small_n(lstm_out, 0, logits_w, logits_b, logits, B * L, 2 * Hl, K, nullptr, stream);
   if (rc != NER_OK) return rc;
diff --git a/chinesener_b200/csrc/rnn_cluster.cuh b/chinesener_b200/csrc/rnn_cluster.cuh
--- a/chinesener_b200/csrc/rnn_cluster.cuh
+++ b/chinesener_b200/csrc/rnn_cluster.cuh
@@ -46,16 +46,24 @@
   int dir;
   int b0;
 };
-__device__ __forceinline__ RowGroup row_group(int C, int B, int R) {
+__device__ __forceinline__ RowGroup row_group(int C, int B, int R, bool dirs_inner = false) {
   const int ngroups = (B + R - 1) / R;
   const int cid = blockIdx.x / C;
-  return RowGroup{(int)cooperative_groups::this_cluster().block_rank(), cid / ngroups, (cid % ngroups) * R};
+  const int rank = (int)cooperative_groups::this_cluster().block_rank();
+  if (dirs_inner) return RowGroup{rank, cid & 1, (cid >> 1) * R};
+  return RowGroup{rank, cid / ngroups, (cid % ngroups) * R};
 }
 
 template <int R>
-__device__ __forceinline__ int load_lengths(int* s_len, const int32_t* __restrict__ seq_len, int b0, int B, int L) {
+__device__ __forceinline__ int load_lengths(int* s_len, const int32_t* __restrict__ seq_len, int b0, int B, int L,
+                                            int* s_row = nullptr, const int32_t* __restrict__ row_order = nullptr) {
   const int tid = threadIdx.x;
-  if (tid < R) s_len[tid] = (b0 + tid < B) ? min(max(seq_len[b0 + tid], 0), L) : 0;
+  if (tid < R) {
+    const int i = b0 + tid;
+    const int b = i < B ? (row_order ? row_order[i] : i) : B;
+    s_len[tid] = b < B ? min(max(seq_len[b], 0), L) : 0;
+    if (s_row) s_row[tid] = b;
+  }
   __syncthreads();
   int maxlen = 0;
 #pragma unroll
@@ -105,10 +113,10 @@
 
 
 __device__ __forceinline__ void zero_past_maxlen(float* out, int R, int b0, int B, int L, int H, int dir, int rank,
-                                                 int HU, int maxlen) {
+                                                 int HU, int maxlen, const int* s_row = nullptr) {
   for (int idx = threadIdx.x; idx < R * HU; idx += blockDim.x) {
     const int r = idx / HU, uu = idx - r * HU;
-    const int b = b0 + r;
+    const int b = s_row ? s_row[r] : b0 + r;
     if (b < B)
       for (int s = maxlen; s < L; ++s) out[((size_t)b * L + s) * 2 * H + (size_t)dir * H + rank * HU + uu] = 0.f;
   }
diff --git a/chinesener_b200/ops.py b/chinesener_b200/ops.py
--- a/chinesener_b200/ops.py
+++ b/chinesener_b200/ops.py
@@ -162,6 +162,14 @@
     return cu, tok_src
 
 
+def seq_row_order(seq_len, L):
+    require_cuda(seq_len)
+    seq_len = _i32(seq_len)
+    order = torch.empty((seq_len.shape[0],), dtype=torch.int32, device=seq_len.device)
+    check(lib().ner_seq_row_order(ptr(seq_len), ptr(order), seq_len.shape[0], L, stream()))
+    return order
+
+
 def bert_embed_ln(word_emb, type_emb, pos_emb, gamma, beta, ids, seg, eps=1e-12, want_f32=True, want_bf16=True,
                   tok_src=None, n_packed=0):
     require_cuda(word_emb, type_emb, pos_emb, gamma, beta, ids, seg, tok_src)
@@ -232,8 +240,8 @@
 
 
 def bilstm_recurrence(xproj, wh_fw, wh_bw, seq_len, B, L, H, activation="tanh", forget_bias=1.0, cu_seqlens=None,
-                      save_for_backward=False, keep_prob=1.0, seed=0):
-    require_cuda(xproj, wh_fw, wh_bw, seq_len, cu_seqlens)
+                      save_for_backward=False, keep_prob=1.0, seed=0, row_order=None):
+    require_cuda(xproj, wh_fw, wh_bw, seq_len, cu_seqlens, row_order)
     assert xproj.dtype == torch.float32 and xproj.shape[1] == 8 * H
     assert cu_seqlens is not None or xproj.shape[0] == B * L
     assert wh_fw.shape == (H, 4 * H) and wh_bw.shape == (H, 4 * H)
@@ -246,7 +254,8 @@
         cst = torch.zeros((B, L, 2 * H), dtype=torch.float32, device=xproj.device)
         hst = torch.zeros((B, L, 2 * H), dtype=torch.float32, device=xproj.device)
     check(lib().ner_bilstm_recurrence(ptr(xproj), ptr(wh_fw), ptr(wh_bw), ptr(_i32(seq_len)), ptr(out), B, L, H, act,
-                                      forget_bias, ptr(cu_seqlens), ptr(gates), ptr(cst), ptr(hst), float(keep_prob),
+                                      forget_bias, ptr(cu_seqlens), ptr(None if row_order is None else _i32(row_order)),
+                                      ptr(gates), ptr(cst), ptr(hst), float(keep_prob),
                                       int(seed) & 0xFFFFFFFFFFFFFFFF, stream()))
     return (out, gates, cst, hst) if save_for_backward else out
 
diff --git a/include/ner_b200.h b/include/ner_b200.h
--- a/include/ner_b200.h
+++ b/include/ner_b200.h
@@ -119,6 +119,7 @@
 
 int ner_seq_pack_plan(const int32_t* mask, int32_t* cu_seqlens, int32_t* tok_src, int B, int L,
                       ner_stream_t stream);
+int ner_seq_row_order(const int32_t* seq_len, int32_t* row_order, int B, int L, ner_stream_t stream);
 
 int ner_split_bf16(const float* src, void* hi_bf16, void* lo_bf16, int M, int D, int Dp,
                    int ld_src, ner_stream_t stream);
@@ -270,7 +271,7 @@
 int ner_bilstm_recurrence(const float* xproj, const float* wh_fw, const float* wh_bw,
                           const int32_t* seq_len, float* out, int B, int L, int H,
                           int activation, float forget_bias, const int32_t* cu_seqlens,
-                          float* gates_out, float* cstate_out, float* hstate_out, float keep_prob,
+                          const int32_t* row_order, float* gates_out, float* cstate_out, float* hstate_out, float keep_prob,
                           uint64_t seed, ner_stream_t stream);
 
 int ner_bilstm_recurrence_bwd(const float* d_out, const float* gates, const float* cstate,
```

Measured after the change: 51200 (median of 6 runs). 1.03x the previous value.
